# victoriyaforsythe/PyRayHF

Measured on AMD Instinct MI355X. Metric: virtual-height integrals/s (profile x frequency pairs), higher is better.
Workload: dtype f64

## Files before the change

### include/prhf.h

```cpp
#ifndef PRHF_H
#define PRHF_H

#include <stdint.h>

#ifdef __cplusplus
extern "C" {
#endif

#define PRHF_ABI_VERSION 4

#define PRHF_OK        0
#define PRHF_EINVAL   -1
#define PRHF_ENEGDEN  -2
#define PRHF_EPEAK0   -3
#define PRHF_EHIP     -4
#define PRHF_ENOMEM   -5

#define PRHF_MODE_O 0
#define PRHF_MODE_X 1

#define PRHF_FLAG_DEVICE_PTRS 0x1u
#define PRHF_FLAG_ASYNC       0x2u
#define PRHF_FLAG_GRID_STABLE 0x4u
#define PRHF_FLAG_SHARED_FIELD 0x8u
// ... 162 lines not shown
                                      double phi_max, int32_t renormalize_every, double fill_n, double fill_grad,
                                      double fill_mup, double* out, double* path_t, double* path_r, double* path_phi,
                                      double* path_v_r, double* path_v_phi, int64_t path_stride, uint32_t flags);

int prhf_gradient_home_f64(prhf_ctx* ctx, int32_t geometry, const double* records, int64_t n_fields, int64_t n0,
                           int64_t n1, const double* axis0, const double* axis1, const int64_t* group_field,
                           const double* group_x0_km, const double* group_z0_km, int64_t n_groups,
                           const int64_t* link_group, const double* link_target_km, int64_t n_links,
                           const double* scan_elevation_deg, int64_t n_scan, double earth_radius_km, double s_max_km,
                           double rtol, double atol, double max_step_km, double z_ground_km, double top, double left,
                           double right, int32_t renormalize_every, double fill_n, double fill_grad, double fill_mup,
                           double range_tol_km, int32_t max_iter, int32_t max_roots, double* out, int64_t* n_brackets,
                           uint32_t flags);

int prhf_gradient_home_counters(prhf_ctx* ctx, uint64_t* counters);

int prhf_trace_gradient_hops_f64(prhf_ctx* ctx, int32_t geometry, const double* records, int64_t n_fields, int64_t n0,
                                 int64_t n1, const double* axis0, const double* axis1, const double* x0_km,
                                 const double* z0_km, const double* elevation_deg, const int64_t* ray_field, int64_t n_rays,
                                 double earth_radius_km, double s_max_km, double rtol, double atol, double max_step_km,
                                 double z_ground_km, double top, double left, double right, int32_t renormalize_every,
                                 double fill_n, double fill_grad, double fill_mup, int32_t n_hops, double* out,
                                 double* path_t, double* path_a, double* path_b, double* path_va, double* path_vb,
                                 int64_t path_stride, uint32_t flags);

int prhf_gradient_hop_home_f64(prhf_ctx* ctx, int32_t geometry, const double* records, int64_t n_fields, int64_t n0,
                               int64_t n1, const double* axis0, const double* axis1, const int64_t* group_field,
                               const double* group_x0_km, const double* group_z0_km, int64_t n_groups,
                               const int64_t* link_group, const double* link_target_km, int64_t n_links,
                               const double* scan_elevation_deg, int64_t n_scan, double earth_radius_km, double s_max_km,
                               double rtol, double atol, double max_step_km, double z_ground_km, double top, double left,
                               double right, int32_t renormalize_every, double fill_n, double fill_grad, double fill_mup,
                               double range_tol_km, int32_t max_iter, int32_t max_roots, int32_t n_hops, double* out,
                               int64_t* n_brackets, uint32_t flags);

int prhf_field_build_f64(prhf_ctx* ctx, const double* den, const double* bmag, const double* bpsi, int64_t n0, int64_t n1,
                         const double* axis0, const double* axis1, const double* freq_hz, int64_t n_freq, int32_t mode,
                         int32_t edge_order, double* records, double* mu_out, double* mup_out, uint32_t flags);

int prhf_gradient_skip_f64(prhf_ctx* ctx, int32_t geometry, const double* records, int64_t n_fields, int64_t n0,
                           int64_t n1, const double* axis0, const double* axis1, const int64_t* group_field,
                           const double* group_x0_km, const double* group_z0_km, int64_t n_groups,
                           const double* scan_elevation_deg, int64_t n_scan, double earth_radius_km, double s_max_km,
                           double rtol, double atol, double max_step_km, double z_ground_km, double top, double left,
                           double right, int32_t renormalize_every, double fill_n, double fill_grad, double fill_mup,
                           double elev_tol_deg, int32_t max_iter, double* out, uint32_t flags);

int prhf_gradient_muf_f64(prhf_ctx* ctx, int32_t geometry, const double* den, const double* bmag, const double* bpsi,
                          int64_t n0, int64_t n1, const double* axis0, const double* axis1, int32_t mode, int32_t edge_order,
                          const double* link_x0_km, const double* link_z0_km, const double* link_target_km, int64_t n_links,
                          double f_lo_hz, double f_hi_hz, int32_t n_bisect, const double* scan_elevation_deg, int64_t n_scan,
                          double earth_radius_km, double s_max_km, double rtol, double atol, double max_step_km,
                          double z_ground_km, double top, double left, double right, int32_t renormalize_every,
                          double fill_n, double fill_grad, double fill_mup, double elev_tol_deg, int32_t max_iter,
                          double* out, uint32_t flags);

int prhf_gradient_skip_counters(prhf_ctx* ctx, uint64_t* counters);

int prhf_gradient_hop_skip_f64(prhf_ctx* ctx, int32_t geometry, const double* records, int64_t n_fields, int64_t n0,
                               int64_t n1, const double* axis0, const double* axis1, const int64_t* group_field,
                               const double* group_x0_km, const double* group_z0_km, int64_t n_groups,
                               const double* scan_elevation_deg, int64_t n_scan, double earth_radius_km, double s_max_km,
                               double rtol, double atol, double max_step_km, double z_ground_km, double top, double left,
                               double right, int32_t renormalize_every, double fill_n, double fill_grad, double fill_mup,
                               double elev_tol_deg, int32_t max_iter, int32_t n_hops, double* out, uint32_t flags);

int prhf_gradient_hop_muf_f64(prhf_ctx* ctx, int32_t geometry, const double* den, const double* bmag, const double* bpsi,
                              int64_t n0, int64_t n1, const double* axis0, const double* axis1, int32_t mode,
                              int32_t edge_order, const double* link_x0_km, const double* link_z0_km,
                              const double* link_target_km, int64_t n_links, double f_lo_hz, double f_hi_hz, int32_t n_bisect,
                              const double* scan_elevation_deg, int64_t n_scan, double earth_radius_km, double s_max_km,
                              double rtol, double atol, double max_step_km, double z_ground_km, double top, double left,
                              double right, int32_t renormalize_every, double fill_n, double fill_grad, double fill_mup,
                              double elev_tol_deg, int32_t max_iter, int32_t n_hops, double* out, uint32_t flags);

int prhf_gradient_hop_skip_counters(prhf_ctx* ctx, uint64_t* counters);

int prhf_pair_plan_counters(prhf_ctx* ctx, uint64_t* counters);

int prhf_panel_counters(prhf_ctx* ctx, uint64_t* counters);

int prhf_panel_upper_counters(prhf_ctx* ctx, uint64_t* counters);

int prhf_occupancy(prhf_ctx* ctx, int64_t n_alt, int32_t math, int32_t* workgroups_per_cu);

int prhf_sync(prhf_ctx* ctx);

int prhf_last_kernel_ms(prhf_ctx* ctx, double* ms);

int prhf_recent_kernel_ms(prhf_ctx* ctx, double* ms, int32_t capacity, int32_t* n);

#ifdef __cplusplus
}
#endif
#endif
```

### pyrayhf_amd/_native.py

```python

from __future__ import annotations

import ctypes
import os
import threading

_HERE = os.path.dirname(os.path.abspath(__file__))
LIB_PATH = os.environ.get("PRHF_LIB") or os.path.join(_HERE, "libprhf.so")

OK, EINVAL, ENEGDEN, EPEAK0, EHIP, ENOMEM = 0, -1, -2, -3, -4, -5
MODE_O, MODE_X = 0, 1
FLAG_DEVICE_PTRS, FLAG_ASYNC, FLAG_GRID_STABLE, FLAG_SHARED_FIELD = 0x1, 0x2, 0x4, 0x8
MATH_FAITHFUL, MATH_FAST, MATH_AUTO = 0, 1, 2
ABI_VERSION = 4

c_double_p = ctypes.POINTER(ctypes.c_double)


class Segment(ctypes.Structure):
    _fields_ = [("prof_begin", ctypes.c_int64), ("prof_end", ctypes.c_int64),
                ("mode", ctypes.c_int32), ("n_points", ctypes.c_int32),
                ("mult_offset", ctypes.c_int64), ("out_offset", ctypes.c_int64)]


# ... 60 lines not shown
    "prhf_snell_fan_f64": (ctypes.c_int, [
        ctypes.c_void_p, ctypes.c_int32, ctypes.c_void_p, ctypes.c_void_p, ctypes.c_int64, ctypes.c_void_p,
        ctypes.c_void_p, ctypes.c_int64, ctypes.c_void_p, ctypes.c_void_p, ctypes.c_void_p, ctypes.c_void_p,
        ctypes.c_int64, ctypes.c_int64, ctypes.c_int64, ctypes.c_int32, ctypes.c_double, ctypes.c_double,
        ctypes.c_double, ctypes.c_int32, ctypes.c_void_p, ctypes.c_void_p, ctypes.c_void_p, ctypes.c_int64,
        ctypes.c_uint32]),
    "prhf_snell_home_f64": (ctypes.c_int, [
        ctypes.c_void_p, ctypes.c_int32, ctypes.c_void_p, ctypes.c_void_p, ctypes.c_int64, ctypes.c_void_p,
        ctypes.c_void_p, ctypes.c_int64, ctypes.c_void_p, ctypes.c_int64, ctypes.c_void_p, ctypes.c_void_p,
        ctypes.c_void_p, ctypes.c_void_p, ctypes.c_int64, ctypes.c_int64, ctypes.c_int64, ctypes.c_int32,
        ctypes.c_double, ctypes.c_double, ctypes.c_double, ctypes.c_int32, ctypes.c_double, ctypes.c_int32,
        ctypes.c_int32, ctypes.c_void_p, ctypes.c_void_p, ctypes.c_uint32]),
    "prhf_snell_skip_f64": (ctypes.c_int, [
        ctypes.c_void_p, ctypes.c_int32, ctypes.c_void_p, ctypes.c_void_p, ctypes.c_int64, ctypes.c_void_p,
        ctypes.c_int64, ctypes.c_void_p, ctypes.c_void_p, ctypes.c_void_p, ctypes.c_void_p, ctypes.c_int64,
        ctypes.c_int64, ctypes.c_int64, ctypes.c_int32, ctypes.c_double, ctypes.c_double, ctypes.c_double,
        ctypes.c_int32, ctypes.c_double, ctypes.c_int32, ctypes.c_void_p, ctypes.c_uint32]),
    "prhf_snell_muf_f64": (ctypes.c_int, [
        ctypes.c_void_p, ctypes.c_int32, ctypes.c_void_p, ctypes.c_void_p, ctypes.c_int64, ctypes.c_double,
        ctypes.c_double, ctypes.c_int32, ctypes.c_void_p, ctypes.c_int64, ctypes.c_void_p, ctypes.c_void_p,
        ctypes.c_void_p, ctypes.c_void_p, ctypes.c_int64, ctypes.c_int64, ctypes.c_int64, ctypes.c_int32,
        ctypes.c_double, ctypes.c_double, ctypes.c_double, ctypes.c_int32, ctypes.c_double, ctypes.c_int32,
        ctypes.c_void_p, ctypes.c_uint32]),
    "prhf_field_pack_f64": (ctypes.c_int, [ctypes.c_void_p, ctypes.c_void_p, ctypes.c_void_p, ctypes.c_int64,
                                           ctypes.c_int64, ctypes.c_int64, ctypes.c_void_p, ctypes.c_void_p,
                                           ctypes.c_int32, ctypes.c_void_p, ctypes.c_uint32]),
    "prhf_field_sample_f64": (ctypes.c_int, [ctypes.c_void_p, ctypes.c_void_p, ctypes.c_int64, ctypes.c_int64,
                                             ctypes.c_int64] + [ctypes.c_void_p] * 5 + [ctypes.c_int64] +
                              [ctypes.c_double] * 3 + [ctypes.c_void_p] * 4 + [ctypes.c_uint32]),
    "prhf_trace_gradient_f64": (ctypes.c_int, [ctypes.c_void_p, ctypes.c_void_p, ctypes.c_int64, ctypes.c_int64,
                                               ctypes.c_int64] + [ctypes.c_void_p] * 6 + [ctypes.c_int64] +
                                [ctypes.c_double] * 8 + [ctypes.c_int32] + [ctypes.c_double] * 3 +
                                [ctypes.c_void_p] * 6 + [ctypes.c_int64, ctypes.c_uint32]),
    "prhf_trace_gradient_spherical_f64": (ctypes.c_int, [ctypes.c_void_p, ctypes.c_void_p, ctypes.c_int64, ctypes.c_int64,
                                                         ctypes.c_int64] + [ctypes.c_void_p] * 6 + [ctypes.c_int64] +
                                          [ctypes.c_double] * 9 + [ctypes.c_int32] + [ctypes.c_double] * 3 +
                                          [ctypes.c_void_p] * 6 + [ctypes.c_int64, ctypes.c_uint32]),
    "prhf_gradient_home_f64": (ctypes.c_int, [ctypes.c_void_p, ctypes.c_int32, ctypes.c_void_p, ctypes.c_int64,
                                              ctypes.c_int64, ctypes.c_int64] + [ctypes.c_void_p] * 5 + [ctypes.c_int64] +
                               [ctypes.c_void_p] * 2 + [ctypes.c_int64, ctypes.c_void_p, ctypes.c_int64] +
                               [ctypes.c_double] * 9 + [ctypes.c_int32] + [ctypes.c_double] * 4 +
                               [ctypes.c_int32, ctypes.c_int32, ctypes.c_void_p, ctypes.c_void_p, ctypes.c_uint32]),
    "prhf_gradient_home_counters": (ctypes.c_int, [ctypes.c_void_p, ctypes.POINTER(ctypes.c_uint64)]),
    "prhf_trace_gradient_hops_f64": (ctypes.c_int, [ctypes.c_void_p, ctypes.c_int32, ctypes.c_void_p, ctypes.c_int64,
                                                    ctypes.c_int64, ctypes.c_int64] + [ctypes.c_void_p] * 6 +
                                     [ctypes.c_int64] + [ctypes.c_double] * 9 + [ctypes.c_int32] + [ctypes.c_double] * 3 +
                                     [ctypes.c_int32] + [ctypes.c_void_p] * 6 + [ctypes.c_int64, ctypes.c_uint32]),
    "prhf_gradient_hop_home_f64": (ctypes.c_int, [ctypes.c_void_p, ctypes.c_int32, ctypes.c_void_p, ctypes.c_int64,
                                                  ctypes.c_int64, ctypes.c_int64] + [ctypes.c_void_p] * 5 +
                                   [ctypes.c_int64] + [ctypes.c_void_p] * 2 +
                                   [ctypes.c_int64, ctypes.c_void_p, ctypes.c_int64] + [ctypes.c_double] * 9 +
                                   [ctypes.c_int32] + [ctypes.c_double] * 4 +
                                   [ctypes.c_int32, ctypes.c_int32, ctypes.c_int32, ctypes.c_void_p, ctypes.c_void_p,
                                    ctypes.c_uint32]),
    "prhf_field_build_f64": (ctypes.c_int, [ctypes.c_void_p] * 4 + [ctypes.c_int64, ctypes.c_int64] +
                             [ctypes.c_void_p] * 3 + [ctypes.c_int64, ctypes.c_int32, ctypes.c_int32] +
                             [ctypes.c_void_p] * 3 + [ctypes.c_uint32]),
    "prhf_gradient_skip_f64": (ctypes.c_int, [ctypes.c_void_p, ctypes.c_int32, ctypes.c_void_p, ctypes.c_int64,
                                              ctypes.c_int64, ctypes.c_int64] + [ctypes.c_void_p] * 5 + [ctypes.c_int64] +
                               [ctypes.c_void_p, ctypes.c_int64] + [ctypes.c_double] * 9 + [ctypes.c_int32] +
                               [ctypes.c_double] * 4 + [ctypes.c_int32, ctypes.c_void_p, ctypes.c_uint32]),
    "prhf_gradient_muf_f64": (ctypes.c_int, [ctypes.c_void_p, ctypes.c_int32] + [ctypes.c_void_p] * 3 +
                              [ctypes.c_int64, ctypes.c_int64, ctypes.c_void_p, ctypes.c_void_p, ctypes.c_int32,
                               ctypes.c_int32] + [ctypes.c_void_p] * 3 +
                              [ctypes.c_int64, ctypes.c_double, ctypes.c_double, ctypes.c_int32, ctypes.c_void_p,
                               ctypes.c_int64] + [ctypes.c_double] * 9 + [ctypes.c_int32] + [ctypes.c_double] * 4 +
                              [ctypes.c_int32, ctypes.c_void_p, ctypes.c_uint32]),
    "prhf_gradient_hop_skip_f64": (ctypes.c_int, [ctypes.c_void_p, ctypes.c_int32, ctypes.c_void_p, ctypes.c_int64,
                                                  ctypes.c_int64, ctypes.c_int64] + [ctypes.c_void_p] * 5 +
                                   [ctypes.c_int64] + [ctypes.c_void_p, ctypes.c_int64] + [ctypes.c_double] * 9 +
                                   [ctypes.c_int32] + [ctypes.c_double] * 4 +
                                   [ctypes.c_int32, ctypes.c_int32, ctypes.c_void_p, ctypes.c_uint32]),
    "prhf_gradient_hop_muf_f64": (ctypes.c_int, [ctypes.c_void_p, ctypes.c_int32] + [ctypes.c_void_p] * 3 +
                                  [ctypes.c_int64, ctypes.c_int64, ctypes.c_void_p, ctypes.c_void_p, ctypes.c_int32,
                                   ctypes.c_int32] + [ctypes.c_void_p] * 3 +
                                  [ctypes.c_int64, ctypes.c_double, ctypes.c_double, ctypes.c_int32, ctypes.c_void_p,
                                   ctypes.c_int64] + [ctypes.c_double] * 9 + [ctypes.c_int32] + [ctypes.c_double] * 4 +
                                  [ctypes.c_int32, ctypes.c_int32, ctypes.c_void_p, ctypes.c_uint32]),
    "prhf_gradient_skip_counters": (ctypes.c_int, [ctypes.c_void_p, ctypes.POINTER(ctypes.c_uint64)]),
    "prhf_gradient_hop_skip_counters": (ctypes.c_int, [ctypes.c_void_p, ctypes.POINTER(ctypes.c_uint64)]),
    "prhf_pair_plan_counters": (ctypes.c_int, [ctypes.c_void_p, ctypes.POINTER(ctypes.c_uint64)]),
    "prhf_panel_counters": (ctypes.c_int, [ctypes.c_void_p, ctypes.POINTER(ctypes.c_uint64)]),
    "prhf_panel_upper_counters": (ctypes.c_int, [ctypes.c_void_p, ctypes.POINTER(ctypes.c_uint64)]),
    "prhf_occupancy": (ctypes.c_int, [ctypes.c_void_p, ctypes.c_int64, ctypes.c_int32,
                                      ctypes.POINTER(ctypes.c_int32)]),
    "prhf_sync": (ctypes.c_int, [ctypes.c_void_p]),
    "prhf_last_kernel_ms": (ctypes.c_int, [ctypes.c_void_p, ctypes.POINTER(ctypes.c_double)]),
    "prhf_recent_kernel_ms": (ctypes.c_int, [ctypes.c_void_p, ctypes.POINTER(ctypes.c_double), ctypes.c_int32,
                                             ctypes.POINTER(ctypes.c_int32)]),
}

_lib = None
_lib_lock = threading.Lock()


def load():
    global _lib
    if _lib is not None:
        return _lib
    with _lib_lock:
        if _lib is not None:
            return _lib
        if not os.path.exists(LIB_PATH):
            raise NativeLibraryError(
                f"{LIB_PATH} not found: build it with `python -c 'import __graft_entry__ as g; g.build()'` "
                "or `make -C pyrayhf_amd/csrc` (hipcc, gfx950). There is no CPU fallback.")
        if os.environ.get("PRHF_NO_TORCH_PRELOAD", "") == "":
            try:
                import torch
            except ImportError:
                pass
        try:
            lib = ctypes.CDLL(LIB_PATH)
        except OSError as exc:
            raise NativeLibraryError(f"cannot load {LIB_PATH}: {exc}") from exc
        for name, (res, args) in _PROTOTYPES.items():
            try:
                fn = getattr(lib, name)
            except AttributeError as exc:
                raise NativeLibraryError(f"{LIB_PATH} does not export {name}; rebuild it") from exc
            fn.restype = res
            fn.argtypes = args
        if lib.prhf_abi_version() != ABI_VERSION:
            raise NativeLibraryError(f"ABI version {lib.prhf_abi_version()} != {ABI_VERSION}; rebuild libprhf.so")
        _lib = lib
        return _lib


def exported_symbols():
    return sorted(_PROTOTYPES)


def last_error():
    msg = load().prhf_last_error()
    return msg.decode("utf-8", "replace") if msg else ""


def error_for(code, msg):
    if code == ENEGDEN:
        return ValueError("Density must be non-negative")
    if code == EPEAK0:
        return IndexError(msg or "density peak at index 0")
    if code == EINVAL:
        return ValueError(msg or "invalid argument")
    if code == ENOMEM:
        return MemoryError(msg)
    return NativeLibraryError(msg or f"libprhf error {code}")


def raise_for(code):
    if code == OK:
        return
    raise error_for(code, last_error())


def device_count():
    n = ctypes.c_int(0)
    raise_for(load().prhf_device_count(ctypes.byref(n)))
    return n.value


class Context:

    def __init__(self, device=0):
        self._lib = load()
        self._h = ctypes.c_void_p()
# ... 173 lines not shown
                                                      *(float(v) for v in controls[:8]), int(controls[8]),
                                                      *(float(v) for v in fills), int(n_hops), out, *paths,
                                                      int(path_stride), flags)

    def gradient_hop_home(self, geometry, records, n_fields, n0, n1, axis0, axis1, group_field, group_x0, group_z0, n_groups,
                          link_group, link_target, n_links, scan_elev, n_scan, earth_radius, controls, fills, range_tol,
                          max_iter, max_roots, n_hops, out, n_brackets, flags):
        return self._lib.prhf_gradient_hop_home_f64(self._h, int(geometry), records, n_fields, n0, n1, axis0, axis1,
                                                    group_field, group_x0, group_z0, n_groups, link_group, link_target,
                                                    n_links, scan_elev, n_scan, float(earth_radius),
                                                    *(float(v) for v in controls[:8]), int(controls[8]),
                                                    *(float(v) for v in fills), float(range_tol), int(max_iter),
                                                    int(max_roots), int(n_hops), out, n_brackets, flags)

    def gradient_home_counters(self):
        buf = (ctypes.c_uint64 * 4)()
        raise_for(self._lib.prhf_gradient_home_counters(self._h, buf))
        return tuple(int(v) for v in buf)

    def field_build(self, den, bmag, bpsi, n0, n1, axis0, axis1, freq_hz, n_freq, mode, edge_order, records, mu, mup,
                    flags):
        return self._lib.prhf_field_build_f64(self._h, den, bmag, bpsi, n0, n1, axis0, axis1, freq_hz, n_freq, int(mode),
                                              int(edge_order), records, mu or None, mup or None, flags)

    def gradient_skip(self, geometry, records, n_fields, n0, n1, axis0, axis1, group_field, group_x0, group_z0, n_groups,
                      scan_elev, n_scan, earth_radius, controls, fills, elev_tol, max_iter, out, flags):
        return self._lib.prhf_gradient_skip_f64(self._h, int(geometry), records, n_fields, n0, n1, axis0, axis1,
                                                group_field, group_x0, group_z0, n_groups, scan_elev, n_scan,
                                                float(earth_radius), *(float(v) for v in controls[:8]), int(controls[8]),
                                                *(float(v) for v in fills), float(elev_tol), int(max_iter), out, flags)

    def gradient_muf(self, geometry, den, bmag, bpsi, n0, n1, axis0, axis1, mode, edge_order, link_x0, link_z0, link_target,
                     n_links, f_lo, f_hi, n_bisect, scan_elev, n_scan, earth_radius, controls, fills, elev_tol, max_iter,
                     out, flags):
        return self._lib.prhf_gradient_muf_f64(self._h, int(geometry), den, bmag, bpsi, n0, n1, axis0, axis1, int(mode),
                                               int(edge_order), link_x0, link_z0, link_target, n_links, float(f_lo),
                                               float(f_hi), int(n_bisect), scan_elev, n_scan, float(earth_radius),
                                               *(float(v) for v in controls[:8]), int(controls[8]),
                                               *(float(v) for v in fills), float(elev_tol), int(max_iter), out, flags)

    def gradient_hop_skip(self, geometry, records, n_fields, n0, n1, axis0, axis1, group_field, group_x0, group_z0, n_groups,
                          scan_elev, n_scan, earth_radius, controls, fills, elev_tol, max_iter, n_hops, out, flags):
        return self._lib.prhf_gradient_hop_skip_f64(self._h, int(geometry), records, n_fields, n0, n1, axis0, axis1,
                                                    group_field, group_x0, group_z0, n_groups, scan_elev, n_scan,
                                                    float(earth_radius), *(float(v) for v in controls[:8]),
                                                    int(controls[8]), *(float(v) for v in fills), float(elev_tol),
                                                    int(max_iter), int(n_hops), out, flags)

    def gradient_hop_muf(self, geometry, den, bmag, bpsi, n0, n1, axis0, axis1, mode, edge_order, link_x0, link_z0,
                         link_target, n_links, f_lo, f_hi, n_bisect, scan_elev, n_scan, earth_radius, controls, fills,
                         elev_tol, max_iter, n_hops, out, flags):
        return self._lib.prhf_gradient_hop_muf_f64(self._h, int(geometry), den, bmag, bpsi, n0, n1, axis0, axis1, int(mode),
                                                   int(edge_order), link_x0, link_z0, link_target, n_links, float(f_lo),
                                                   float(f_hi), int(n_bisect), scan_elev, n_scan, float(earth_radius),
                                                   *(float(v) for v in controls[:8]), int(controls[8]),
                                                   *(float(v) for v in fills), float(elev_tol), int(max_iter),
                                                   int(n_hops), out, flags)

    def gradient_hop_skip_counters(self):
        buf = (ctypes.c_uint64 * 5)()
        raise_for(self._lib.prhf_gradient_hop_skip_counters(self._h, buf))
        return tuple(int(v) for v in buf)

    def gradient_skip_counters(self):
        buf = (ctypes.c_uint64 * 4)()
        raise_for(self._lib.prhf_gradient_skip_counters(self._h, buf))
        return tuple(int(v) for v in buf)

    def pair_plan_counters(self):
        buf = (ctypes.c_uint64 * 2)()
        raise_for(self._lib.prhf_pair_plan_counters(self._h, buf))
        return tuple(int(v) for v in buf)

    def panel_counters(self):
        buf = (ctypes.c_uint64 * 2)()
        raise_for(self._lib.prhf_panel_counters(self._h, buf))
        return tuple(int(v) for v in buf)

    def panel_upper_counters(self):
        buf = (ctypes.c_uint64 * 2)()
        raise_for(self._lib.prhf_panel_upper_counters(self._h, buf))
        return tuple(int(v) for v in buf)

    def occupancy(self, n_alt, math):
        n = ctypes.c_int32(0)
        raise_for(self._lib.prhf_occupancy(self._h, int(n_alt), int(math), ctypes.byref(n)))
        return n.value

    def sync(self):
        return self._lib.prhf_sync(self._h)

    def last_kernel_ms(self):
        ms = ctypes.c_double(0.0)
        raise_for(self._lib.prhf_last_kernel_ms(self._h, ctypes.byref(ms)))
        return ms.value

    def recent_kernel_ms(self, count=64):
        buf = (ctypes.c_double * max(int(count), 1))()
        n = ctypes.c_int32(0)
        raise_for(self._lib.prhf_recent_kernel_ms(self._h, buf, int(count), ctypes.byref(n)))
        return [buf[i] for i in range(n.value)]


_tls = threading.local()


def default_device():
    for key in ("PRHF_DEVICE", "LOCAL_RANK"):
        if os.environ.get(key, "") != "":
            return int(os.environ[key])
    return 0


def host_context(device=None):
    ctx = context(device)
    ctx.set_stream(0, borrow=False)
    return ctx


def context(device=None):
    dev = default_device() if device is None else int(device)
    cache = getattr(_tls, "ctx", None)
    if cache is None:
        cache = _tls.ctx = {}
    ctx = cache.get(dev)
    if ctx is None:
        ctx = cache[dev] = Context(dev)
    return ctx
```

### pyrayhf_amd/csrc/prhf_api.cpp

```cpp

#include <hip/hip_runtime_api.h>

#include <algorithm>
#include <cctype>
#include <cmath>
#include <cstdarg>
#include <cstdio>
#include <cstdlib>
#include <cstring>
#include <new>
#include <string>
#include <vector>
#include <xmmintrin.h>

#include "prhf.h"
#include "prhf_kernels.h"
#include "prhf_plan.h"

namespace {

thread_local std::string g_err;

int fail(int code, const char* fmt, ...) {
    char buf[512];
// ... 44 lines not shown
    int prev_ = -1;
    bool switched_ = false;
    hipError_t err_ = hipSuccess;
};
#define ENTER_DEVICE(dev)            \
    DeviceScope device_scope_(dev);  \
    HIP_TRY(device_scope_.error())

hipError_t create_events_untimed(hipEvent_t* ev, int n) {
    for (int i = 0; i < n; ++i) {
        const hipError_t e = hipEventCreateWithFlags(&ev[i], hipEventDisableTiming);
        if (e != hipSuccess) return e;
    }
    return hipSuccess;
}

hipError_t create_events(hipEvent_t* ev, int n) {
    for (int i = 0; i < n; ++i) {
        const hipError_t e = hipEventCreate(&ev[i]);
        if (e != hipSuccess) return e;
    }
    return hipSuccess;
}

}

struct prhf_ctx {
    int device = 0;
    hipStream_t own_stream = nullptr;
    hipStream_t aux_stream = nullptr;
    hipEvent_t fork_ev = nullptr, join_ev = nullptr;
    hipStream_t up_stream = nullptr, down_stream = nullptr;
    hipEvent_t slab_up[3] = {}, slab_done[3] = {}, slab_free = nullptr;
    hipStream_t stream = nullptr;
    static constexpr int kTimingRing = 64;
    hipEvent_t ring0[kTimingRing] = {}, ring1[kTimingRing] = {};
    unsigned long long n_timed = 0;
    int slot = 0;
    int pending = 0;
    bool timed = false;
    hipEvent_t begin_ev() { pending = (int)(n_timed % kTimingRing); return ring0[pending]; }
    hipEvent_t pending_end_ev() const { return ring1[pending]; }
    hipEvent_t end_ev() const { return ring1[slot]; }
    void mark_timed() { slot = pending; ++n_timed; timed = true; }
    int math = PRHF_MATH_AUTO;
    Knobs knobs;
    int cu_count = 256;
    int large_bar = 0;
    DevBuf arena;
    DevBuf partial;
    DevBuf altmin;
    DevBuf pairs;
    DevBuf ftab;
    DevBuf levels;
    DevBuf ptab;
    DevBuf leftover;
    DevBuf leftover_x;
    DevBuf leftover_tall;
    DevBuf leftover_tall_x;
    DevBuf order;
    DevBuf tall;
    DevBuf vjp;
    const double* pairs_src = nullptr;
    int64_t pairs_len = 0;
    prhf::StridedPieces pairs_pieces = {};
    struct HostGrid {
        const double* host = nullptr;
        int64_t len = 0;
        DevBuf mult, pairs;
        bool pairs_ready = false;
        prhf::StridedPieces pieces = {};
    };
    static constexpr int kHostGrids = 16;
    HostGrid host_grid[kHostGrids];
    int n_host_grids = 0;
    bool order_clean = false;
    unsigned* d_status = nullptr;
    unsigned* h_status = nullptr;
    unsigned* h_status_dev = nullptr;
    double* h_pack = nullptr;
    double* h_pack_dev = nullptr;
    unsigned long long* d_words = nullptr;
    unsigned long long* h_words = nullptr;
    unsigned long long* d_plan_counters = nullptr;
    bool status_pending = false;
    uint64_t grad_home_counters[PRHF_GRAD_HOME_COUNTERS] = {};
    DevBuf fields;
    uint64_t grad_skip_counters[PRHF_GRAD_SKIP_COUNTERS + 1] = {};
};

namespace {

int ensure(prhf_ctx* c, DevBuf& b, size_t bytes) {
    if (bytes <= b.cap) return PRHF_OK;
    if (b.p) {
        HIP_TRY(hipStreamSynchronize(c->stream));
        HIP_TRY(hipFree(b.p));
        b.p = nullptr;
        b.cap = 0;
    }
    size_t want = bytes + bytes / 4 + 4096;
    hipError_t e = hipMalloc(&b.p, want);
    if (e != hipSuccess) {
        b.p = nullptr;
        return fail(PRHF_ENOMEM, "hipMalloc(%zu) failed: %s", want, hipGetErrorString(e));
    }
    b.cap = want;
    return PRHF_OK;
}

struct Residual {
    const double* vh_obs;
    double* residual;
    double* cost;
    int64_t n_iono = 0;
    const int32_t* ionogram_of_row = nullptr;
    int64_t* best = nullptr;
    double* best_cost = nullptr;
    size_t cost_elems(int64_t n_prof) const { return (size_t)n_prof * (size_t)(n_iono && !ionogram_of_row ? n_iono : 1); }
};

int status_to_code(unsigned bits) {
    if (bits & PRHF_STATUS_PEAK0)
        return fail(PRHF_EPEAK0, "density peak at index 0: no bottomside levels below the peak");
    if (bits & PRHF_STATUS_NANINPUT)
        return fail(PRHF_EINVAL, "NaN in a profile (alt, bmag or bpsi below the density peak)");
    if (bits & PRHF_STATUS_NEGDEN) return fail(PRHF_ENEGDEN, "Density must be non-negative");
    if (bits & PRHF_STATUS_BADGROUP) return fail(PRHF_EINVAL, "ray_group outside [0, n_groups)");
    if (bits & PRHF_STATUS_BADINDEX) return fail(PRHF_EINVAL, "profile_index outside [0, n_prof)");
    if (bits & PRHF_STATUS_BADFIELD) return fail(PRHF_EINVAL, "field index outside [0, n_fields)");
    if (bits & PRHF_STATUS_PATHLEN) return fail(PRHF_EINVAL, "a ray has more path nodes than path_stride");
    return PRHF_OK;
}

struct Call {
    prhf_ctx* c;
    const double *freq, *den, *bmag, *bpsi, *alt, *mult;
    int64_t n_freq, n_prof, n_alt, prof_stride, alt_stride, mult_len;
    const prhf_segment* segs;
    int32_t n_segs;
    double* out;
    uint32_t flags;
    const Residual* post;
    bool dev, shared_field;
    prhf_ctx::HostGrid* grid;
    double* d_out;
    size_t in_elems, out_elems;
    bool out_direct;
    double* vh_dev;
    const double* d_obs;
    double *d_res, *d_cost;
    const int32_t* d_ion;
    int64_t* d_best;
    double* d_best_cost;
    unsigned* order_made;
};

prhf_ctx::HostGrid* find_host_grid(prhf_ctx* c, const double* mult, int64_t mult_len) {
    for (int g = 0; g < c->n_host_grids; ++g)
        if (c->host_grid[g].host == mult && c->host_grid[g].len == mult_len) return &c->host_grid[g];
    return nullptr;
}

int check_arguments(const Call& k) {
    if (!k.c) return fail(PRHF_EINVAL, "null context");
    if (!k.freq || !k.den || !k.bmag || !k.bpsi || !k.alt || !k.mult || !k.segs || (!k.out && !k.post))
        return fail(PRHF_EINVAL, "null array pointer");
    if (k.post && (!k.post->vh_obs || (!k.post->residual && !k.post->cost)))
        return fail(PRHF_EINVAL, "null array pointer");
    if (k.n_freq < 1 || k.n_prof < 0 || k.n_alt < 1) return fail(PRHF_EINVAL, "bad shape");
    if (k.n_alt > kMaxAltTall) return fail(PRHF_EINVAL, "n_alt %lld exceeds the limit of %lld levels",
                                           (long long)k.n_alt, kMaxAltTall);
    if (k.n_freq > (1 << 20)) return fail(PRHF_EINVAL, "n_freq too large");
    if (k.prof_stride < k.n_alt || (k.alt_stride != 0 && k.alt_stride < k.n_alt))
        return fail(PRHF_EINVAL, "row stride shorter than a row");
    if (k.n_segs < 1 || k.n_segs > PRHF_MAX_SEGMENTS)
        return fail(PRHF_EINVAL, "1..%d segments per launch", PRHF_MAX_SEGMENTS);
    if (k.flags & ~(PRHF_FLAG_DEVICE_PTRS | PRHF_FLAG_ASYNC | PRHF_FLAG_GRID_STABLE | PRHF_FLAG_SHARED_FIELD))
        return fail(PRHF_EINVAL, "unknown flag bits");
    if ((k.flags & PRHF_FLAG_ASYNC) && !k.dev) return fail(PRHF_EINVAL, "PRHF_FLAG_ASYNC needs device pointers");
    const bool grid_known = !k.dev && (k.flags & PRHF_FLAG_GRID_STABLE) && find_host_grid(k.c, k.mult, k.mult_len);
    if (!k.dev && !grid_known) {
        const long long bad = first_decreasing_grid_entry(k.mult, k.mult_len, k.segs, k.n_segs);
        if (bad >= 0) return fail(PRHF_EINVAL, "multiplier[%lld] decreases: the stretched grid must be non-decreasing", bad);
    }
    return PRHF_OK;
}

int decide_tall(const Call& k, bool& tall, long long& lds_levels) {
    prhf_ctx* c = k.c;
    tall = k.n_alt > kMaxAlt;
    lds_levels = k.n_alt;
    if (!(tall && k.n_prof > 0 && c->knobs.trim_lds != 0)) return PRHF_OK;
    long long max_peak = 0;
    if (k.dev) {
        HIP_TRY(hipMemsetAsync(c->d_status + kWordPeak, 0, sizeof(unsigned), c->stream));
        HIP_TRY(prhf::launch_peak_levels(k.den, k.n_prof, k.n_alt, k.prof_stride, c->d_status + kWordPeak, c->stream));
        unsigned peak = 0;
        HIP_TRY(hipMemcpyAsync(&peak, c->d_status + kWordPeak, sizeof(unsigned), hipMemcpyDeviceToHost, c->stream));
        HIP_TRY(hipStreamSynchronize(c->stream));
        max_peak = peak;
    } else {
        for (int64_t p = 0; p < k.n_prof; ++p) {
            const double* d = k.den + (size_t)p * k.prof_stride;
            double bv = -HUGE_VAL;
            long long bi = 0;
            for (int64_t i = 0; i < k.n_alt; ++i) {
                const double key = (d[i] != d[i]) ? HUGE_VAL : d[i];
                if (key > bv) { bv = key; bi = i; }
            }
            max_peak = std::max(max_peak, bi);
        }
    }
    if (max_peak + 1 <= kMaxAlt) {
// ... 153 lines not shown
    int rc;
    if ((rc = ensure(c, table, (size_t)pl.table_entries * 16)) != PRHF_OK) return rc;
    HIP_TRY(prhf::launch_grid_pairs(d_mult, mult_len, static_cast<double*>(table.p), c->stream));
    HIP_TRY(prhf::launch_grid_strided(d_mult, static_cast<double*>(table.p), pl.pieces, c->stream));
    return PRHF_OK;
}

int update_tables(Call& k, const LaunchPlan& pl, prhf::KArgs& a) {
    prhf_ctx* c = k.c;
    if (!pl.want_pairs) return PRHF_OK;
    int rc;
    auto same_pieces = [&](const prhf::StridedPieces& o) { return std::memcmp(&o, &pl.pieces, sizeof pl.pieces) == 0; };
    if (k.grid) {
        if (!k.grid->pairs_ready || !same_pieces(k.grid->pieces)) {
            if ((rc = build_pair_table(c, k.grid->pairs, a.mult, k.mult_len, pl)) != PRHF_OK) return rc;
            k.grid->pairs_ready = true;
            k.grid->pieces = pl.pieces;
        }
        a.pairs = static_cast<const double*>(k.grid->pairs.p);
    } else {
        const bool stable = k.dev && (k.flags & PRHF_FLAG_GRID_STABLE) != 0;
        if (!(stable && c->pairs.p && c->pairs_src == a.mult && c->pairs_len == k.mult_len && same_pieces(c->pairs_pieces))) {
            c->pairs_src = nullptr;
            if ((rc = build_pair_table(c, c->pairs, a.mult, k.mult_len, pl)) != PRHF_OK) return rc;
            if (stable) {
                c->pairs_src = a.mult;
                c->pairs_len = k.mult_len;
                c->pairs_pieces = pl.pieces;
            }
        }
        a.pairs = static_cast<const double*>(c->pairs.p);
    }
    if (!pl.freq_table) return PRHF_OK;
    if ((rc = ensure(c, c->ftab, ((size_t)k.n_freq + 1) * 64)) != PRHF_OK) return rc;
    prhf::ZeroWords zero;
    std::memset(&zero, 0, sizeof zero);
    auto zero_head = [&](DevBuf& b, size_t bytes) -> int {
        int rcz = ensure(c, b, bytes);
        if (rcz != PRHF_OK) return rcz;
        zero.p[zero.n] = static_cast<unsigned*>(b.p);
        zero.words[zero.n++] = 1;
        return PRHF_OK;
    };
    zero.p[zero.n] = c->d_status;
    zero.words[zero.n++] = kStatusWords;
    if (pl.o.blocks > 0) {
        if ((rc = zero_head(c->leftover, pl.o.list_bytes)) != PRHF_OK) return rc;
        if ((rc = zero_head(c->leftover_tall, pl.o.list_bytes)) != PRHF_OK) return rc;
    }
    if (pl.x.blocks > 0) {
        if ((rc = zero_head(c->leftover_x, pl.x.list_bytes)) != PRHF_OK) return rc;
        if ((rc = zero_head(c->leftover_tall_x, pl.x.list_bytes)) != PRHF_OK) return rc;
    }
    if (pl.short_order) {
        const size_t words = PRHF_ORDER_CLASSES * (size_t)(pl.o.blocks + 1);
        const void* before = c->order.p;
        if ((rc = ensure(c, c->order, words * sizeof(unsigned))) != PRHF_OK) return rc;
        unsigned* order = static_cast<unsigned*>(c->order.p);
        if (!c->order_clean || c->order.p != before)
            HIP_TRY(hipMemsetAsync(order, 0, PRHF_ORDER_CLASSES * sizeof(unsigned), c->stream));
        prhf::KArgs ap = a;
        ap.n_segs = pl.o.n_segs;
        ap.n_blocks = pl.o.blocks;
        std::copy(pl.o.seg, pl.o.seg + pl.o.n_segs, ap.seg);
        c->order_clean = false;
        HIP_TRY(prhf::launch_short_order(ap, order, a.freq, static_cast<double*>(c->ftab.p), zero, c->stream));
        k.order_made = order;
    } else {
        HIP_TRY(prhf::launch_freq_table(a.freq, k.n_freq, static_cast<double*>(c->ftab.p), zero, c->stream));
    }
    a.ftab = static_cast<const double*>(c->ftab.p);
    return PRHF_OK;
}

int zero_control_words(prhf_ctx* c, const LaunchPlan& pl) {
    if (!pl.zero_queues) return PRHF_OK;
    HIP_TRY(hipMemsetAsync(c->d_status, 0, kLaunchQueueWords * sizeof(unsigned), c->stream));
    if (pl.x.n_segs > 0) HIP_TRY(hipMemsetAsync(c->d_status + kWordShortXFull, 0, sizeof(unsigned), c->stream));
    return PRHF_OK;
}

int launch_general(prhf_ctx* c, const LaunchPlan& pl, prhf::KArgs& a) {
    if (pl.queue) a.queue = c->d_status + kWordGeneral;
    if (pl.tall) HIP_TRY(prhf::launch_vfo_tall(a, pl.grid, c->stream));
    else HIP_TRY(prhf::launch_vfo(a, pl.grid, pl.launch_tier, pl.lds_bytes, c->stream));
    return PRHF_OK;
}

struct ShortRoute {
    StatusWord first, full, follow;
    DevBuf *left, *left_tall;
    int follow_tier;
    unsigned* order;
    bool traced;
};

template <class Launch>
int launch_short_kind(prhf_ctx* c, const LaunchPlan& pl, const ShortKind& sk, const ShortRoute& r, const prhf::KArgs& a,
                      hipStream_t stream, Launch launch) {
    if (sk.blocks == 0) return PRHF_OK;
    prhf::KArgs as = a;
    as.n_segs = sk.n_segs;
    std::copy(sk.seg, sk.seg + sk.n_segs, as.seg);
    as.n_blocks = sk.blocks;
    as.short_prio = (int)c->knobs.short_prio;
    as.partial = nullptr;
    as.altmin = nullptr;
    as.trace = nullptr;
    int rc;
#ifdef PRHF_TRACE
    static DevBuf trace_short;
    const size_t short_trace_words = (size_t)sk.blocks * kWavesPerBlock * 8;
    unsigned long long* trace = nullptr;
    if (std::getenv("PRHF_TRACE_FILE") && r.traced) {
        if ((rc = ensure(c, trace_short, short_trace_words * 8)) != PRHF_OK) return rc;
        HIP_TRY(hipMemsetAsync(trace_short.p, 0, short_trace_words * 8, stream));
        as.trace = trace = static_cast<unsigned long long*>(trace_short.p);
    }
#endif
    if ((rc = ensure(c, *r.left, sk.list_bytes)) != PRHF_OK) return rc;
    as.leftover = static_cast<unsigned*>(r.left->p);
    if (!pl.freq_table) HIP_TRY(hipMemsetAsync(as.leftover, 0, sizeof(unsigned), stream));
    if (sk.second) {
        if ((rc = ensure(c, *r.left_tall, sk.list_bytes)) != PRHF_OK) return rc;
        as.leftover_tall = static_cast<unsigned*>(r.left_tall->p);
        if (!pl.freq_table) HIP_TRY(hipMemsetAsync(as.leftover_tall, 0, sizeof(unsigned), stream));
    }
    as.lds_levels = sk.first.lds_levels;
    as.short_queue = sk.first.short_queue;
    as.queue = sk.first.queue ? c->d_status + r.first : nullptr;
    as.order = r.order;
    if ((rc = launch(as, sk.first)) != PRHF_OK) return rc;
    if (sk.second) {
        as.trace = nullptr;
        as.lds_levels = sk.full.lds_levels;
        as.short_queue = sk.full.short_queue;
        as.block_list = as.leftover_tall;
        as.order = nullptr;
        as.leftover_tall = nullptr;
        as.queue = c->d_status + r.full;
        if ((rc = launch(as, sk.full)) != PRHF_OK) return rc;
    }
#ifdef PRHF_TRACE
    if (trace) {
        std::vector<unsigned long long> host(short_trace_words);
        HIP_TRY(hipMemcpyAsync(host.data(), trace, short_trace_words * 8, hipMemcpyDeviceToHost, stream));
        HIP_TRY(hipStreamSynchronize(stream));
        if (FILE* fp = std::fopen(std::getenv("PRHF_TRACE_FILE"), "wb")) {
            std::fwrite(host.data(), 8, short_trace_words, fp);
            std::fclose(fp);
        }
    }
#endif
    as.trace = nullptr;
    as.lds_levels = a.lds_levels;
    as.short_queue = sk.first.short_queue;
    as.leftover_tall = nullptr;
    as.order = nullptr;
    as.block_list = as.leftover;
    as.leftover = nullptr;
    as.queue = c->d_status + r.follow;
    as.zero_after = r.order;
    HIP_TRY(prhf::launch_vfo(as, sk.follow_grid, r.follow_tier, pl.lds_bytes, stream));
    if (as.zero_after) c->order_clean = true;
    return PRHF_OK;
}

// ... 58 lines not shown
        HIP_TRY(prhf::launch_vfo_shortx(as, l.grid, l.lds_bytes, l.threads, short_stream));
        return PRHF_OK;
    });
    if (rc != PRHF_OK) return rc;
    rc = launch_short_kind(c, pl, pl.o, route_o, a, short_stream, [&](const prhf::KArgs& as, const ShortLaunch& l) -> int {
        HIP_TRY(prhf::launch_vfo_short(as, l.grid, l.lds_bytes, l.threads, pl.o.lanes, short_stream));
        return PRHF_OK;
    });
    if (rc != PRHF_OK) return rc;
    if (pl.forked) {
        HIP_TRY(hipEventRecord(c->join_ev, c->aux_stream));
        HIP_TRY(hipStreamWaitEvent(c->stream, c->join_ev, 0));
        return PRHF_OK;
    }
    return launch_general(c, pl, a);
}

int download_and_sync(Call& k) {
    prhf_ctx* c = k.c;
    const size_t out_elems = k.out_elems;
    const bool out_via_pack = !k.out_direct && !k.dev && k.out && out_elems && c->h_pack && out_elems * 8 <= kPackBytes / 4 &&
                              k.in_elems * 8 <= kPackBytes / 2;
    double* h_out = c->h_pack ? c->h_pack + kPackBytes / 16 : nullptr;
    if (k.out_direct) {
    } else if (out_via_pack)
        HIP_TRY(hipMemcpyAsync(h_out, k.d_out, out_elems * 8, hipMemcpyDeviceToHost, c->stream));
    else if (!k.dev && out_elems && k.out)
        HIP_TRY(hipMemcpyAsync(k.out, k.d_out, out_elems * 8, hipMemcpyDeviceToHost, c->stream));
    if (!k.dev && k.post) {
        if (k.post->residual)
            HIP_TRY(hipMemcpyAsync(k.post->residual, k.d_res, out_elems * 8, hipMemcpyDeviceToHost, c->stream));
        if (k.post->cost && !k.post->n_iono)
            HIP_TRY(hipMemcpyAsync(k.post->cost, k.d_cost, (size_t)k.n_prof * 8, hipMemcpyDeviceToHost, c->stream));
        if (k.post->n_iono) {
            if (k.post->cost_elems(k.n_prof))
                HIP_TRY(hipMemcpyAsync(k.post->cost, k.d_cost, k.post->cost_elems(k.n_prof) * 8, hipMemcpyDeviceToHost,
                                       c->stream));
            HIP_TRY(hipMemcpyAsync(k.post->best, k.d_best, (size_t)k.post->n_iono * 8, hipMemcpyDeviceToHost, c->stream));
            HIP_TRY(hipMemcpyAsync(k.post->best_cost, k.d_best_cost, (size_t)k.post->n_iono * 8, hipMemcpyDeviceToHost, c->stream));
        }
    }
    if (k.flags & PRHF_FLAG_ASYNC) return PRHF_OK;
    const int rc = prhf_sync(c);
    if (out_via_pack || k.out_direct) std::memcpy(k.out, h_out, out_elems * 8);
    return rc;
}

int run(prhf_ctx* c, const double* freq, int64_t n_freq, const double* den, const double* bmag,
        const double* bpsi, const double* alt, int64_t n_prof, int64_t n_alt, int64_t prof_stride,
        int64_t alt_stride, const double* mult, int64_t mult_len, const prhf_segment* segs, int32_t n_segs,
        double* out, uint32_t flags, const Residual* post = nullptr) {
    Call k = {c, freq, den, bmag, bpsi, alt, mult, n_freq, n_prof, n_alt, prof_stride, alt_stride, mult_len, segs, n_segs,
              out, flags, post, (flags & PRHF_FLAG_DEVICE_PTRS) != 0, (flags & PRHF_FLAG_SHARED_FIELD) != 0};
    int rc;
    if ((rc = check_arguments(k)) != PRHF_OK) return rc;
    ENTER_DEVICE(c->device);
    bool tall;
    long long lds_levels;
    if ((rc = decide_tall(k, tall, lds_levels)) != PRHF_OK) return rc;

    const LaunchShape shape = {n_prof, n_freq, n_alt, lds_levels, tall, mult_len, c->cu_count, c->math};
    LaunchPlan pl;
    char why[160];
    if (plan_launch(shape, segs, n_segs, c->knobs, pl, why, sizeof why) != PRHF_OK) return fail(PRHF_EINVAL, "%s", why);

    prhf::KArgs a;
    std::memset(&a, 0, sizeof a);
    a.n_freq = n_freq;
    a.n_alt = n_alt;
    a.lds_levels = lds_levels;
    a.n_segs = pl.n_segs;
    std::copy(pl.seg, pl.seg + pl.n_segs, a.seg);
    a.n_blocks = pl.blocks;
    a.no_candidates = pl.no_candidates;
    a.plan_counters = c->d_plan_counters;
    a.plan_cap = (int)c->knobs.pair_plan_cap;
    if ((rc = stage_inputs(k, pl, a)) != PRHF_OK) return rc;

    const bool timed_launch = k.dev || c->knobs.timing != 0;
    if (timed_launch) HIP_TRY(hipEventRecord(c->begin_ev(), c->stream));
    if ((rc = update_tables(k, pl, a)) != PRHF_OK) return rc;
#ifdef PRHF_TRACE
    static DevBuf trace_buf;
    const size_t trace_words = (size_t)pl.blocks * kWavesPerBlock * 6;
    if (std::getenv("PRHF_TRACE_FILE") && pl.blocks > 0) {
        if ((rc = ensure(c, trace_buf, trace_words * 8)) != PRHF_OK) return rc;
        HIP_TRY(hipMemsetAsync(trace_buf.p, 0, trace_words * 8, c->stream));
        a.trace = static_cast<unsigned long long*>(trace_buf.p);
    }
#endif
    if (pl.tall_stride) {
        a.tall_stride = pl.tall_stride;
        if ((rc = ensure(c, c->tall, (size_t)pl.tall_slabs * a.tall_stride)) != PRHF_OK) return rc;
        a.tall = static_cast<unsigned char*>(c->tall.p);
    }
    if ((rc = zero_control_words(c, pl)) != PRHF_OK) return rc;
    if ((rc = launch_all(k, pl, a)) != PRHF_OK) return rc;
#ifdef PRHF_TRACE
    if (a.trace) {
        std::vector<unsigned long long> host(trace_words);
        HIP_TRY(hipMemcpyAsync(host.data(), a.trace, trace_words * 8, hipMemcpyDeviceToHost, c->stream));
        HIP_TRY(hipStreamSynchronize(c->stream));
        if (FILE* fp = std::fopen(std::getenv("PRHF_TRACE_FILE"), "wb")) {
            std::fwrite(host.data(), 8, trace_words, fp);
            std::fclose(fp);
        }
    }
#endif
    if (post && post->n_iono) {
        if ((rc = launch_many(c, k.vh_dev, n_prof, k.d_obs, post->n_iono, n_freq, k.d_ion, k.d_res, k.d_cost, k.d_best,
                              k.d_best_cost)) != PRHF_OK) return rc;
    } else if (post) HIP_TRY(prhf::launch_residual(k.vh_dev, k.d_obs, n_prof, (int)n_freq, k.d_res, k.d_cost, c->stream));
    if (timed_launch) {
        HIP_TRY(hipEventRecord(c->pending_end_ev(), c->stream));
        c->mark_timed();
    }
    c->status_pending = true;
    return download_and_sync(k);
}

int run_host_slabs(prhf_ctx* c, const double* freq, int64_t n_freq, const double* den, const double* bmag,
                   const double* bpsi, const double* alt, int64_t n_prof, int64_t n_alt, int64_t prof_stride,
                   int64_t alt_stride, const double* mult, int32_t n_points, int32_t mode, double* out, uint32_t flags) {
    const bool shared_field = (flags & PRHF_FLAG_SHARED_FIELD) != 0;
    ENTER_DEVICE(c->device);
    const size_t n_alt_rows = alt_stride ? (size_t)n_prof : 1, n_field_rows = shared_field ? 1 : (size_t)n_prof;
    const size_t row_bytes = (size_t)n_alt * 8;
    const size_t elems = (size_t)n_freq + ((size_t)n_prof + 2 * n_field_rows + n_alt_rows) * (size_t)n_alt + (size_t)n_points +
                         (size_t)n_prof * (size_t)n_freq;
    int rc;
    if ((rc = ensure(c, c->arena, elems * 8)) != PRHF_OK) return rc;
    double* d_freq = static_cast<double*>(c->arena.p);
    double* d_den = d_freq + n_freq;
    double* d_bmag = d_den + (size_t)n_prof * n_alt;
    double* d_bpsi = d_bmag + n_field_rows * n_alt;
    double* d_alt = d_bpsi + n_field_rows * n_alt;
    double* d_mult = d_alt + n_alt_rows * n_alt;
    double* d_out = d_mult + n_points;
    HIP_TRY(hipEventRecord(c->slab_free, c->stream));
    HIP_TRY(hipStreamWaitEvent(c->up_stream, c->slab_free, 0));
    HIP_TRY(hipMemcpyAsync(d_freq, freq, (size_t)n_freq * 8, hipMemcpyHostToDevice, c->up_stream));
    HIP_TRY(hipMemcpyAsync(d_mult, mult, (size_t)n_points * 8, hipMemcpyHostToDevice, c->up_stream));
    if (!alt_stride) HIP_TRY(hipMemcpyAsync(d_alt, alt, row_bytes, hipMemcpyHostToDevice, c->up_stream));
    if (shared_field) {
        HIP_TRY(hipMemcpyAsync(d_bmag, bmag, row_bytes, hipMemcpyHostToDevice, c->up_stream));
        HIP_TRY(hipMemcpyAsync(d_bpsi, bpsi, row_bytes, hipMemcpyHostToDevice, c->up_stream));
    }
    const int n_slabs = 3;
    const int64_t cut[4] = {0, std::max<int64_t>(1, n_prof / 10), std::max<int64_t>(2, (n_prof * 4) / 10), n_prof};
    const uint32_t dev_flags = PRHF_FLAG_DEVICE_PTRS | PRHF_FLAG_ASYNC | (shared_field ? PRHF_FLAG_SHARED_FIELD : 0);
    int first_error = PRHF_OK;
    for (int k = 0; k < n_slabs && first_error == PRHF_OK; ++k) {
        const int64_t p0 = cut[k], rows = cut[k + 1] - cut[k];
        if (rows <= 0) continue;
        auto up2d = [&](double* dst, const double* src, int64_t stride) {
            return hipMemcpy2DAsync(dst + (size_t)p0 * n_alt, row_bytes, src + (size_t)p0 * stride, (size_t)stride * 8, row_bytes,
                                    (size_t)rows, hipMemcpyHostToDevice, c->up_stream);
        };
        HIP_TRY(up2d(d_den, den, prof_stride));
        if (!shared_field) {
            HIP_TRY(up2d(d_bmag, bmag, prof_stride));
            HIP_TRY(up2d(d_bpsi, bpsi, prof_stride));
        }
        if (alt_stride) HIP_TRY(up2d(d_alt, alt, alt_stride));
        HIP_TRY(hipEventRecord(c->slab_up[k], c->up_stream));
        HIP_TRY(hipStreamWaitEvent(c->stream, c->slab_up[k], 0));
        prhf_segment seg;
        seg.prof_begin = 0;
        seg.prof_end = rows;
        seg.mode = mode;
        seg.n_points = n_points;
        seg.mult_offset = 0;
        seg.out_offset = 0;
        rc = run(c, d_freq, n_freq, d_den + (size_t)p0 * n_alt, shared_field ? d_bmag : d_bmag + (size_t)p0 * n_alt,
                 shared_field ? d_bpsi : d_bpsi + (size_t)p0 * n_alt, alt_stride ? d_alt + (size_t)p0 * n_alt : d_alt, rows, n_alt,
                 n_alt, alt_stride ? n_alt : 0, d_mult, n_points, &seg, 1, d_out + (size_t)p0 * n_freq, dev_flags);
        if (rc != PRHF_OK) { first_error = rc; break; }
        HIP_TRY(hipEventRecord(c->slab_done[k], c->stream));
        if (k > 0) {
            HIP_TRY(hipStreamWaitEvent(c->down_stream, c->slab_done[k - 1], 0));
            HIP_TRY(hipMemcpyAsync(out + (size_t)cut[k - 1] * n_freq, d_out + (size_t)cut[k - 1] * n_freq,
                                   (size_t)(cut[k] - cut[k - 1]) * n_freq * 8, hipMemcpyDeviceToHost, c->down_stream));
        }
    }
    if (first_error == PRHF_OK) {
        HIP_TRY(hipStreamWaitEvent(c->down_stream, c->slab_done[n_slabs - 1], 0));
        HIP_TRY(hipMemcpyAsync(out + (size_t)cut[n_slabs - 1] * n_freq, d_out + (size_t)cut[n_slabs - 1] * n_freq,
                               (size_t)(cut[n_slabs] - cut[n_slabs - 1]) * n_freq * 8, hipMemcpyDeviceToHost, c->down_stream));
    }
    HIP_TRY(hipStreamSynchronize(c->up_stream));
    const int rc_sync = prhf_sync(c);
    HIP_TRY(hipStreamSynchronize(c->down_stream));
    return first_error != PRHF_OK ? first_error : rc_sync;
}

}

extern "C" {

int prhf_abi_version(void) { return PRHF_ABI_VERSION; }

const char* prhf_last_error(void) { return g_err.c_str(); }

int prhf_device_count(int* n) {
    if (!n) return fail(PRHF_EINVAL, "null pointer");
    *n = 0;
    HIP_TRY(hipGetDeviceCount(n));
    return PRHF_OK;
}

int prhf_ctx_create(int device, prhf_ctx** out) {
    if (!out) return fail(PRHF_EINVAL, "null pointer");
    *out = nullptr;
    int n = 0;
    HIP_TRY(hipGetDeviceCount(&n));
    if (device < 0 || device >= n) return fail(PRHF_EINVAL, "device %d not in [0, %d)", device, n);
    ENTER_DEVICE(device);
    prhf_ctx* c = new (std::nothrow) prhf_ctx;
    if (!c) return fail(PRHF_ENOMEM, "out of host memory");
    c->device = device;
    hipError_t e;
    if ((e = hipStreamCreateWithFlags(&c->own_stream, hipStreamNonBlocking)) != hipSuccess ||
        (e = hipStreamCreateWithFlags(&c->aux_stream, hipStreamNonBlocking)) != hipSuccess ||
        (e = hipEventCreateWithFlags(&c->fork_ev, hipEventDisableTiming)) != hipSuccess ||
        (e = hipEventCreateWithFlags(&c->join_ev, hipEventDisableTiming)) != hipSuccess ||
        (e = hipStreamCreateWithFlags(&c->up_stream, hipStreamNonBlocking)) != hipSuccess ||
        (e = hipStreamCreateWithFlags(&c->down_stream, hipStreamNonBlocking)) != hipSuccess ||
        (e = hipEventCreateWithFlags(&c->slab_free, hipEventDisableTiming)) != hipSuccess ||
        (e = create_events_untimed(c->slab_up, 3)) != hipSuccess ||
        (e = create_events_untimed(c->slab_done, 3)) != hipSuccess ||
        (e = create_events(c->ring0, prhf_ctx::kTimingRing)) != hipSuccess ||
        (e = create_events(c->ring1, prhf_ctx::kTimingRing)) != hipSuccess ||
        (e = hipMalloc(reinterpret_cast<void**>(&c->d_status), kStatusWords * sizeof(unsigned))) != hipSuccess ||
        (e = hipHostMalloc(reinterpret_cast<void**>(&c->h_status), PRHF_STATUS_WORDS * sizeof(unsigned),
                           hipHostMallocMapped | hipHostMallocCoherent)) != hipSuccess ||
        (e = hipHostGetDevicePointer(reinterpret_cast<void**>(&c->h_status_dev), c->h_status, 0)) != hipSuccess ||
        (e = hipMemset(c->d_status, 0, kStatusWords * sizeof(unsigned))) != hipSuccess ||
        (e = hipHostMalloc(reinterpret_cast<void**>(&c->h_pack), kPackBytes, hipHostMallocMapped | hipHostMallocCoherent)) !=
            hipSuccess ||
        (e = hipHostGetDevicePointer(reinterpret_cast<void**>(&c->h_pack_dev), c->h_pack, 0)) != hipSuccess ||
        (e = hipMalloc(reinterpret_cast<void**>(&c->d_words), 2 * sizeof(unsigned long long))) != hipSuccess ||
        (e = hipHostMalloc(reinterpret_cast<void**>(&c->h_words), 2 * sizeof(unsigned long long),
                           hipHostMallocDefault)) != hipSuccess ||
        (e = hipMalloc(reinterpret_cast<void**>(&c->d_plan_counters), 6 * sizeof(unsigned long long))) != hipSuccess ||
        (e = hipMemset(c->d_plan_counters, 0, 6 * sizeof(unsigned long long))) != hipSuccess ||
        (e = prhf::configure_kernels(staged_lds_bytes(kMaxAlt))) != hipSuccess) {
        prhf_ctx_destroy(c);
        return fail(PRHF_EHIP, "context setup failed: %s", hipGetErrorString(e));
    }
    c->stream = c->own_stream;
    std::memset(c->h_status, 0, PRHF_STATUS_WORDS * sizeof(unsigned));
#ifdef PRHF_DIAG
    for (const KnobName& k : kKnobNames) {
        std::string env = "PRHF_";
        for (const char* p = k.name; *p; ++p) env += (char)std::toupper((unsigned char)*p);
        if (const char* v = std::getenv(env.c_str())) c->knobs.*(k.field) = std::min(k.hi, std::max(k.lo, std::atof(v)));
    }
#endif
    (void)hipDeviceGetAttribute(&c->cu_count, hipDeviceAttributeMultiprocessorCount, device);
    if (hipDeviceGetAttribute(&c->large_bar, hipDeviceAttributeIsLargeBar, device) != hipSuccess) c->large_bar = 0;
    if (c->cu_count < 1) c->cu_count = 256;
    *out = c;
    return PRHF_OK;
}

int prhf_ctx_destroy(prhf_ctx* c) {
    if (!c) return PRHF_OK;
    DeviceScope device_scope_(c->device);
    if (c->stream) (void)hipStreamSynchronize(c->stream);
    if (c->arena.p) (void)hipFree(c->arena.p);
    if (c->partial.p) (void)hipFree(c->partial.p);
    if (c->altmin.p) (void)hipFree(c->altmin.p);
    if (c->pairs.p) (void)hipFree(c->pairs.p);
    if (c->ftab.p) (void)hipFree(c->ftab.p);
    if (c->levels.p) (void)hipFree(c->levels.p);
    if (c->ptab.p) (void)hipFree(c->ptab.p);
    if (c->leftover.p) (void)hipFree(c->leftover.p);
    if (c->leftover_x.p) (void)hipFree(c->leftover_x.p);
    if (c->leftover_tall.p) (void)hipFree(c->leftover_tall.p);
    if (c->leftover_tall_x.p) (void)hipFree(c->leftover_tall_x.p);
    if (c->order.p) (void)hipFree(c->order.p);
    if (c->tall.p) (void)hipFree(c->tall.p);
    if (c->vjp.p) (void)hipFree(c->vjp.p);
    if (c->fields.p) (void)hipFree(c->fields.p);
    for (int g = 0; g < c->n_host_grids; ++g) {
        if (c->host_grid[g].mult.p) (void)hipFree(c->host_grid[g].mult.p);
        if (c->host_grid[g].pairs.p) (void)hipFree(c->host_grid[g].pairs.p);
    }
    if (c->d_status) (void)hipFree(c->d_status);
    if (c->h_status) (void)hipHostFree(c->h_status);
    if (c->h_pack) (void)hipHostFree(c->h_pack);
    if (c->d_words) (void)hipFree(c->d_words);
    if (c->h_words) (void)hipHostFree(c->h_words);
    if (c->d_plan_counters) (void)hipFree(c->d_plan_counters);
    for (int i = 0; i < prhf_ctx::kTimingRing; ++i) {
        if (c->ring0[i]) (void)hipEventDestroy(c->ring0[i]);
        if (c->ring1[i]) (void)hipEventDestroy(c->ring1[i]);
    }
    if (c->aux_stream) { (void)hipStreamSynchronize(c->aux_stream); (void)hipStreamDestroy(c->aux_stream); }
    if (c->up_stream) { (void)hipStreamSynchronize(c->up_stream); (void)hipStreamDestroy(c->up_stream); }
    if (c->down_stream) { (void)hipStreamSynchronize(c->down_stream); (void)hipStreamDestroy(c->down_stream); }
    for (int i = 0; i < 3; ++i) {
        if (c->slab_up[i]) (void)hipEventDestroy(c->slab_up[i]);
        if (c->slab_done[i]) (void)hipEventDestroy(c->slab_done[i]);
    }
    if (c->slab_free) (void)hipEventDestroy(c->slab_free);
    if (c->fork_ev) (void)hipEventDestroy(c->fork_ev);
    if (c->join_ev) (void)hipEventDestroy(c->join_ev);
    if (c->own_stream) (void)hipStreamDestroy(c->own_stream);
    delete c;
    return PRHF_OK;
}

int prhf_ctx_set_stream(prhf_ctx* c, void* hip_stream, int32_t borrow) {
    if (!c) return fail(PRHF_EINVAL, "null context");
    hipStream_t next = borrow ? static_cast<hipStream_t>(hip_stream) : c->own_stream;
    if (next == c->stream) return PRHF_OK;
    ENTER_DEVICE(c->device);
    if (c->timed) HIP_TRY(hipStreamWaitEvent(next, c->end_ev(), 0));
    c->stream = next;
    return PRHF_OK;
}

int prhf_ctx_set_option(prhf_ctx* c, const char* name, double value) {
    if (!c || !name) return fail(PRHF_EINVAL, "null pointer");
    for (const KnobName& k : kKnobNames)
        if (std::strcmp(k.name, name) == 0) {
            if (!(value >= k.lo && value <= k.hi))
                return fail(PRHF_EINVAL, "option %s: %g outside [%g, %g]", name, value, k.lo, k.hi);
// ... 1704 lines not shown
    HIP_TRY(hipEventRecord(c->pending_end_ev(), c->stream));
    c->mark_timed();
    c->status_pending = true;
    if (!dev) HIP_TRY(hipMemcpyAsync(out, d_result, out_elems * 8, hipMemcpyDeviceToHost, c->stream));
    return grad_skip_finish(c, h.queue);
}
}

int prhf_gradient_muf_f64(prhf_ctx* c, int32_t geometry, const double* den, const double* bmag, const double* bpsi, int64_t n0,
                          int64_t n1, const double* axis0, const double* axis1, int32_t mode, int32_t edge_order,
                          const double* link_x0_km, const double* link_z0_km, const double* link_target_km, int64_t n_links,
                          double f_lo_hz, double f_hi_hz, int32_t n_bisect, const double* scan_elevation_deg, int64_t n_scan,
                          double earth_radius_km, double s_max_km, double rtol, double atol, double max_step_km,
                          double z_ground_km, double top, double left, double right, int32_t renormalize_every, double fill_n,
                          double fill_grad, double fill_mup, double elev_tol_deg, int32_t max_iter, double* out, uint32_t flags) {
    if (!c) return fail(PRHF_EINVAL, "null context");
    return grad_muf_run(c, 0, geometry, den, bmag, bpsi, n0, n1, axis0, axis1, mode, edge_order, link_x0_km, link_z0_km, link_target_km,
                        n_links, f_lo_hz, f_hi_hz, n_bisect, scan_elevation_deg, n_scan, earth_radius_km, s_max_km, rtol, atol,
                        max_step_km, z_ground_km, top, left, right, renormalize_every, fill_n, fill_grad, fill_mup, elev_tol_deg,
                        max_iter, out, flags);
}

int prhf_gradient_hop_muf_f64(prhf_ctx* c, int32_t geometry, const double* den, const double* bmag, const double* bpsi,
                              int64_t n0, int64_t n1, const double* axis0, const double* axis1, int32_t mode,
                              int32_t edge_order, const double* link_x0_km, const double* link_z0_km,
                              const double* link_target_km, int64_t n_links, double f_lo_hz, double f_hi_hz, int32_t n_bisect,
                              const double* scan_elevation_deg, int64_t n_scan, double earth_radius_km, double s_max_km,
                              double rtol, double atol, double max_step_km, double z_ground_km, double top, double left,
                              double right, int32_t renormalize_every, double fill_n, double fill_grad, double fill_mup,
                              double elev_tol_deg, int32_t max_iter, int32_t n_hops, double* out, uint32_t flags) {
    if (!c) return fail(PRHF_EINVAL, "null context");
    if (n_hops < 1 || n_hops > PRHF_GRAD_MAX_HOPS) return fail(PRHF_EINVAL, "n_hops is 1 .. 16");
    return grad_muf_run(c, n_hops, geometry, den, bmag, bpsi, n0, n1, axis0, axis1, mode, edge_order, link_x0_km, link_z0_km, link_target_km,
                        n_links, f_lo_hz, f_hi_hz, n_bisect, scan_elevation_deg, n_scan, earth_radius_km, s_max_km, rtol, atol,
                        max_step_km, z_ground_km, top, left, right, renormalize_every, fill_n, fill_grad, fill_mup, elev_tol_deg,
                        max_iter, out, flags);
}

int prhf_gradient_skip_counters(prhf_ctx* c, uint64_t* counters) {
    if (!c || !counters) return fail(PRHF_EINVAL, "null pointer");
    for (int k = 0; k < PRHF_GRAD_SKIP_COUNTERS; ++k) counters[k] = c->grad_skip_counters[k];
    return PRHF_OK;
}

int prhf_gradient_hop_skip_counters(prhf_ctx* c, uint64_t* counters) {
    if (!c || !counters) return fail(PRHF_EINVAL, "null pointer");
    for (int k = 0; k <= PRHF_GRAD_SKIP_COUNTERS; ++k) counters[k] = c->grad_skip_counters[k];
    return PRHF_OK;
}

int prhf_pair_plan_counters(prhf_ctx* c, uint64_t* counters) {
    if (!c || !counters) return fail(PRHF_EINVAL, "null pointer");
    DeviceScope device_scope_(c->device);
    unsigned long long w[2] = {0, 0};
    HIP_TRY(hipStreamSynchronize(c->stream));
    HIP_TRY(hipMemcpy(w, c->d_plan_counters, sizeof w, hipMemcpyDeviceToHost));
    counters[0] = w[0];
    counters[1] = w[1];
    return PRHF_OK;
}

int prhf_panel_counters(prhf_ctx* c, uint64_t* counters) {
    if (!c || !counters) return fail(PRHF_EINVAL, "null pointer");
    DeviceScope device_scope_(c->device);
    unsigned long long w[2] = {0, 0};
    HIP_TRY(hipStreamSynchronize(c->stream));
    HIP_TRY(hipMemcpy(w, c->d_plan_counters + 2, sizeof w, hipMemcpyDeviceToHost));
    counters[0] = w[0];
    counters[1] = w[1];
    return PRHF_OK;
}

int prhf_panel_upper_counters(prhf_ctx* c, uint64_t* counters) {
    if (!c || !counters) return fail(PRHF_EINVAL, "null pointer");
    DeviceScope device_scope_(c->device);
    unsigned long long w[2] = {0, 0};
    HIP_TRY(hipStreamSynchronize(c->stream));
    HIP_TRY(hipMemcpy(w, c->d_plan_counters + 4, sizeof w, hipMemcpyDeviceToHost));
    counters[0] = w[0] - w[1];
    counters[1] = w[1];
    return PRHF_OK;
}

int prhf_occupancy(prhf_ctx* c, int64_t n_alt, int32_t math, int32_t* workgroups_per_cu) {
    if (!c || !workgroups_per_cu) return fail(PRHF_EINVAL, "null pointer");
    if (n_alt < 1 || n_alt > kMaxAlt) return fail(PRHF_EINVAL, "n_alt out of range");
    ENTER_DEVICE(c->device);
    int n = 0;
    HIP_TRY(prhf::query_occupancy(math, staged_lds_bytes(n_alt), &n));
    *workgroups_per_cu = n;
    return PRHF_OK;
}

int prhf_sync(prhf_ctx* c) {
    if (!c) return fail(PRHF_EINVAL, "null context");
    ENTER_DEVICE(c->device);
    HIP_TRY(hipStreamSynchronize(c->stream));
    if (c->status_pending) {
        c->status_pending = false;
        unsigned bits = 0;
        for (int b = 0; b < PRHF_STATUS_WORDS; ++b) {
            if (reinterpret_cast<volatile unsigned*>(c->h_status)[b]) bits |= 1u << b;
            c->h_status[b] = 0;
        }
        return status_to_code(bits);
    }
    return PRHF_OK;
}

int prhf_last_kernel_ms(prhf_ctx* c, double* ms) {
    if (!c || !ms) return fail(PRHF_EINVAL, "null pointer");
    if (!c->timed) return fail(PRHF_EINVAL, "no launch has been timed on this context");
    ENTER_DEVICE(c->device);
    HIP_TRY(hipEventSynchronize(c->end_ev()));
    float t = 0.f;
    HIP_TRY(hipEventElapsedTime(&t, c->ring0[c->slot], c->end_ev()));
    *ms = t;
    return PRHF_OK;
}

int prhf_recent_kernel_ms(prhf_ctx* c, double* ms, int32_t capacity, int32_t* n_out) {
    if (!c || !ms || !n_out || capacity < 0) return fail(PRHF_EINVAL, "null pointer or negative capacity");
    ENTER_DEVICE(c->device);
    long long n = (long long)std::min<unsigned long long>(c->n_timed, (unsigned long long)prhf_ctx::kTimingRing);
    if (n > capacity) n = capacity;
    *n_out = (int32_t)n;
    if (n == 0) return PRHF_OK;
    HIP_TRY(hipEventSynchronize(c->end_ev()));
    for (long long i = 0; i < n; ++i) {
        const int s = (int)((c->n_timed - (unsigned long long)n + (unsigned long long)i) % prhf_ctx::kTimingRing);
        float t = 0.f;
        HIP_TRY(hipEventElapsedTime(&t, c->ring0[s], c->ring1[s]));
        ms[i] = t;
    }
    return PRHF_OK;
}

}
```

### pyrayhf_amd/csrc/prhf_kernels.h

```cpp
#ifndef PRHF_KERNELS_H
#define PRHF_KERNELS_H

#include <hip/hip_runtime_api.h>
#include <stddef.h>
#include <stdint.h>

#define PRHF_KMODE_O 0
#define PRHF_KMODE_X 1

#define PRHF_STATUS_NEGDEN 0x1
#define PRHF_STATUS_PEAK0  0x2
#define PRHF_STATUS_BADINDEX 0x4
#define PRHF_STATUS_BADFIELD 0x20
#define PRHF_STATUS_PATHLEN 0x40
#define PRHF_STATUS_WORDS 8
#define PRHF_STATUS_NANINPUT 0x10
#define PRHF_STATUS_BADGROUP 0x8

#ifndef PRHF_BLOCK_THREADS
#define PRHF_BLOCK_THREADS 512
#endif
#ifndef PRHF_SHORT_THREADS
#define PRHF_SHORT_THREADS 512
#endif
#ifndef PRHF_SHORT_WAVES_PER_SIMD
#define PRHF_SHORT_WAVES_PER_SIMD 4
#endif
#define PRHF_HINT_BUCKETS 1024
#define PRHF_MAX_CAND 1024
#define PRHF_MAX_SEGMENTS 8
#define PRHF_RED_DOUBLES 160
#define PRHF_NODE_BYTES 96
#define PRHF_SNODE_BYTES 80
#define PRHF_SHORT_MIN_POINTS 2
#define PRHF_SHORT_MAX_POINTS 1024
#define PRHF_SHORTX_MAX_POINTS 1024
#define PRHF_SHORT_MASKS 32
#define PRHF_SHORT_MAX_QUEUE 4096
#define PRHF_ORDER_CLASSES 16
#ifndef PRHF_COMPACT_THREADS
#define PRHF_COMPACT_THREADS 256
#endif
#ifndef PRHF_COMPACT_WGS_PER_CU
#define PRHF_COMPACT_WGS_PER_CU 4
#endif
#ifndef PRHF_COMPACT_MIN_QUEUE
#define PRHF_COMPACT_MIN_QUEUE 256
#endif
#define PRHF_PAIR_PAD 256
#ifndef PRHF_TOP_MIN_POINTS
#define PRHF_TOP_MIN_POINTS 1024
#endif
#ifndef PRHF_TOP3_MIN_POINTS
#define PRHF_TOP3_MIN_POINTS 8192
#endif
#ifndef PRHF_STRIDED_MIN_SEGMENT
#define PRHF_STRIDED_MIN_SEGMENT 64
#endif
#ifndef PRHF_PANEL_BLOCK
#define PRHF_PANEL_BLOCK 128
#endif
#ifndef PRHF_PANEL_MIN_SEGMENT
#define PRHF_PANEL_MIN_SEGMENT 8
#endif
#ifndef PRHF_MIN_WAVES_PER_SIMD
#define PRHF_MIN_WAVES_PER_SIMD 4
#endif

namespace prhf {

constexpr int short_waves_per_simd(int threads) {
    return threads < PRHF_SHORT_THREADS && threads * PRHF_COMPACT_WGS_PER_CU / 256 > PRHF_SHORT_WAVES_PER_SIMD
               ? threads * PRHF_COMPACT_WGS_PER_CU / 256 : PRHF_SHORT_WAVES_PER_SIMD;
}

struct SegDev {
    long long prof_begin, prof_end;
    long long mult_off;
    long long out_off;
    long long block_begin;
    long long partial_off;
    long long altmin_off;
    int mode, n_points;
    int chunks;
    int chunk_len;
    int slots;
    int blocks_per_prof;
    int tier;
    long long tail_prof;
    int tail_bpp;
    int panel_upper;
    double well_conditioned;
    int lean;
    int prio;
    long long sp_off;
    int strided_lower;
    int panel_lower;
    int panel_nodes;
    int strided_grade;
    int pair_plan;
    int thread_scan;
};

struct KArgs {
    const double* freq;
    const double* den;
    const double* bmag;
    const double* bpsi;
    const double* alt;
    const double* mult;
    const double* pairs;
    const double* ftab;
    double* out;
    double* partial;
    double* altmin;
    unsigned* status;
    unsigned* queue;
    long long n_blocks;
    unsigned long long* trace;
    long long n_freq, n_alt, prof_stride, alt_stride;
    long long field_stride;
    int n_segs;
    int no_candidates;
    unsigned* leftover;
    unsigned* leftover_tall;
    const unsigned* block_list;
    int short_queue;
    int short_prio;
    const unsigned* order;
    unsigned* zero_after;
    unsigned char* tall;
    unsigned long long tall_stride;
    long long lds_levels;
    unsigned long long* plan_counters;
    int plan_cap;
    SegDev seg[PRHF_MAX_SEGMENTS];
};

inline size_t lds_bytes_for(long long n_alt) {
    return (size_t)(n_alt + 1) * PRHF_NODE_BYTES + (size_t)n_alt * 16 + PRHF_HINT_BUCKETS * 2 + PRHF_MAX_CAND * 2 +
           PRHF_RED_DOUBLES * 8;
}

inline size_t lds_bytes_tall() { return PRHF_HINT_BUCKETS * 2 + PRHF_MAX_CAND * 2 + PRHF_RED_DOUBLES * 8; }
inline size_t tall_slab_bytes(long long n_alt) {
    return (((size_t)(n_alt + 1) * PRHF_NODE_BYTES + (size_t)n_alt * 16) + 255) & ~(size_t)255;
}

inline __host__ __device__ size_t short_lds_lists(long long n_alt, long long n_freq, int threads) {
    const size_t b = (size_t)(n_alt > n_freq ? n_alt : n_freq) * 8 + (size_t)n_freq * 24 + (size_t)(threads / 64) * PRHF_SHORT_MASKS * 12 +
                     PRHF_RED_DOUBLES * 8 + (size_t)n_freq * 4 + (size_t)n_freq * 2;
    return (b + 15) & ~(size_t)15;
}
inline size_t short_lds_fixed(long long n_alt, long long n_freq, int threads) {
    return short_lds_lists(n_alt, n_freq, threads) + (size_t)(n_alt + 1) * PRHF_SNODE_BYTES;
}
inline __host__ __device__ size_t shortx_lds_lists(long long n_alt, long long n_freq) {
    const size_t b = (size_t)n_alt * 16 + (size_t)n_freq * 24 + PRHF_RED_DOUBLES * 8 + (size_t)n_freq * 2;
    return (b + 15) & ~(size_t)15;
}
inline size_t shortx_lds_bytes(long long n_alt, long long n_freq) {
    return shortx_lds_lists(n_alt, n_freq) + (size_t)(n_alt + 1) * PRHF_SNODE_BYTES;
}
inline int short_queue_entries(long long n_alt, long long n_freq, size_t budget, int threads) {
    const size_t fixed = short_lds_fixed(n_alt, n_freq, threads);
    if (fixed + 8 * 64 > budget) return 0;
    const size_t q = (budget - fixed) / 8;
    return (int)(q > PRHF_SHORT_MAX_QUEUE ? PRHF_SHORT_MAX_QUEUE : q);
}

hipError_t configure_kernels(size_t max_lds_bytes);
hipError_t query_occupancy(int tier, size_t lds_bytes, int* blocks_per_cu);
hipError_t launch_grid_pairs(const double* mult, long long n, double* pairs, hipStream_t stream);
struct StridedPieces {
    int n;
    int n_points[PRHF_MAX_SEGMENTS];
    long long mult_off[PRHF_MAX_SEGMENTS];
    long long sp_off[PRHF_MAX_SEGMENTS];
};
inline long long strided_piece_entries(long long n_points) { return 1 + ((n_points + 7) / 8 + 1) + PRHF_PAIR_PAD; }
hipError_t launch_grid_strided(const double* mult, double* pairs, const StridedPieces& pc, hipStream_t stream);
struct ZeroWords {
    unsigned* p[8];
    int words[8];
    int n;
};
hipError_t launch_freq_table(const double* freq_mhz, long long n_freq, double* tab, const ZeroWords& zero, hipStream_t stream);
hipError_t launch_vfo(const KArgs& a, long long grid_blocks, int tier, size_t lds_bytes, hipStream_t stream);
hipError_t launch_vfo_tall(const KArgs& a, long long grid_blocks, hipStream_t stream);
hipError_t launch_peak_levels(const double* den, long long n_prof, long long n_alt, long long prof_stride,
                              unsigned* max_peak, hipStream_t stream);
hipError_t launch_vfo_short(const KArgs& a, long long grid_blocks, size_t lds_bytes, int threads, int lanes, hipStream_t stream);
hipError_t launch_short_order(const KArgs& a, unsigned* order, const double* freq_mhz, double* tab, const ZeroWords& zero,
                              hipStream_t stream);
hipError_t launch_vfo_shortx(const KArgs& a, long long grid_blocks, size_t lds_bytes, int threads, hipStream_t stream);
hipError_t launch_mu_mup(const double* X, const double* Y, const double* psi, long long n, int mode, int tier,
                         unsigned long long* absmax_scratch, unsigned long long* absmax_host,
                         double* mu, double* mup, hipStream_t stream);
hipError_t launch_find_vh(const double* X, const double* Y, const double* psi, const double* dh, long long n_rows,
                          long long n_cols, double alt_min, int mode, int tier,
                          unsigned long long* absmax_scratch, unsigned long long* absmax_host, double* vh,
                          hipStream_t stream);

struct RegridArgs {
    const double* freq_hz;
    const double* den;
    const double* bmag;
    const double* bpsi;
    const double* alt;
    const double* mult;
    double* out_freq;
    double* out_den;
    double* out_bmag;
    double* out_bpsi;
    double* out_dist;
    double* out_alt;
    double* out_crit;
    long long* out_ind;
    unsigned* status;
    long long n_freq, n_alt;
    long long lds_levels;
    int n_points, mode;
};
hipError_t launch_regrid(const RegridArgs& a, size_t lds_bytes, hipStream_t stream);
#define PRHF_VJP_THREADS 256
struct VjpArgs {
    const double* freq;
    const double* den;
    const double* bmag;
    const double* bpsi;
    const double* alt;
    const double* mult;
    const double* grad_vh;
    double* out;
    unsigned* status;
    long long n_prof, n_freq, n_alt;
    long long prof_stride, field_stride, alt_stride;
    long long lds_levels;
    int n_points, mode;
    int waves;
};
inline size_t vjp_lds_bytes(long long levels, int waves, bool jacobian) {
    return (size_t)(levels + 1) * PRHF_NODE_BYTES + (size_t)levels * 16 + PRHF_HINT_BUCKETS * 2 + PRHF_RED_DOUBLES * 8 +
           (size_t)waves * (jacobian ? 1 : 2) * (size_t)levels * 8;
}
hipError_t launch_vfo_vjp(const VjpArgs& a, bool jacobian, size_t lds_bytes, hipStream_t stream);
#define PRHF_SNELL_OUTPUTS 8
struct SnellArgs {
    const double* den;
    const double* bmag;
    const double* bpsi;
    const double* alt;
    const double* freq_hz;
    const double* elev_deg;
    const long long* prof_idx;
    const long long* ray_group;
    const double* group_freq;
    const long long* group_prof;
    long long n_groups;
    double* levels;
    double* group_entries;
    int* group_kidx;
    int* group_info;
    unsigned* ray_queue;
    int resident_cus;
    double* prof_info;
    double* ptab;
    long long n_prof;
    double* out;
    double* path_x;
    double* path_z;
// ... 228 lines not shown
```

### pyrayhf_amd/csrc/prhf_kernels.hip

```cpp

#include <hip/hip_runtime.h>
#include <stdint.h>

#include "prhf_crmath.h"
#include "prhf_kernels.h"

namespace prhf {

namespace {

constexpr double kPlasma = 8.97866275;
constexpr double kGyro = 2.799249247e10;
constexpr double kBackoff = 1e-6;
constexpr double kDegToRad = 0.017453292519943295;
constexpr double kUnmagTol = 1e-12;
constexpr double kLightKmS = 299792.458;
constexpr double kPolyAngle = 3e-4;
constexpr double kQuadAngle = 4e-5;
constexpr double kTrigAngle = 0.05;
constexpr double kLinTol = 1e-10;

struct __attribute__((aligned(16))) Node {
    double alt, off, den, sden, b, sb, u0, u1, u2, u3, psi, spsi;
};
// ... 247 lines not shown
    double col_star = 0.0;
    if (MODE == PRHF_KMODE_O) {
        const double ulp_half = f2 * 0x1p-53;
        const int stride = (K + 63) >> 6;
        const int probe = min((lane + 1) * stride - 1, K - 1);
        const unsigned long long coarse = __ballot((pf2[probe] - f2) > ulp_half);
        double amax = -__builtin_inf(), a_star = 0.0;
        if (coarse) {
            const int lo = (__ffsll((long long)coarse) - 1) * stride;
            const int k = min(lo + lane, K - 1);
            const unsigned long long fine = __ballot(lane < stride && (pf2[k] - f2) > ulp_half);
            kstar = lo + __ffsll((long long)fine) - 1;
            a_star = pf2[kstar];
            if (kstar > 0) amax = pf2[kstar - 1];
        } else {
            amax = pf2[K - 1];
        }
        lmax = amax / f2;
        col_star = a_star / f2;
    } else {
        for (int base = 0; base < K; base += 64) {
            const int k = base + lane;
            double col = -__builtin_inf();
            if (k < K) col = pf2[k] / f2 + gb[k] / f_hz;
            const unsigned long long hit = __ballot(col > 1.0);
            if (hit) {
                const int first = __ffsll((long long)hit) - 1;
                kstar = base + first;
                col_star = __shfl(col, first);
                if (lane < first) lmax = fmax(lmax, col);
                break;
            }
            lmax = fmax(lmax, col);
        }
    }
    const double below = (MODE == PRHF_KMODE_O) ? lmax : wave_max(lmax);
    double h;
    if (kstar == K) {
        if (!(below >= 1.0)) return false;
        h = nodes[K - 1].alt;
    } else if (kstar == 0) {
        h = nodes[0].alt;
    } else {
        const int j = kstar - 1;
        const double aj = nodes[j].alt;
        if (below == 1.0) {
            h = aj;
        } else {
            const double slope = (nodes[j + 1].alt - aj) / (col_star - below);
            h = slope * (1.0 - below) + aj;
        }
    }
    *h_out = h - kBackoff;
    return true;
}

struct BlockInfo {
    int K;
    int bad;
    int unmag;
    int uniform;
    int poly_angle;
    int n_cand;
    int nan_b;
    int nan_p;
    const double* heights;
    double a0;
    double inv_w;
    double inv_step;
};

enum { kKeepAltMin = 0,
       kKeepPf2Max = 1,
       kKeepGbMax = 2 };
template <int THREADS>
__device__ __forceinline__ const double* kept_scalars(const double* red) { return red + 10 * (THREADS / 64); }

constexpr int kHintBuckets = PRHF_HINT_BUCKETS;
constexpr int kNanRow = 0x100;
static_assert(kNanRow >= (1 << PRHF_STATUS_WORDS), "kNanRow must not be a status bit");

#ifdef PRHF_TRACE
__device__ __forceinline__ unsigned long long* trace_marks() {
    __shared__ unsigned long long marks[4];
    return marks;
}
#define PRHF_MARK(i) do { if (threadIdx.x == 0) trace_marks()[i] = wall_clock64(); } while (0)
#else
#define PRHF_MARK(i) do { } while (0)
#endif

template <int TIER, int THREADS>
__device__ __forceinline__ BlockInfo stage_profile(const double* __restrict__ den,
                                                   const double* __restrict__ bmag,
                                                   const double* __restrict__ bpsi,
                                                   const double* __restrict__ alt,
                                                   const double* __restrict__ freq, int n_freq,
                                                   int n_alt, Node* nodes, double* pf2, double* gb,
                                                   unsigned short* hint, double* red, int capacity,
                                                   bool bottomside_alt = false) {
#pragma clang fp contract(off)
    constexpr int W = THREADS / 64;
    static_assert(10 * W + 3 <= PRHF_RED_DOUBLES, "reduction scratch too small");
    const int tid = threadIdx.x, lane = tid & 63, wave = tid >> 6;
    double bv = -__builtin_inf();
    int bi = 0x7fffffff;
    double amin = __builtin_inf();
    int nan_in = 0;
    for (int i = tid; i < n_alt; i += THREADS) {
        const double v = den[i], al = alt[i];
        const double key = (v != v) ? __builtin_inf() : v;
        if (key > bv) { bv = key; bi = i; }
        amin = fmin(amin, al);
        nan_in |= (al != al && !bottomside_alt) ? 1 : 0;
    }
    double fm = __builtin_inf();
    for (int i = tid; i < n_freq; i += THREADS) fm = fmin(fm, fabs(freq[i]));
    {
        double v0, v1;
        int i0, i1;
        halves(bv, &v0, &v1);
        halves(bi, &i0, &i1);
        const bool second = v1 > v0 || (v1 == v0 && i1 < i0);
        bv = second ? v1 : v0;
        bi = second ? i1 : i0;
#define PRHF_ARGMAX_STEP(OFF) do {                                                  \
            const double ov = lane_xor<OFF>(bv);                                    \
            const int oi = lane_xor<OFF>(bi);                                       \
            if (ov > bv || (ov == bv && oi < bi)) { bv = ov; bi = oi; }             \
        } while (0)
        PRHF_ARGMAX_STEP(16); PRHF_ARGMAX_STEP(8); PRHF_ARGMAX_STEP(4); PRHF_ARGMAX_STEP(2); PRHF_ARGMAX_STEP(1);
#undef PRHF_ARGMAX_STEP
    }
    amin = wave_min(amin);
    fm = wave_min(fm);
    nan_in = __any(nan_in) ? 1 : 0;
    if (lane == 0) {
        red[wave] = bv;
        red[W + wave] = (double)bi;
        red[2 * W + wave] = amin;
        red[3 * W + wave] = fm;
        red[9 * W + wave] = (double)nan_in;
    }
    __syncthreads();
    bv = red[0];
    bi = (int)red[W];
    amin = red[2 * W];
    fm = red[3 * W];
    nan_in = (int)red[9 * W];
#pragma unroll
    for (int w = 1; w < W; ++w) {
        const double ov = red[w];
        const int oi = (int)red[W + w];
        if (ov > bv || (ov == bv && oi < bi)) { bv = ov; bi = oi; }
        amin = fmin(amin, red[2 * W + w]);
        fm = fmin(fm, red[3 * W + w]);
        nan_in |= (int)red[9 * W + w];
    }
    PRHF_MARK(0);
    BlockInfo info;
    info.K = uniform((bi == 0x7fffffff) ? 0 : bi);
    red[10 * W + kKeepAltMin] = amin;
    fm = uniform(fm);
    info.bad = 0;
    info.unmag = 0;
    info.uniform = 0;
    info.poly_angle = 0;
    info.n_cand = -1;
    info.a0 = 0.0;
    info.inv_w = 0.0;
    info.inv_step = 0.0;
    const int K = info.K;
    info.nan_b = 0;
    info.nan_p = 0;
    if (uniform(nan_in)) {
        info.bad = kNanRow;
        info.K = 0;
        return info;
    }
    if (K == 0) {
        info.bad = PRHF_STATUS_PEAK0;
        return info;
    }
    if (K >= capacity) {
        info.bad = PRHF_STATUS_BADINDEX;
        info.K = 0;
        return info;
    }
    const double step0 = (K > 1) ? alt[1] - alt[0] : 1.0;
    double bmax = 0.0, pmax = 0.0;
    int neg = 0, ragged = 0, trig = 0, cubic = 0, quadratic = 0, steep = 0;
    for (int k = tid; k <= K; k += THREADS) {
        Node nd;
        if (k == K) {
            nd.alt = __builtin_inf();
            nd.den = nd.sden = nd.b = nd.sb = nd.u0 = nd.u1 = nd.u2 = nd.u3 = nd.off = nd.psi = nd.spsi = 0.0;
            nodes[k] = nd;
            continue;
        }
        const double a = alt[k], d = den[k], b = bmag[k], p = bpsi[k];
        nd.alt = a; nd.den = d; nd.b = b; nd.off = 0.0;
        double spsi = 0.0, turn = 0.0;
        if (k + 1 < K) {
            const double da = alt[k + 1] - a;
            const double dp = bpsi[k + 1] - p;
            nd.sden = (den[k + 1] - d) / da;
            nd.sb = (bmag[k + 1] - b) / da;
            spsi = dp / da;
            turn = fabs(dp) * kDegToRad;
            ragged |= (fabs(da - step0) > 1e-11 * fabs(step0)) ? 1 : 0;
        } else {
            nd.sden = 0.0; nd.sb = 0.0;
        }
        nd.psi = p;
        nd.spsi = spsi;
        nd.off = alt[0] - a;
        if (turn < kPolyAngle) {
            const double r = spsi * kDegToRad;
            double sp, cp;
            prhf_cr::sincos_table(p * kDegToRad, &sp, &cp);
            const double s2p = 2.0 * (sp * cp), c2p = (cp - sp) * (cp + sp);
            nd.u0 = sp * sp;
            nd.u1 = s2p * r;
            nd.u2 = c2p * (r * r);
            nd.u3 = (-2.0 / 3.0) * s2p * (r * r * r);
            if (turn < kQuadAngle) {
                const double L = (k + 1 < K) ? alt[k + 1] - a : 0.0;
                nd.u0 = nd.u0 + nd.u3 * (L * L * L) * (1.0 / 32.0);
                nd.u1 = nd.u1 - nd.u3 * (L * L) * (9.0 / 16.0);
                nd.u2 = nd.u2 + nd.u3 * L * 1.5;
                nd.u3 = 0.0;
                if (fabs(nd.u2) * (L * L) * 0.125 <= kLinTol) {
                    nd.u0 = nd.u0 - nd.u2 * (L * L) * 0.125;
                    nd.u1 = nd.u1 + nd.u2 * L;
                    nd.u2 = 0.0;
                } else {
                    quadratic = 1;
                }
            } else {
                cubic = 1;
            }
            nd.u0 = 2.0 - 2.0 * nd.u0; nd.u1 = -2.0 * nd.u1; nd.u2 = -2.0 * nd.u2; nd.u3 = -2.0 * nd.u3;
        } else {
            nd.u0 = nd.u1 = nd.u2 = 0.0;
            nd.u3 = qnan();
            trig = 1;
            steep |= (turn > kTrigAngle) ? 1 : 0;
        }
        steep |= (b != b || p != p || nd.sb != nd.sb || spsi != spsi) ? 1 : 0;
        nodes[k] = nd;
        const double fn = sqrt(d) * kPlasma;
        pf2[k] = fn * fn;
        gb[k] = kGyro * b;
        pmax = fmax(pmax, fn * fn);
        bmax = fmax(bmax, fabs(b));
        neg |= (d < 0.0) ? 1 : 0;
        neg |= (b != b) ? 2 : 0;
        neg |= (p != p) ? 4 : 0;
        neg |= ((k == 0 && b == b) || (k + 1 < K && b == b && bmag[k + 1] == bmag[k + 1])) ? 8 : 0;
        neg |= (bottomside_alt && a != a) ? 16 : 0;
    }
    bmax = wave_max(bmax);
    pmax = wave_max(pmax);
    neg = (__any(neg & 1) ? 1 : 0) | (__any(neg & 2) ? 2 : 0) | (__any(neg & 4) ? 4 : 0) | (__any(neg & 8) ? 8 : 0) |
          (bottomside_alt && __any(neg & 16) ? 16 : 0);
    ragged = __any(ragged) ? 1 : 0;
    trig = __any(steep) ? 5 : (__any(trig) ? 1 : (__any(cubic) ? 2 : (__any(quadratic) ? 3 : 0)));
    if (lane == 0) {
        red[4 * W + wave] = bmax;
        red[5 * W + wave] = (double)neg;
        red[6 * W + wave] = (double)trig;
        red[7 * W + wave] = (double)ragged;
        red[8 * W + wave] = pmax;
    }
    __syncthreads();
    pmax = red[8 * W];
    bmax = red[4 * W];
    neg = (int)red[5 * W];
    trig = (int)red[6 * W];
    ragged = (int)red[7 * W];
#pragma unroll
    for (int w = 1; w < W; ++w) {
        bmax = fmax(bmax, red[4 * W + w]);
        pmax = fmax(pmax, red[8 * W + w]);
        neg |= (int)red[5 * W + w];
        {
            const int o = (int)red[6 * W + w];
            trig = (trig == 5 || o == 5) ? 5
                 : ((trig == 1 || o == 1) ? 1 : ((trig == 2 || o == 2) ? 2 : ((trig == 3 || o == 3) ? 3 : 0)));
        }
        ragged |= (int)red[7 * W + w];
    }
    bmax = uniform(bmax);
    red[10 * W + kKeepPf2Max] = pmax;
    red[10 * W + kKeepGbMax] = kGyro * bmax;
    neg = uniform(neg);
    trig = uniform(trig);
    ragged = uniform(ragged);
    if (neg & 1) info.bad = PRHF_STATUS_NEGDEN;
    info.nan_b = (neg & 2) ? 1 : 0;
    info.nan_p = (neg & 4) ? 1 : 0;
    if (bottomside_alt && (neg & 16) && !info.bad) {
        info.bad = kNanRow;
        return info;
    }
    info.unmag = ((neg & 8) && (kGyro * bmax) / (fm * 1e6) < kUnmagTol) ? 1 : 0;
    info.poly_angle = trig == 5 ? 0 : (trig == 1 ? 4 : (trig == 2 ? 1 : (trig == 3 ? 2 : 3)));
    if (info.poly_angle == 4) {
        for (int k = tid; k < K; k += THREADS) {
            double sp, cp;
            prhf_cr::sincos_table(nodes[k].psi * kDegToRad, &sp, &cp);
            nodes[k].u0 = (cp - sp) * (cp + sp);
            nodes[k].u1 = 2.0 * (nodes[k].spsi * kDegToRad);
            nodes[k].u2 = 2.0 * (sp * cp);
            nodes[k].u3 = qnan();
        }
        __syncthreads();
    }
    const double a0 = uniform(nodes[0].alt);
    const double span = uniform(nodes[K - 1].alt) - a0;
    info.a0 = a0;
    info.uniform = (!ragged && K > 1 && step0 > 0.0) ? 1 : 0;
    info.inv_step = info.uniform ? 1.0 / step0 : 0.0;
    info.inv_w = (span > 0.0) ? (double)kHintBuckets / span : 0.0;
    if (!info.uniform) {
        const double w = span / (double)kHintBuckets;
        for (int b = tid; b < kHintBuckets; b += THREADS) {
            const double t = a0 + (double)b * w;
            int lo = 0, hi = K - 1;
            while (lo < hi) {
                const int mid = (lo + hi + 1) >> 1;
                if (nodes[mid].alt <= t) lo = mid; else hi = mid - 1;
            }
            hint[b] = (unsigned short)lo;
        }
        __syncthreads();
    }
    return info;
}

__device__ __forceinline__ int guess_segment(const unsigned short* __restrict__ hint, const BlockInfo& info,
                                             double z) {
    int j;
    if (info.uniform) {
        j = (int)((z - info.a0) * info.inv_step);
        j = j < 0 ? 0 : (j > info.K - 1 ? info.K - 1 : j);
    } else {
        int bucket = (int)((z - info.a0) * info.inv_w);
        bucket = bucket < 0 ? 0 : (bucket > kHintBuckets - 1 ? kHintBuckets - 1 : bucket);
        j = hint[bucket];
    }
    return j;
}

template <int MODE, int TIER, bool UNMAG>
__device__ __forceinline__ double point_mup(const Node& nd, double dz, double f_hz, double f2, double cX,
                                            double cY2, bool poly_angle, double well_conditioned) {
    double mu, mup;
    const double sden_ = dz == 0.0 ? 0.0 : nd.sden, sb_ = dz == 0.0 ? 0.0 : nd.sb, spsi_ = dz == 0.0 ? 0.0 : nd.spsi;
    if (TIER == 0) {
#pragma clang fp contract(off)
        const double den = sden_ * dz + nd.den;
        if (!UNMAG) {
            const double Xq = den * cX;
            if (__all(1.0 - Xq > well_conditioned)) {
#pragma clang fp contract(fast)
                const double b = sb_ * dz + nd.b;
                index_fast<MODE>(Xq, (b * b) * cY2, sin_sq_deg(spsi_ * dz + nd.psi), &mu, &mup);
                return mup;
            }
        }
        const double fn = sqrt(den) * kPlasma;
        const double X = (fn * fn) / f2;
        if (UNMAG) {
            index_unmagnetised(X, &mu, &mup);
        } else {
            const double b = sb_ * dz + nd.b;
            const double psi = spsi_ * dz + nd.psi;
            const double Y = (kGyro * b) / f_hz;
            index_faithful<MODE>(X, Y, psi, &mu, &mup);
        }
    } else {
#pragma clang fp contract(fast)
        const double den = sden_ * dz + nd.den;
        const double X = den * cX;
        if (UNMAG) {
            index_unmagnetised(X, &mu, &mup);
        } else {
            const double b = sb_ * dz + nd.b;
            const double Y2 = (b * b) * cY2;
            double S2;
            if (poly_angle || nd.u3 == nd.u3) {
                S2 = 1.0 - 0.5 * (nd.u0 + dz * (nd.u1 + dz * (nd.u2 + dz * nd.u3)));
            } else {
                S2 = sin_sq_deg(spsi_ * dz + nd.psi);
            }
            index_fast<MODE>(X, Y2, S2, &mu, &mup);
        }
    }
    return mup;
}

template <int MODE, bool THIRD>
__device__ __forceinline__ double group_index_lean(double den, double hY2, double C2, double cX, double* a_out) {
#pragma clang fp contract(fast)
    constexpr double sgn = (MODE == PRHF_KMODE_O) ? 1.0 : -1.0;
    const double a = __builtin_fma(-cX, den, 1.0);
    const double YL2 = hY2 * C2;
    const double h = __builtin_fma(-0.5, YL2, hY2);
    const double t = a * YL2;
    const double ta = t * a;
    const double alpha = __builtin_fma(h, h, ta);
    const double rbeta = rsqrt_tier<THIRD>(alpha);
    const double G = __builtin_fma(sgn * alpha, rbeta, -h);
    const double D = a + G;
    const double N = __builtin_fma(a, a, G);
    const double w = rsqrt_tier<THIRD>(N * D);
    const double DmX = __builtin_fma(-cX, den, D);
    const double v = __builtin_fma(-0.5, ta, t);
// ... 1120 lines not shown
                acc = 0.0;
                first = uniform(i0);
#ifdef PRHF_MARK_FALLBACK
                acc = 1e6;
#endif
            } else {
                acc = r.acc;
                first = uniform(r.first) & ((1 << kPanelStateShift) - 1);
            }
            panel_state = uniform(r.first) >> kPanelStateShift;
        }
    }
    const int n_iter = uniform((i1 - first + 63) >> 6);
    int i = i1 - (n_iter << 6) + lane;
    auto grid = [&](int idx) { return mult[idx < first ? first : (idx < last ? idx : last)]; };
    double m0 = 0.0, m1 = 0.0;
    if (n_iter > 0) {
        m0 = grid(i);
        m1 = grid(i + 1);
    }
    for (int it = 0; it < n_iter; ++it) {
        const int inext = i + 64;
        const double n0 = grid(inext);
        const double n1 = grid(inext + 1);
        const bool active = i >= first;
        double z, dh;
        if (TIER == 0) {
#pragma clang fp contract(off)
            z = m0 * span + a0;
            dh = (i < last) ? (m1 * span + a0) - z : kBackoff;
        } else {
            z = __builtin_fma(m0, span, a0);
            dh = (i < last) ? (m1 - m0) * span : kBackoff;
        }
        int j = guess_segment(hint, info, z);
        Node nd = nodes[j];
        const double an = nodes[j + 1].alt;
        if (__builtin_expect(__any((j > 0 && z < nd.alt) || z >= an), 0)) {
            while (j > 0 && z < nodes[j].alt) --j;
            while (j + 1 < K && z >= nodes[j + 1].alt) ++j;
            nd = nodes[j];
        }
        double dz;
        if (TIER == 0) {
            dz = z - nd.alt;
            if (dz < 0.0) dz = 0.0;
        } else {
            dz = fmax(__builtin_fma(m0, span, nd.off), 0.0);
        }
        const double mup = point_mup<MODE, TIER, UNMAG>(nd, dz, f_hz, f2, cX, cY2, poly_angle, well_conditioned);
        const double term = mup * dh;
        if (active && term == term) acc = acc + term;
        i = inext;
        m0 = n0;
        m1 = n1;
    }
    return wave_sum(acc);
}

template <int THREADS>
__device__ __forceinline__ void prefix_max_in_place(double* v, int K, double* red) {
    constexpr int W = THREADS / 64;
    const int tid = threadIdx.x, lane = tid & 63, wave = tid >> 6;
    const int per = (K + THREADS - 1) / THREADS;
    const int base = tid * per;
    double mine = -__builtin_inf();
    for (int i = 0; i < per; ++i)
        if (base + i < K) mine = fmax(mine, v[base + i]);
    const double inc = wave_scan_max(mine);
    double before = wave_shift_up_1(inc, -__builtin_inf());
    if (lane == 63) red[wave] = inc;
    __syncthreads();
#pragma unroll
    for (int w = 0; w < W; ++w)
        if (w < wave) before = fmax(before, red[w]);
    for (int i = 0; i < per; ++i)
        if (base + i < K) {
            before = fmax(before, v[base + i]);
            v[base + i] = before;
        }
    __syncthreads();
}

template <int THREADS>
__device__ __forceinline__ int list_candidates(const KArgs& a, const SegDev& sg, const double* keep,
                                               long long pair_base, unsigned short* cand, int* cand_count,
                                               const Node* nodes, const double* pf2, const double* gb, int K,
                                               double* heights) {
    constexpr int W = THREADS / 64;
    const int tid = threadIdx.x, lane = tid & 63, wave = tid >> 6;
    const int F = (int)a.n_freq;
    const double pmax = keep[kKeepPf2Max], gmax = keep[kKeepGbMax];
    int total = 0;
    for (int base = 0; base < F; base += THREADS) {
        const int f = base + tid;
        bool may = false;
        double h = 0.0;
        if (f < F) {
            const double* row = a.ftab + 8 * (long long)f;
            if (heights && sg.mode == PRHF_KMODE_X) {
#pragma clang fp contract(off)
                const double f_hz = row[0], f2 = row[1], rf2 = row[4], rf = row[5];
                int ks = K, kb = -1, nb = 0;
                double m1 = -__builtin_inf(), m2 = -__builtin_inf();
                bool exact = false;
                const int K_scan = (pmax * rf2 + gmax * rf < 1.0 - 1e-9) ? 0 : K;
                constexpr int U = 8;
                int k = 0;
                for (; k + U <= K_scan; k += U) {
                    double c[U];
#pragma unroll
                    for (int i = 0; i < U; ++i) c[i] = __builtin_fma(pf2[k + i], rf2, gb[k + i] * rf);
                    const double g = fmax(fmax(fmax(c[0], c[1]), fmax(c[2], c[3])), fmax(fmax(c[4], c[5]), fmax(c[6], c[7])));
                    if (g > 1.0 - 1e-13) break;
                    const double t = fmin(m1, g);
                    if (g > m1) { kb = k; nb = U; }
                    m1 = fmax(m1, g);
                    m2 = fmax(m2, t);
                }
                for (; k < K_scan; ++k) {
                    const double c = __builtin_fma(pf2[k], rf2, gb[k] * rf);
                    if (__builtin_fabs(c - 1.0) <= 1e-13) { exact = true; break; }
                    if (c > 1.0) { ks = k; break; }
                    if (c > m1) { m2 = m1; m1 = c; kb = k; nb = 1; }
                    else if (c > m2) m2 = c;
                }
                if (!exact && kb >= 0 && !(m1 - m2 > 1e-14 * __builtin_fabs(m1))) exact = true;
                double below = -__builtin_inf(), col_star = 0.0;
                if (K_scan == 0) {
                    ks = K;
                } else if (exact) {
                    ks = K;
                    for (int kk = 0; kk < K; ++kk) {
                        const double col = pf2[kk] / f2 + gb[kk] / f_hz;
                        if (col > 1.0) { ks = kk; col_star = col; break; }
                        below = fmax(below, col);
                    }
                } else {
                    for (int i = 0; i < nb; ++i) {
                        const double c = __builtin_fma(pf2[kb + i], rf2, gb[kb + i] * rf);
                        if (c >= m1 - 4e-15 * __builtin_fabs(m1)) below = fmax(below, pf2[kb + i] / f2 + gb[kb + i] / f_hz);
                    }
                    if (ks < K) col_star = pf2[ks] / f2 + gb[ks] / f_hz;
                }
                if (ks == K) {
                    may = below >= 1.0;
                    h = nodes[K - 1].alt;
                } else if (ks == 0) {
                    may = true;
                    h = nodes[0].alt;
                } else {
                    may = true;
                    const double aj = nodes[ks - 1].alt;
                    if (below == 1.0) {
                        h = aj;
                    } else {
                        const double slope = (nodes[ks].alt - aj) / (col_star - below);
                        h = slope * (1.0 - below) + aj;
                    }
                }
                h = h - kBackoff;
            } else if (heights) {
#pragma clang fp contract(off)
                const double f2 = row[1];
                const double ulp_half = f2 * 0x1p-53;
                int lo = 0, hi = K;
                while (lo < hi) {
                    const int mid = (lo + hi) >> 1;
                    if ((pf2[mid] - f2) > ulp_half) hi = mid; else lo = mid + 1;
                }
                const int kstar = lo;
                const double below = (kstar > 0 ? pf2[kstar - 1] : -__builtin_inf()) / f2;
                if (kstar == K) {
                    may = below >= 1.0;
                    h = nodes[K - 1].alt;
                } else if (kstar == 0) {
                    may = true;
                    h = nodes[0].alt;
                } else {
                    may = true;
                    const double aj = nodes[kstar - 1].alt;
                    if (below == 1.0) {
                        h = aj;
                    } else {
                        const double col_star = pf2[kstar] / f2;
                        const double slope = (nodes[kstar].alt - aj) / (col_star - below);
                        h = slope * (1.0 - below) + aj;
                    }
                }
                h = h - kBackoff;
            } else {
                double ub = pmax * row[4];
                if (sg.mode == PRHF_KMODE_X) ub = ub + gmax * row[5];
                may = !(ub < 1.0 - 1e-9);
            }
            if (!may) a.out[sg.out_off + pair_base + f] = qnan();
        }
        const unsigned long long mask = __ballot(may);
        if (lane == 0) cand_count[wave] = __popcll(mask);
        __syncthreads();
        int at = total, chunk = 0;
#pragma unroll
        for (int w = 0; w < W; ++w) {
            const int n = cand_count[w];
            if (w < wave) at += n;
            chunk += n;
        }
        if (may) {
            const int pos = at + __popcll(mask & ((1ull << lane) - 1ull));
            cand[pos] = (unsigned short)f;
            if (heights) heights[pos] = h;
        }
        __syncthreads();
        total += chunk;
    }
    return uniform(total);
}

struct PairFreq {
    double f_hz, f2, cX, cY2, inv_f2, inv_f;
};
__device__ __forceinline__ PairFreq pair_freq(const KArgs& a, int f) {
#pragma clang fp contract(off)
    PairFreq p;
    if (a.ftab) {
        const double* row = a.ftab + 8 * (long long)f;
        p.f_hz = uniform(row[0]); p.f2 = uniform(row[1]); p.cX = uniform(row[2]); p.cY2 = uniform(row[3]);
        p.inv_f2 = uniform(row[4]); p.inv_f = uniform(row[5]);
    } else {
        const double fm = a.freq[f];
        p.f_hz = uniform((fm > 0.0 && fm < __builtin_inf()) ? fm * 1e6 : qnan());
        p.f2 = uniform(p.f_hz * p.f_hz);
        p.cX = uniform((kPlasma * kPlasma) / p.f2);
        const double cY = kGyro / p.f_hz;
        p.cY2 = uniform(cY * cY);
        p.inv_f2 = uniform(1.0 / p.f2);
        p.inv_f = uniform(1.0 / p.f_hz);
    }
    return p;
}

template <int MODE>
__device__ __forceinline__ bool pair_reflects(const Node* nodes, const double* pf2, const double* gb,
                                              const BlockInfo& info, const double* keep, const PairFreq& pf,
                                              int lane, int list_pos, double* h_out) {
    if (info.heights) {
        *h_out = uniform(info.heights[list_pos]);
        return true;
    }
    if (info.K > 1 && info.n_cand < 0) {
        double ub = keep[kKeepPf2Max] * pf.inv_f2;
        if (MODE == PRHF_KMODE_X) ub = ub + keep[kKeepGbMax] * pf.inv_f;
        if (uniform((int)(ub < 1.0 - 1e-9))) return false;
    }
    double h = 0.0;
    const bool r = uniform((int)reflection_height<MODE>(nodes, pf2, gb, info.K, pf.f_hz, pf.f2, lane, &h)) != 0;
    *h_out = uniform(h);
    return r;
}

template <int MODE, int TIER>
__device__ __forceinline__ double one_level_term(const Node* nodes, const BlockInfo& info, const PairFreq& pf,
                                                 double well_conditioned) {
    const bool poly = info.poly_angle != 0 && info.poly_angle != 4;
    const double mup = info.unmag
        ? point_mup<MODE, TIER, true>(nodes[0], 0.0, pf.f_hz, pf.f2, pf.cX, pf.cY2, poly, well_conditioned)
        : point_mup<MODE, TIER, false>(nodes[0], 0.0, pf.f_hz, pf.f2, pf.cX, pf.cY2, poly, well_conditioned);
    const double term = mup * kBackoff;
    return (term == term) ? term : 0.0;
}

template <int MODE, int TIER>
__device__ __forceinline__ bool collapsed_grid_sum(const Node* nodes, const BlockInfo& info, const PairFreq& pf,
                                                   const double* __restrict__ mult, int n_points, double h_refl,
                                                   double well_conditioned, double* sum_out) {
#pragma clang fp contract(off)
    const double span = h_refl - info.a0;
    const double z_first = mult[0] * span + info.a0;
    const double z_last = mult[n_points - 1] * span + info.a0;
    const double S = (z_last - z_first) + kBackoff;
    if (!(__builtin_fabs(S) > 1e-21)) return false;
    const bool poly = info.poly_angle != 0 && info.poly_angle != 4;
    const double mup = info.unmag
        ? point_mup<MODE, TIER, true>(nodes[0], 0.0, pf.f_hz, pf.f2, pf.cX, pf.cY2, poly, well_conditioned)
        : point_mup<MODE, TIER, false>(nodes[0], 0.0, pf.f_hz, pf.f2, pf.cX, pf.cY2, poly, well_conditioned);
    const double term = mup * S;
    *sum_out = (term == term) ? term : 0.0;
    return true;
}

struct PlanRoom {
    unsigned base0, base1, base2;
    int cap0, cap01;
    int total;
};
__device__ __forceinline__ unsigned plan_slot(const PlanRoom& r, int i) {
    return i < r.cap0 ? r.base0 + (unsigned)i * (unsigned)kPlanBytes
                      : (i < r.cap01 ? r.base1 + (unsigned)(i - r.cap0) * (unsigned)kPlanBytes
                                     : r.base2 + (unsigned)(i - r.cap01) * (unsigned)kPlanBytes);
}

__device__ __attribute__((noinline)) bool plan_pair(const Node* nodes, int K, const double2* __restrict__ pairs, int n_points,
                                                    double span, double kj, double cX, double cY2, bool grade,
                                                    unsigned* rec) {
    const int i_last = n_points - 1;
    const double n1 = (double)i_last;
    const int j_top = (int)(pairs[i_last].x * kj);
    if (j_top < 0 || j_top > K - 1) return false;
    int search_hi = i_last + 1, run_end = i_last & ~63;
    auto find = [&](int j, int* lo_out) {
        if (j < 0) return 2;
        const double m_star = (double)j / kj;
        const int base = stretch_guess(m_star, n1);
        if (!(base >= 0 && base + 3 < search_hi)) return 0;
        const unsigned hit4 = (pairs[base].x >= m_star ? 1u : 0u) | (pairs[base + 1].x >= m_star ? 2u : 0u) |
                              (pairs[base + 2].x >= m_star ? 4u : 0u) | (pairs[base + 3].x >= m_star ? 8u : 0u);
        if (!(hit4 != 0u && (hit4 & 1u) == 0u)) return 0;
        const int lo = base + __ffs((int)hit4) - 1;
        if (((lo + 63) & ~63) + 128 > run_end) return 2;
        *lo_out = lo;
        search_hi = lo + 1;
        run_end = lo & ~63;
        return 1;
    };
    int lo0 = 0, lo1 = 0, lo2 = 0, n_seg = 0;
    const int f0 = find(j_top, &lo0);
    if (f0 == 0) return false;
    if (f0 == 1) {
        n_seg = 1;
        const int f1 = find(j_top - 1, &lo1);
        if (f1 == 0) return false;
        if (f1 == 1) {
            n_seg = 2;
            const int f2 = find(j_top - 2, &lo2);
            if (f2 == 0) return false;
            if (f2 == 1) n_seg = 3;
        }
    }
    const double hcY2 = 0.5 * cY2;
    const double cYs = hcY2 * rsqrt_cubic(hcY2);
    auto span_of = [&](int j, int lo, int q_s) {
        const Node& nd = nodes[j];
        const SegLinear lin = seg_linear(nd.off, nd.den, nd.sden, nd.b, nd.sb, span, cYs);
        const StridedZones sp = strided_zones(lo, q_s, (lo + 63) & ~63, lin, cX, n1, grade);
        const unsigned zz = (unsigned)(sp.z2_s >> 6) | ((unsigned)(sp.z1_s >> 6) << 10);
        return ((unsigned long long)zz << 32) | ((unsigned)(sp.a_s >> 6) | ((unsigned)(sp.e_s >> 6) << 10));
    };
    const unsigned long long s0 = n_seg > 0 ? span_of(j_top, lo0, i_last - 1) : 0ull;
    const unsigned long long s1 = n_seg > 1 ? span_of(j_top - 1, lo1, lo0 - 1) : 0ull;
    const unsigned long long s2 = n_seg > 2 ? span_of(j_top - 2, lo2, lo1 - 1) : 0ull;
    const unsigned ae0 = (unsigned)s0, ae1 = (unsigned)s1, ae2 = (unsigned)s2;
    const unsigned zz0 = (unsigned)(s0 >> 32), zz1 = (unsigned)(s1 >> 32), zz2 = (unsigned)(s2 >> 32);
    rec[0] = (unsigned)lo0 | ((unsigned)lo1 << 16);
    rec[1] = (unsigned)lo2 | ((unsigned)j_top << 16);
    rec[2] = ae0 | ((ae1 & 1023u) << 20) | ((unsigned)n_seg << 30);
    rec[3] = (ae1 >> 10) | (ae2 << 10) | kPlanValid;
    rec[4] = zz0 | ((zz1 & 1023u) << 20);
    rec[5] = (zz1 >> 10) | (zz2 << 10);
    return true;
}

template <int TIER, int THREADS, bool G>
__device__ __forceinline__ PlanRoom plan_pairs(const KArgs& a, const SegDev& sg, const Node* nodes, double* pf2, double* gb,
                                               unsigned short* hint, const unsigned short* cand, const BlockInfo& info,
                                               int block_in_prof, int blocks_per_prof, unsigned* plan_cnt) {
    constexpr int W = THREADS / 64;
    PlanRoom room;
    room.base0 = room.base1 = room.base2 = 0u;
    room.cap0 = room.cap01 = room.total = 0;
    if (TIER != 1 || G) return room;
    const bool shape_ok = sg.pair_plan && sg.mode == PRHF_KMODE_X && sg.lean && a.pairs && sg.sp_off > 0 && sg.chunks == 1 &&
                          sg.n_points >= PRHF_TOP3_MIN_POINTS && sg.n_points < 65536 && info.heights && info.n_cand > 0 &&
                          info.uniform && !info.unmag && info.poly_angle >= 1 && info.poly_angle <= 3;
    if (!shape_ok) return room;
    const double2* pairs = reinterpret_cast<const double2*>(a.pairs) + sg.mult_off;
    if (reinterpret_cast<const unsigned*>(pairs + (sg.sp_off - sg.mult_off))[0] != 0u) return room;
    typedef __attribute__((address_space(3))) const double* LdsDouble;
    typedef __attribute__((address_space(3))) const unsigned short* LdsU16;
    const int levels = (int)a.lds_levels;
    const int used = (info.n_cand + 1) & ~1;
    room.base0 = (unsigned)(uintptr_t)(LdsDouble)gb;
    room.base1 = (unsigned)(uintptr_t)(LdsU16)hint;
    room.base2 = (unsigned)(uintptr_t)(LdsDouble)(pf2 + used);
    room.cap0 = levels * 8 / kPlanBytes;
    room.cap01 = room.cap0 + kHintBuckets * 2 / kPlanBytes;
    room.total = room.cap01 + max(levels - used, 0) * 8 / kPlanBytes;
    if (a.plan_cap > 0) room.total = min(room.total, a.plan_cap);
    const int first_item = block_in_prof * W, round_items = blocks_per_prof * W;
    int n_planned = 0, n_self = 0;
    for (int u = threadIdx.x;; u += THREADS) {
        const int t = (u / W) * round_items + first_item + (u % W);
        if (t >= info.n_cand) break;
        const double span = info.heights[t] - info.a0;
        const double kj = span * info.inv_step;
        const bool main_loop = span > 0.0 && kj <= (double)(info.K - 1);
        bool done = false;
        if (u < room.total) {
            constexpr int kWords = kPlanBytes / 4;
            unsigned* rec = u < room.cap0 ? reinterpret_cast<unsigned*>(gb) + kWords * u
                                          : (u < room.cap01 ? reinterpret_cast<unsigned*>(hint) + kWords * (u - room.cap0)
                                                            : reinterpret_cast<unsigned*>(pf2 + used) + kWords * (u - room.cap01));
            if (main_loop) {
                const double* row = a.ftab + 8 * (long long)cand[t];
                done = plan_pair(nodes, info.K, pairs, sg.n_points, span, kj, row[2], row[3], sg.strided_grade != 0, rec);
            }
            if (!done) rec[3] = 0u;
        }
        if (main_loop) {
            if (done) ++n_planned; else ++n_self;
        }
    }
    if (n_planned) atomicAdd(&plan_cnt[0], (unsigned)n_planned);
    if (n_self) atomicAdd(&plan_cnt[1], (unsigned)n_self);
    __syncthreads();
    if (threadIdx.x == 0 && a.plan_counters) {
        if (plan_cnt[0]) atomicAdd(&a.plan_counters[0], (unsigned long long)plan_cnt[0]);
        if (plan_cnt[1]) atomicAdd(&a.plan_counters[1], (unsigned long long)plan_cnt[1]);
    }
    room.base0 = (unsigned)uniform((int)room.base0);
    room.base1 = (unsigned)uniform((int)room.base1);
    room.base2 = (unsigned)uniform((int)room.base2);
    room.cap0 = uniform(room.cap0);
    room.cap01 = uniform(room.cap01);
    room.total = uniform(room.total);
    return room;
}

template <int MODE, int TIER, int THREADS, bool G>
__device__ __forceinline__ void run_items(const KArgs& a, const SegDev& sg, const Node* nodes,
                                          const double* pf2, const double* gb, const unsigned short* hint,
                                          const unsigned short* cand, const BlockInfo& info, long long prof_local,
                                          int block_in_prof, int blocks_per_prof, int* item_next, double* red,
                                          const PlanRoom& room) {
    constexpr int W = THREADS / 64;
    const int lane = threadIdx.x & 63;
    const double* keep = kept_scalars<THREADS>(red);
    const double wc = uniform(sg.well_conditioned);
    const int F = uniform((int)a.n_freq);
    const int C = uniform(sg.chunks);
    const int T = info.n_cand >= 0 ? info.n_cand : F * C;
    const double* mult = a.mult + sg.mult_off;
    const double2* pairs = (a.pairs && sg.lean) ? reinterpret_cast<const double2*>(a.pairs) + sg.mult_off : nullptr;
    const int sp_off = (pairs && sg.sp_off > 0)
                           ? uniform((int)(sg.sp_off - sg.mult_off) | (sg.strided_lower ? kStridedLowerBit : 0) |
                                     (sg.strided_lower && sg.panel_lower ? kPanelLowerBit : 0) |
                                     (sg.strided_lower && sg.panel_lower && sg.panel_nodes == 4 ? kPanelNodes4Bit : 0) |
                                     (!G && sg.strided_lower && sg.panel_lower && sg.panel_upper ? kPanelUpperBit : 0) |
                                     (sg.strided_grade ? kStridedGradeBit : 0)) : 0;
    const long long pair_base = prof_local * F;
    const int first_item = block_in_prof * W, round_items = blocks_per_prof * W;
    static_assert(11 * W + 8 <= PRHF_RED_DOUBLES, "reduction scratch too small");
    const int S = uniform(sg.slots), wave = threadIdx.x >> 6;
    const bool local = S > 0;
    double* part = red + 10 * W + 8;
    if (local && lane == 0) part[wave] = 0.0;
    int pulled = 0;
    int panel_cnt = 0;
    auto next_item = [&]() {
        const int u = uniform(atomicAdd(item_next, 1)) >> 6;
        pulled = u;
        return uniform((u / W) * round_items + first_item + (u % W));
    };
    int t = local ? uniform(block_in_prof * W + wave) : next_item();
    const int t_end = local ? uniform(min(F * S, t + 1)) : T;
    for (; t < t_end; t = local ? t_end : next_item()) {
        int f = t, c = 0;
        if (local) {
            f = t / S;
            c = t % S;
            if (c >= C) break;
        } else if (info.n_cand >= 0) {
            f = uniform((int)cand[t]);
        } else if (C > 1) {
            f = t % F;
            c = t / F;
        }
        double result = qnan();
        bool reflects = false;
        int panel = 0;
        const unsigned plan_lds = pulled < room.total ? plan_slot(room, pulled) : 0u;
        if (!info.bad) {
            const PairFreq pf = pair_freq(a, f);
            double h = 0.0;
            reflects = pair_reflects<MODE>(nodes, pf2, gb, info, keep, pf, lane, t, &h);
            double collapsed = 0.0;
            if (reflects && info.K > 1 && h < info.a0 &&
                uniform((int)collapsed_grid_sum<MODE, TIER>(nodes, info, pf, mult, sg.n_points, h, sg.well_conditioned,
                                                            &collapsed))) {
                result = (c == C - 1) ? uniform(collapsed) : 0.0;
            } else if (reflects) {
                const int i0 = c * sg.chunk_len;
                const int i1 = min(sg.n_points, i0 + sg.chunk_len);
                if (info.unmag)
                    result = integrate_chunk<MODE, TIER, true, G>(nodes, hint, info, mult, pairs, sg.n_points, i0, i1,
                                                               pf.f_hz, pf.f2, pf.cX, pf.cY2, h, lane, wc, sp_off, plan_lds, panel);
                else
                    result = integrate_chunk<MODE, TIER, false, G>(nodes, hint, info, mult, pairs, sg.n_points, i0,
                                                                i1, pf.f_hz, pf.f2, pf.cX, pf.cY2, h, lane, wc, sp_off, plan_lds, panel);
            } else if (info.K == 1) {
                result = (c == C - 1) ? one_level_term<MODE, TIER>(nodes, info, pf, sg.well_conditioned) : 0.0;
                reflects = true;
            }
        }
        if constexpr (MODE == PRHF_KMODE_X && TIER == 1 && !G) {
            panel_cnt += panel == 2 ? 0x10000 : (panel != 0 ? 1 : 0);
            if (panel == 4 && lane == 0 && a.plan_counters) atomicAdd(&a.plan_counters[5], 1ull);
        }
        if (lane == 0) {
            if (local) {
                part[wave] = reflects ? result : qnan();
            } else if (C == 1) {
                const double vh = (reflects && result != 0.0) ? result + keep[kKeepAltMin] : qnan();
                a.out[sg.out_off + pair_base + f] = vh;
            } else {
                a.partial[sg.partial_off + (pair_base + f) * C + c] = reflects ? result : qnan();
            }
        }
    }
    if constexpr (MODE == PRHF_KMODE_X && TIER == 1 && !G) {
        if (lane == 0 && a.plan_counters) {
            if (panel_cnt & 0xffff) atomicAdd(&a.plan_counters[2], (unsigned long long)(panel_cnt & 0xffff));
            if (panel_cnt >> 16) atomicAdd(&a.plan_counters[3], (unsigned long long)(panel_cnt >> 16));
            if (sg.panel_upper && (panel_cnt & 0xffff)) atomicAdd(&a.plan_counters[4], (unsigned long long)(panel_cnt & 0xffff));
        }
    }
    if (local) {
        __syncthreads();
        const int item = block_in_prof * W + wave;
        const int f = item / S;
        if (f < F && item % S == 0 && lane == 0) {
            double sum = 0.0;
            for (int cc = 0; cc < C; ++cc) sum = sum + part[wave + cc];
            a.out[sg.out_off + pair_base + f] = (sum == sum && sum != 0.0) ? sum + keep[kKeepAltMin] : qnan();
        }
    }
}

}

template <int TIER, int THREADS, bool G>
__device__ __forceinline__ unsigned long long run_block(const KArgs& a, const SegDev& sg, Node* nodes, double* pf2, double* gb,
                                          unsigned short* hint, unsigned short* cand, int* cand_count, double* red,
                                          long long prof_local, int block_in_prof, int blocks_per_prof,
                                          int* item_next, unsigned* plan_cnt) {
    const long long p = sg.prof_begin + prof_local;
    BlockInfo info = stage_profile<TIER, THREADS>(
        a.den + p * a.prof_stride, a.bmag + p * a.field_stride, a.bpsi + p * a.field_stride,
        a.alt + p * a.alt_stride, a.freq, (int)a.n_freq, (int)a.n_alt, nodes, pf2, gb, hint, red, (int)a.lds_levels);
    PRHF_MARK(1);
    if (sg.mode == PRHF_KMODE_X && info.nan_b && !info.bad) info.bad = kNanRow;
    if (sg.mode == PRHF_KMODE_O && !info.bad) prefix_max_in_place<THREADS>(pf2, info.K, red);
    PRHF_MARK(2);
    info.n_cand = -1;
    info.heights = nullptr;
    if (a.ftab && !a.no_candidates && sg.chunks == 1 && a.n_freq <= PRHF_MAX_CAND && !info.bad && info.K > 1)
    {
        double* heights = nullptr;
        if (a.n_freq <= a.lds_levels) {
            if (sg.mode == PRHF_KMODE_O) heights = gb;
            else if (a.n_freq <= THREADS && sg.thread_scan) heights = pf2;
        }
        info.n_cand = list_candidates<THREADS>(a, sg, kept_scalars<THREADS>(red), prof_local * a.n_freq, cand,
                                               cand_count, nodes, pf2, gb, info.K, heights);
        info.heights = heights;
    }
#ifdef PRHF_TRACE
    const unsigned long long t_staged = wall_clock64();
#else
    const unsigned long long t_staged = 0;
#endif
    if (threadIdx.x == 0 && block_in_prof == 0) {
        if (info.bad) post_status(a.status, (unsigned)info.bad);
        if (sg.chunks > 1 && sg.slots == 0) a.altmin[sg.altmin_off + prof_local] = kept_scalars<THREADS>(red)[kKeepAltMin];
    }
    const PlanRoom room = plan_pairs<TIER, THREADS, G>(a, sg, nodes, pf2, gb, hint, cand, info, block_in_prof, blocks_per_prof,
                                                       plan_cnt);
    if (sg.mode == PRHF_KMODE_O)
        run_items<PRHF_KMODE_O, TIER, THREADS, G>(a, sg, nodes, pf2, gb, hint, cand, info, prof_local, block_in_prof,
                                               blocks_per_prof, item_next, red, room);
    else
        run_items<PRHF_KMODE_X, TIER, THREADS, G>(a, sg, nodes, pf2, gb, hint, cand, info, prof_local, block_in_prof,
                                               blocks_per_prof, item_next, red, room);
    return t_staged;
}

template <int TIER_SEL, int THREADS, bool TALL>
__device__ __forceinline__ void vfo_kernel_body(const KArgs& a) {
    extern __shared__ __attribute__((aligned(16))) unsigned char smem[];
    const int n_alt = (int)a.lds_levels;
    Node* nodes;
    double* pf2;
    unsigned short* hint;
    if (TALL) {
        unsigned char* slab = a.tall + (size_t)blockIdx.x * a.tall_stride;
        nodes = reinterpret_cast<Node*>(slab);
        pf2 = reinterpret_cast<double*>(slab + (size_t)(n_alt + 1) * sizeof(Node));
        hint = reinterpret_cast<unsigned short*>(smem);
    } else {
        nodes = reinterpret_cast<Node*>(smem);
        pf2 = reinterpret_cast<double*>(smem + (size_t)(n_alt + 1) * sizeof(Node));
        hint = reinterpret_cast<unsigned short*>(pf2 + 2 * (size_t)n_alt);
    }
    double* gb = pf2 + n_alt;
    unsigned short* cand = hint + kHintBuckets;
    double* red = reinterpret_cast<double*>(cand + PRHF_MAX_CAND);

    __shared__ long long next_bid;
    __shared__ int item_next;
    __shared__ int cand_count[PRHF_BLOCK_THREADS / 64 + 1];
    __shared__ unsigned plan_cnt[2];
    const unsigned* list = a.block_list;
    const long long n_blocks = list ? (long long)list[0] : a.n_blocks;
    if (a.zero_after && blockIdx.x == 0 && threadIdx.x < PRHF_ORDER_CLASSES) a.zero_after[threadIdx.x] = 0u;
    long long ticket = blockIdx.x;
    if (ticket >= n_blocks) return;
    long long bid = list ? (long long)list[1 + ticket] : ticket;
    for (;;) {
        if (threadIdx.x == 0) {
            item_next = 0;
            plan_cnt[0] = plan_cnt[1] = 0u;
        }
#ifdef PRHF_TRACE
        const unsigned long long t_start = wall_clock64();
#endif
        int s = 0;
        while (s + 1 < a.n_segs && bid >= a.seg[s + 1].block_begin) ++s;
        const SegDev& sg = a.seg[s];
        long long lb = bid - sg.block_begin;
        const long long head_blocks = sg.tail_prof * sg.blocks_per_prof;
        int bpp = sg.blocks_per_prof;
        long long prof0 = 0;
        if (lb >= head_blocks) {
            lb -= head_blocks;
            bpp = sg.tail_bpp;
            prof0 = sg.tail_prof;
        }
        const long long prof_local = prof0 + lb / bpp;
        const int block_in_prof = (int)(lb % bpp);
        int prio = sg.prio;
        if (a.n_segs == 1 && a.queue != nullptr) {
            const long long left = n_blocks - ticket, round = gridDim.x;
            prio = left > 3 * round ? 3 : (left > 2 * round ? 2 : (left > round ? 1 : 0));
        }
        if (a.n_segs > 1 || a.queue != nullptr) {
            if (prio >= 3) __builtin_amdgcn_s_setprio(3);
            else if (prio == 2) __builtin_amdgcn_s_setprio(2);
            else if (prio == 1) __builtin_amdgcn_s_setprio(1);
            else __builtin_amdgcn_s_setprio(0);
        }

        const unsigned long long t_staged = (TIER_SEL == 0 || (TIER_SEL == 2 && sg.tier == 0))
            ? run_block<0, THREADS, TALL>(a, sg, nodes, pf2, gb, hint, cand, cand_count, red, prof_local, block_in_prof, bpp,
                                    &item_next, plan_cnt)
            : run_block<1, THREADS, TALL>(a, sg, nodes, pf2, gb, hint, cand, cand_count, red, prof_local, block_in_prof, bpp,
                                    &item_next, plan_cnt);
        (void)t_staged;
#ifdef PRHF_TRACE
        if (a.trace && (threadIdx.x & 63) == 0) {
            unsigned long long* t = a.trace + (bid * (THREADS / 64) + (threadIdx.x >> 6)) * 6;
            t[0] = t_start;
            t[1] = wall_clock64();
            t[2] = t_staged;
            t[3] = trace_marks()[0];
            t[4] = trace_marks()[1];
            t[5] = trace_marks()[2];
        }
#endif
        if (a.queue == nullptr) break;
        __syncthreads();
        if (threadIdx.x == 0) next_bid = (long long)gridDim.x + atomicAdd(a.queue, 1u);
        __syncthreads();
        ticket = uniform((int)next_bid);
        if (ticket >= n_blocks) break;
        bid = list ? (long long)list[1 + ticket] : ticket;
    }
}

template <int TIER_SEL, int THREADS>
__global__ __launch_bounds__(THREADS, PRHF_MIN_WAVES_PER_SIMD) void vfo_kernel(const KArgs a) {
    vfo_kernel_body<TIER_SEL, THREADS, false>(a);
}
template <int THREADS>
__global__ __launch_bounds__(THREADS, PRHF_MIN_WAVES_PER_SIMD) void vfo_tall_kernel(const KArgs a) {
    vfo_kernel_body<2, THREADS, true>(a);
}

__global__ void grid_pairs_kernel(const double* __restrict__ mult, long long n, double2* __restrict__ pairs) {
    const long long i = (long long)blockIdx.x * blockDim.x + threadIdx.x;
    if (i >= n + PRHF_PAIR_PAD) return;
    if (i >= n) {
        pairs[i] = make_double2(0.0, 0.0);
        return;
    }
    const double m = mult[i];
    pairs[i] = make_double2(fmin(fmax(m, 0.0), 1.0), (i + 1 < n ? mult[i + 1] : m) - m);
}

hipError_t launch_grid_pairs(const double* mult, long long n, double* pairs, hipStream_t stream) {
    if (n <= 0) return hipSuccess;
    hipLaunchKernelGGL(grid_pairs_kernel, dim3((unsigned)((n + PRHF_PAIR_PAD + 255) / 256)), dim3(256), 0, stream, mult,
                       n, reinterpret_cast<double2*>(pairs));
    return hipGetLastError();
}

__global__ __launch_bounds__(1024) void grid_strided_kernel(const double* __restrict__ mult, double2* __restrict__ pairs,
                                                            const StridedPieces pc) {
    const int p = blockIdx.x, tid = threadIdx.x;
    const int N = pc.n_points[p];
    const double* m = mult + pc.mult_off[p];
    double2* out = pairs + pc.sp_off[p];
    const double c0 = 1.0 / 22025.465794806718;
    const double c1 = -expm1(-10.0 / (double)(N - 1));
    int bad = 0;
    for (int i = tid; i + 1 < N; i += 1024) {
        const double mi = m[i];
        const double dev = __builtin_fabs((m[i + 1] - mi) - c1 * ((1.0 - mi) + c0));
        if (!(dev <= 1e-14)) bad = 1;
    }
    const int any_bad = __syncthreads_or(bad);
    const int cnt = (N + 7) / 8 + 1;
    for (int j = tid; j < cnt + PRHF_PAIR_PAD; j += 1024) {
        double2 e = make_double2(0.0, 0.0);
        if (j < cnt && 8 * j < N) {
            const double mm = fmin(fmax(m[8 * j], 0.0), 1.0);
            e = make_double2(mm, 8.0 * (c1 * ((1.0 - mm) + c0)));
        }
        out[1 + j] = e;
    }
    if (tid == 0) {
        double2 h;
        const bool origin = __builtin_fabs(m[0]) <= 1e-14 && __builtin_fabs(m[N - 1] - 1.0) <= 1e-14;
        const unsigned long long word = (any_bad ? 1ull : 0ull) | (origin ? 0ull : 2ull);
        __builtin_memcpy(&h.x, &word, sizeof word);
        h.y = c1;
        out[0] = h;
    }
}

hipError_t launch_grid_strided(const double* mult, double* pairs, const StridedPieces& pc, hipStream_t stream) {
    if (pc.n <= 0) return hipSuccess;
    hipLaunchKernelGGL(grid_strided_kernel, dim3((unsigned)pc.n), dim3(1024), 0, stream, mult,
                       reinterpret_cast<double2*>(pairs), pc);
    return hipGetLastError();
}

__global__ __launch_bounds__(256) void freq_table_kernel(const double* __restrict__ freq_mhz, long long n_freq,
                                                         double* __restrict__ tab, const ZeroWords zero) {
#pragma clang fp contract(off)
    const long long f = (long long)blockIdx.x * blockDim.x + threadIdx.x;
    if (f < n_freq) {
        const double fm = freq_mhz[f];
        const double f_hz = (fm > 0.0 && fm < __builtin_inf()) ? fm * 1e6 : qnan();
        const double f2 = f_hz * f_hz;
        const double cY = kGyro / f_hz;
        double* row = tab + 8 * f;
        row[0] = f_hz; row[1] = f2; row[2] = (kPlasma * kPlasma) / f2; row[3] = cY * cY;
        row[4] = 1.0 / f2; row[5] = 1.0 / f_hz; row[6] = 0.0; row[7] = 0.0;
    }
    if (blockIdx.x != 0) return;
    for (int k = 0; k < zero.n; ++k)
        for (int i = threadIdx.x; i < zero.words[k]; i += blockDim.x) zero.p[k][i] = 0u;
    __shared__ double part[4];
    __shared__ double part_max[4];
    double fm = __builtin_inf(), fx = 0.0;
    for (long long i = threadIdx.x; i < n_freq; i += blockDim.x) {
        const double v = fabs(freq_mhz[i]);
        fm = fmin(fm, v);
// ... 357 lines not shown
    const long long row = (long long)blockIdx.x * (blockDim.x >> 6) + (threadIdx.x >> 6);
    if (row >= n_prof) return;
    const double* v = vh_model + row * n_freq;
    double sum = 0.0, cnt = 0.0;
    for (int f = lane; f < n_freq; f += 64) {
        const double a = fabs(v[f]);
        if (a == a) { sum += a; cnt += 1.0; }
    }
    sum = wave_sum(sum);
    cnt = wave_sum(cnt);
    const double mean = (cnt > 0.0) ? sum / cnt : qnan();
    const double fill = (mean == mean) ? fmax(mean, 100.0) : qnan();
    double c = 0.0;
    for (int f = lane; f < n_freq; f += 64) {
        double m = v[f];
        if (!(m == m)) m = fill;
        const double r = vh_obs[f] - m;
        if (residual) residual[row * n_freq + f] = r;
        c += r * r;
    }
    c = wave_sum(c);
    if (lane == 0 && cost) cost[row] = c;
}

hipError_t launch_residual(const double* vh_model, const double* vh_obs, long long n_prof, int n_freq,
                           double* residual, double* cost, hipStream_t stream) {
    if (n_prof <= 0) return hipSuccess;
    hipLaunchKernelGGL(residual_kernel, dim3((unsigned)((n_prof + 3) / 4)), dim3(256), 0, stream, vh_model, vh_obs,
                       n_prof, n_freq, residual, cost);
    return hipGetLastError();
}

#include "prhf_residual_many.inc"
#include "prhf_short.inc"

static const void* short_kernel_for(int threads, int lanes) {
    if (threads == PRHF_COMPACT_THREADS)
        return lanes == 8 ? reinterpret_cast<const void*>(&vfo_short_kernel<PRHF_COMPACT_THREADS, 8>)
                          : reinterpret_cast<const void*>(&vfo_short_kernel<PRHF_COMPACT_THREADS, 16>);
    if (threads == PRHF_SHORT_THREADS)
        return lanes == 8 ? reinterpret_cast<const void*>(&vfo_short_kernel<PRHF_SHORT_THREADS, 8>)
                          : reinterpret_cast<const void*>(&vfo_short_kernel<PRHF_SHORT_THREADS, 16>);
    return nullptr;
}

hipError_t launch_vfo_short(const KArgs& a, long long grid_blocks, size_t lds_bytes, int threads, int lanes, hipStream_t stream) {
    if (grid_blocks <= 0 || a.n_blocks <= 0) return hipSuccess;
    const void* kernel = short_kernel_for(threads, lanes);
    if (!kernel || (lanes != 8 && lanes != 16)) return hipErrorInvalidValue;
    void* params[] = {const_cast<KArgs*>(&a)};
    return hipLaunchKernel(kernel, dim3((unsigned)grid_blocks), dim3((unsigned)threads), params, lds_bytes, stream);
}

hipError_t launch_short_order(const KArgs& a, unsigned* order, const double* freq_mhz, double* tab, const ZeroWords& zero,
                              hipStream_t stream) {
    if (a.n_blocks <= 0) return hipErrorInvalidValue;
    hipLaunchKernelGGL(short_order_kernel, dim3((unsigned)((a.n_blocks + 63) / 64)), dim3(1024), 0, stream, a, order, freq_mhz,
                       tab, zero);
    return hipGetLastError();
}

hipError_t launch_vfo_shortx(const KArgs& a, long long grid_blocks, size_t lds_bytes, int threads, hipStream_t stream) {
    if (grid_blocks <= 0 || a.n_blocks <= 0) return hipSuccess;
    if (threads == PRHF_COMPACT_THREADS)
        hipLaunchKernelGGL((vfo_shortx_kernel<PRHF_COMPACT_THREADS>), dim3((unsigned)grid_blocks), dim3(PRHF_COMPACT_THREADS),
                           lds_bytes, stream, a);
    else if (threads == PRHF_SHORT_THREADS)
        hipLaunchKernelGGL((vfo_shortx_kernel<PRHF_SHORT_THREADS>), dim3((unsigned)grid_blocks), dim3(PRHF_SHORT_THREADS),
                           lds_bytes, stream, a);
    else
        return hipErrorInvalidValue;
    return hipGetLastError();
}

#include "prhf_snell.inc"
#include "prhf_homing.inc"
#include "prhf_skip.inc"
#include "prhf_gradient.inc"
#include "prhf_gradient_homing.inc"
#include "prhf_gradient_hops.inc"
#include "prhf_gradient_skip.inc"
#include "prhf_vjp.inc"

hipError_t query_occupancy(int tier, size_t lds_bytes, int* blocks_per_cu) {
    constexpr int THREADS = PRHF_BLOCK_THREADS;
    if (tier == 0)
        return hipOccupancyMaxActiveBlocksPerMultiprocessor(blocks_per_cu, vfo_kernel<0, THREADS>, THREADS, lds_bytes);
    if (tier == 1)
        return hipOccupancyMaxActiveBlocksPerMultiprocessor(blocks_per_cu, vfo_kernel<1, THREADS>, THREADS, lds_bytes);
    return hipOccupancyMaxActiveBlocksPerMultiprocessor(blocks_per_cu, vfo_kernel<2, THREADS>, THREADS, lds_bytes);
}

hipError_t configure_kernels(size_t max_lds_bytes) {
    constexpr int THREADS = PRHF_BLOCK_THREADS;
    const void* kernels[] = {reinterpret_cast<const void*>(&vfo_kernel<0, THREADS>),
                             reinterpret_cast<const void*>(&vfo_kernel<1, THREADS>),
                             reinterpret_cast<const void*>(&vfo_kernel<2, THREADS>),
                             short_kernel_for(PRHF_SHORT_THREADS, 16), short_kernel_for(PRHF_SHORT_THREADS, 8),
                             short_kernel_for(PRHF_COMPACT_THREADS, 16), short_kernel_for(PRHF_COMPACT_THREADS, 8),
                             reinterpret_cast<const void*>(&vfo_shortx_kernel<PRHF_SHORT_THREADS>),
                             reinterpret_cast<const void*>(&vfo_shortx_kernel<PRHF_COMPACT_THREADS>),
                             reinterpret_cast<const void*>(&regrid_kernel<512>)};
    for (const void* k : kernels) {
        hipError_t e = hipFuncSetAttribute(k, hipFuncAttributeMaxDynamicSharedMemorySize, (int)max_lds_bytes);
        if (e != hipSuccess) return e;
    }
    return hipSuccess;
}

}
```

### pyrayhf_amd/csrc/prhf_plan.h

```cpp

#ifndef PRHF_PLAN_H
#define PRHF_PLAN_H

#include <algorithm>
#include <cmath>
#include <cstdint>
#include <cstdio>
#include <cstring>

#include "prhf.h"
#include "prhf_kernels.h"

namespace {

struct Knobs {
    double target_waves = 4096;
    double lean_min_points = 65;
    double well_conditioned = 1e-5;
    double thread_scan_min = 0.0;
    double no_candidates = 0;
    double persistent = 1;
    double tail_rounds = 1.0;
    double tail_bpp = 4;
    double split_min_points = 1024;
    double split_few_profiles = 1;
    double short_kernel = 1;
    double shortx_kernel = 1;
    double short_concurrent = 1;
    double short_queue = 0;
    double direct_upload = 1;
    double timing = 0;
    double trim_lds = 1;
    double short_compact = 1;
    double short_prio = 4;
    double short_order = 1;
    double short_lanes = 0;
    double host_slabs = 3;
    double local_chunks = 1;
    double tall_lean = 1;
    double snell_table = 4;
    double strided_top = 1;
    double strided_lower = 1;
    double panel_lower = 1;
    double panel_nodes = 4;
    double panel_upper = 1;
    double strided_grade = 1;
    double pair_plan = 1;
    double pair_plan_cap = 0;
};
struct KnobName {
    const char* name;
    double Knobs::*field;
    double lo, hi;
};
const KnobName kKnobNames[] = {
    {"target_waves", &Knobs::target_waves, 64, 1e9},
    {"lean_min_points", &Knobs::lean_min_points, 2, 1e9},
    {"well_conditioned", &Knobs::well_conditioned, 0, 1},
    {"thread_scan_min", &Knobs::thread_scan_min, 0, 1e300},
    {"no_candidates", &Knobs::no_candidates, 0, 1},
    {"persistent", &Knobs::persistent, 0, 1},
    {"tail_rounds", &Knobs::tail_rounds, 0, 1e6},
    {"tail_bpp", &Knobs::tail_bpp, 1, 64},
    {"split_min_points", &Knobs::split_min_points, 1, 1e9},
    {"split_few_profiles", &Knobs::split_few_profiles, 0, 1},
    {"short_kernel", &Knobs::short_kernel, 0, 1},
    {"shortx_kernel", &Knobs::shortx_kernel, 0, 1},
    {"short_concurrent", &Knobs::short_concurrent, 0, 1},
    {"short_queue", &Knobs::short_queue, 0, PRHF_SHORT_MAX_QUEUE},
    {"local_chunks", &Knobs::local_chunks, 0, 1},
    {"direct_upload", &Knobs::direct_upload, 0, 1},
    {"timing", &Knobs::timing, 0, 1},
    {"trim_lds", &Knobs::trim_lds, 0, 1},
    {"short_compact", &Knobs::short_compact, 0, 1},
    {"short_prio", &Knobs::short_prio, 0, 7},
    {"host_slabs", &Knobs::host_slabs, 1, 3},
    {"short_order", &Knobs::short_order, 0, 1},
    {"short_lanes", &Knobs::short_lanes, 0, 16},
    {"snell_table", &Knobs::snell_table, 0, 1e9},
    {"tall_lean", &Knobs::tall_lean, 0, 1},
    {"strided_top", &Knobs::strided_top, 0, 1},
    {"strided_lower", &Knobs::strided_lower, 0, 1},
    {"panel_lower", &Knobs::panel_lower, 0, 1},
    {"panel_nodes", &Knobs::panel_nodes, 4, 8},
    {"panel_upper", &Knobs::panel_upper, 0, 1},
    {"strided_grade", &Knobs::strided_grade, 0, 1},
    {"pair_plan", &Knobs::pair_plan, 0, 1},
    {"pair_plan_cap", &Knobs::pair_plan_cap, 0, 1024},
};
constexpr int kWavesPerBlock = PRHF_BLOCK_THREADS / 64;

inline void plan_slice(prhf::SegDev& s, long long n_freq, long long wg_slots, const Knobs& kn) {
    const long long kTargetWaves = (long long)kn.target_waves;
    const bool kSplitFewProfiles = kn.split_few_profiles != 0;
    const long long kSplitMinPoints = (long long)kn.split_min_points;
    const double kTailRounds = kn.tail_rounds;
    const int kTailBpp = (int)kn.tail_bpp;
    const long long P = s.prof_end - s.prof_begin;
    const long long pairs = P * n_freq;
    const long long N = s.n_points;
    long long chunks = 1, chunk_len = ((N + 63) / 64) * 64;
    if (pairs > 0 && pairs < kTargetWaves && N > 256) {
        long long want = std::min((kTargetWaves + pairs - 1) / pairs, (N + 255) / 256);
        chunk_len = (((N + want - 1) / want + 63) / 64) * 64;
        chunks = (N + chunk_len - 1) / chunk_len;
    }
    s.slots = 0;
    if (chunks > 1 && kn.local_chunks != 0) {
        long long want = std::min<long long>(std::min((kTargetWaves + pairs - 1) / pairs, (N + 255) / 256), kWavesPerBlock);
        long long S = 1;
        while (S * 2 <= want) S *= 2;
        if (S > 1) {
            chunk_len = (((N + S - 1) / S + 63) / 64) * 64;
            chunks = (N + chunk_len - 1) / chunk_len;
            s.slots = (int)S;
        }
    }
    s.chunks = (int)chunks;
    s.chunk_len = (int)chunk_len;
    if (s.slots > 0) {
        s.blocks_per_prof = (int)((n_freq * s.slots + kWavesPerBlock - 1) / kWavesPerBlock);
        s.tail_prof = P;
        s.tail_bpp = s.blocks_per_prof;
        return;
    }
    const long long items = n_freq * chunks;
    long long waves = std::max<long long>(1, std::min(items, (kTargetWaves + std::max<long long>(P, 1) - 1) /
                                                                 std::max<long long>(P, 1)));
    s.blocks_per_prof = (int)((waves + kWavesPerBlock - 1) / kWavesPerBlock);
    if (kSplitFewProfiles && chunks == 1 && N >= kSplitMinPoints && P > 0 && P * s.blocks_per_prof < 4 * wg_slots) {
        long long bpp = std::min<long long>(32, (4 * wg_slots + P - 1) / P);
        while (bpp > 1 && items < bpp * kWavesPerBlock * 2) --bpp;
        if (bpp > s.blocks_per_prof) s.blocks_per_prof = (int)bpp;
    }
    s.tail_prof = P;
    s.tail_bpp = s.blocks_per_prof;
    const long long tail = (long long)(kTailRounds * (double)wg_slots);
    if (kTailBpp > 1 && s.blocks_per_prof == 1 && chunks == 1 && N >= 1024 && P >= 4 * tail && tail > 0 &&
        n_freq >= (long long)kTailBpp * kWavesPerBlock) {
        s.tail_prof = P - tail;
        s.tail_bpp = kTailBpp;
    }
}

inline bool slice_plans_pairs(const prhf::SegDev& s, bool tall, long long n_freq, long long lds_levels, const Knobs& kn) {
    return kn.pair_plan != 0 && !tall && s.sp_off > 0 && s.chunks == 1 && s.slots == 0 && s.lean != 0 && s.tier == 1 &&
           s.mode == PRHF_KMODE_X && s.thread_scan != 0 && kn.no_candidates == 0 && n_freq <= PRHF_BLOCK_THREADS &&
           n_freq <= lds_levels && s.n_points >= PRHF_TOP3_MIN_POINTS && s.n_points < 65536;
}

inline long long first_decreasing_grid_entry(const double* mult, int64_t mult_len, const prhf_segment* segs, int32_t n_segs) {
    for (int32_t g = 0; g < n_segs; ++g)
        if (segs[g].mult_offset >= 0 && segs[g].n_points >= 1 && segs[g].mult_offset + segs[g].n_points <= mult_len)
            for (int64_t i = segs[g].mult_offset + 1; i < segs[g].mult_offset + segs[g].n_points; ++i)
                if (mult[i] < mult[i - 1]) return (long long)i;
    return -1;
}

inline int validate_work_list(const prhf_segment* segs, int32_t n_segs, int64_t n_prof, int64_t n_freq, int64_t mult_len,
                              char* msg, size_t msg_len) {
    for (int i = 0; i < n_segs; ++i) {
        const prhf_segment& u = segs[i];
        if (u.prof_begin < 0 || u.prof_end < u.prof_begin || u.prof_end > n_prof) {
            std::snprintf(msg, msg_len, "segment %d: profile range outside [0, n_prof]", i);
            return PRHF_EINVAL;
        }
        if (u.mode != PRHF_MODE_O && u.mode != PRHF_MODE_X) {
            std::snprintf(msg, msg_len, "mode must be 'O' or 'X'");
            return PRHF_EINVAL;
        }
        if (u.n_points < 1) {
// ... 28 lines not shown
    kWordShortX = 4,
    kWordShortXFollow = 5,
    kLaunchQueueWords = 6,
    kWordRayQueue = 6,
    kWordPeak = 7,
    kWordShortXFull = 8,
    kStatusWords = 12,
};

#ifndef PRHF_COMPACT_RESERVE
#define PRHF_COMPACT_RESERVE 512
#endif
constexpr size_t kLdsPerCu = 160 * 1024;
constexpr size_t kShortReserve = 512;
constexpr size_t kLdsHalf = kLdsPerCu / 2 - kShortReserve, kLdsFull = kLdsPerCu - kShortReserve;
constexpr size_t kLdsQuarter = kLdsPerCu / PRHF_COMPACT_WGS_PER_CU - PRHF_COMPACT_RESERVE;

inline size_t staged_lds_bytes(long long levels) { return prhf::lds_bytes_for(levels); }

inline long long resident_slots(int cu_count, size_t lds_bytes, size_t reserve) {
    return (long long)cu_count * (lds_bytes + reserve <= kLdsPerCu / 2 ? 2 : 1);
}

template <class LdsOf>
inline long long compact_levels_for(long long lds_levels, LdsOf lds_of) {
    long long L = lds_levels;
    while (L > 1 && lds_of(L) > kLdsQuarter) --L;
    return (2 * L >= lds_levels && L >= 8 && lds_of(L) <= kLdsQuarter) ? L : 0;
}

struct LaunchShape {
    long long n_prof, n_freq, n_alt;
    long long lds_levels;
    bool tall;
    long long mult_len;
    int cu_count;
    int math;
};

struct ShortLaunch {
    long long lds_levels;
    int threads;
    int queue_entries;
    int short_queue;
    size_t lds_bytes;
    long long slots;
    long long grid;
    bool queue;
};

struct ShortKind {
    int n_segs;
    long long blocks;
    ShortLaunch first;
    bool second;
    ShortLaunch full;
    int lanes;
    long long follow_grid;
    size_t list_bytes;
    prhf::SegDev seg[PRHF_MAX_SEGMENTS];
};

struct LaunchPlan {
    int n_segs;
    bool tall;
    int launch_tier;
    long long blocks;
    long long wg_slots;
    long long grid;
    bool queue;
    size_t lds_bytes;
    int no_candidates;
    long long partial_elems, altmin_elems;
    long long out_rows;
    unsigned long long tall_stride;
    long long tall_slabs;
    bool want_pairs;
    long long table_entries;
    bool any_plan;
    bool freq_table;
    bool short_order;
    bool zero_queues;
    bool forked;
    prhf::StridedPieces pieces;
    prhf::SegDev seg[PRHF_MAX_SEGMENTS];
    ShortKind o, x;
};

inline ShortLaunch size_short_launch(bool xmode, bool compact, long long levels, int queue_entries, bool from_list,
                                     long long blocks, const LaunchShape& sh, const Knobs& kn) {
    ShortLaunch l;
    l.lds_levels = levels;
    l.threads = compact ? PRHF_COMPACT_THREADS : PRHF_SHORT_THREADS;
    l.queue_entries = xmode ? 0 : queue_entries;
    const int fixed = (int)kn.short_queue;
    l.short_queue = fixed > 0 && !xmode ? -std::min(fixed, queue_entries) : l.queue_entries;
    l.lds_bytes = xmode ? prhf::shortx_lds_bytes(levels, sh.n_freq)
                        : prhf::short_lds_fixed(levels, sh.n_freq, l.threads) + 8 * (size_t)queue_entries;
    l.slots = compact ? (long long)sh.cu_count * PRHF_COMPACT_WGS_PER_CU : resident_slots(sh.cu_count, l.lds_bytes, kShortReserve);
    l.queue = from_list || blocks > l.slots;
    l.grid = std::min(blocks, l.slots);
    return l;
}

inline void plan_short_kind(ShortKind& k, bool xmode, int full_queue, long long wg_slots, const LaunchShape& sh, const Knobs& kn) {
    k.blocks = 0;
    for (int i = 0; i < k.n_segs; ++i) {
        k.seg[i].block_begin = k.blocks;
        k.blocks += k.seg[i].prof_end - k.seg[i].prof_begin;
    }
    k.second = false;
    k.lanes = 0;
    k.follow_grid = std::min(k.blocks, wg_slots);
    k.list_bytes = (size_t)(k.blocks + 1) * sizeof(unsigned);
    k.first = k.full = ShortLaunch();
    if (k.blocks == 0) return;
    long long compact = 0;
    int compact_queue = 0;
    if (kn.short_compact != 0) {
        if (xmode) {
            compact = compact_levels_for(sh.lds_levels, [&](long long L) { return prhf::shortx_lds_bytes(L, sh.n_freq); });
        } else {
            compact = compact_levels_for(sh.lds_levels, [&](long long L) {
                return prhf::short_lds_fixed(L, sh.n_freq, PRHF_COMPACT_THREADS) + 8 * PRHF_COMPACT_MIN_QUEUE;
            });
            if (compact) compact_queue = prhf::short_queue_entries(compact, sh.n_freq, kLdsQuarter, PRHF_COMPACT_THREADS);
        }
    }
    k.first = size_short_launch(xmode, compact > 0, compact ? compact : sh.lds_levels, compact ? compact_queue : full_queue,
                                false, k.blocks, sh, kn);
    k.second = compact > 0 && compact < sh.lds_levels;
    if (k.second) k.full = size_short_launch(xmode, false, sh.lds_levels, full_queue, true, k.blocks, sh, kn);
    if (!xmode) {
        int longest = 0;
        for (int i = 0; i < k.n_segs; ++i) longest = std::max(longest, k.seg[i].n_points);
        k.lanes = kn.short_lanes == 0 ? (longest <= 256 ? 8 : 16) : (kn.short_lanes < 12 ? 8 : 16);
    }
}

inline int plan_launch(const LaunchShape& sh, const prhf_segment* segs, int32_t n_user_segs, const Knobs& kn, LaunchPlan& pl,
                       char* msg, size_t msg_len) {
    const long long n_freq = sh.n_freq, n_prof = sh.n_prof, lds_levels = sh.lds_levels;
    const bool tall = sh.tall;
    const int kLeanMinPoints = (int)kn.lean_min_points;
    const bool kNoCandidates = kn.no_candidates != 0, kPersistent = kn.persistent != 0;
    if (validate_work_list(segs, n_user_segs, n_prof, n_freq, sh.mult_len, msg, msg_len) != PRHF_OK) return PRHF_EINVAL;
    pl.tall = tall;
    pl.lds_bytes = tall ? prhf::lds_bytes_tall() : staged_lds_bytes(lds_levels);
    pl.wg_slots = resident_slots(sh.cu_count, pl.lds_bytes, 0);
    const size_t short_budget = prhf::short_queue_entries(lds_levels, n_freq, kLdsHalf, PRHF_SHORT_THREADS) ? kLdsHalf : kLdsFull;
    const int full_queue = prhf::short_queue_entries(lds_levels, n_freq, short_budget, PRHF_SHORT_THREADS);

    pl.n_segs = pl.o.n_segs = pl.x.n_segs = 0;
    pl.want_pairs = false;
    pl.out_rows = 0;
    for (int i = 0; i < n_user_segs; ++i) {
        const prhf_segment& u = segs[i];
        prhf::SegDev s;
        std::memset(&s, 0, sizeof s);
        s.prof_begin = u.prof_begin;
        s.prof_end = u.prof_end;
        s.mult_off = u.mult_offset;
        s.out_off = u.out_offset;
        s.mode = u.mode == PRHF_MODE_O ? PRHF_KMODE_O : PRHF_KMODE_X;
        s.n_points = u.n_points;
        s.tier = sh.math == PRHF_MATH_AUTO ? (u.mode == PRHF_MODE_O ? 0 : 1) : (sh.math == PRHF_MATH_FAST ? 1 : 0);
// ... 10 lines not shown
                                n_prof * n_freq >= 4096 && !kNoCandidates;
        const bool is_short = kn.short_kernel != 0 && fits_short && s.tier == 0 && s.well_conditioned < 1.0 &&
                              s.n_points <= PRHF_SHORT_MAX_POINTS && full_queue > 0;
        const bool is_shortx = kn.shortx_kernel != 0 && fits_short && s.tier == 1 && s.mode == PRHF_KMODE_X &&
                               s.n_points <= PRHF_SHORTX_MAX_POINTS && s.thread_scan &&
                               prhf::shortx_lds_bytes(lds_levels, n_freq) <= kLdsFull;
        if (is_short || is_shortx) {
            ShortKind& k = is_short ? pl.o : pl.x;
            prhf::SegDev& t = k.seg[k.n_segs++];
            t = s;
            t.lean = 1;
            t.blocks_per_prof = 1;
            t.tail_prof = t.prof_end - t.prof_begin;
            t.tail_bpp = 1;
            pl.want_pairs = true;
        } else {
            pl.want_pairs = pl.want_pairs || s.lean != 0;
            pl.seg[pl.n_segs++] = s;
        }
    }
    pl.launch_tier = 0;
    for (int i = 0; i < pl.n_segs; ++i) pl.launch_tier = (i == 0 || pl.launch_tier == pl.seg[i].tier) ? pl.seg[i].tier : 2;
    auto cost = [](const prhf::SegDev& s) {
        const double per_point = s.tier == 1 ? 1.0 : (s.well_conditioned < 1.0 ? 1.8 : 3.5);
        return (double)s.n_points / s.chunks / s.blocks_per_prof * per_point;
    };
    for (int i = 1; i < pl.n_segs; ++i)
        for (int k = i; k > 0 && cost(pl.seg[k]) > cost(pl.seg[k - 1]); --k) std::swap(pl.seg[k], pl.seg[k - 1]);
    pl.blocks = pl.partial_elems = pl.altmin_elems = 0;
    for (int i = 0; i < pl.n_segs; ++i) {
        prhf::SegDev& s = pl.seg[i];
        const long long P = s.prof_end - s.prof_begin;
        s.prio = std::max(0, 3 - i);
        s.block_begin = pl.blocks;
        pl.blocks += s.tail_prof * s.blocks_per_prof + (P - s.tail_prof) * s.tail_bpp;
        if (s.chunks > 1 && s.slots == 0) {
            s.partial_off = pl.partial_elems;
            s.altmin_off = pl.altmin_elems;
            pl.partial_elems += P * n_freq * s.chunks;
            pl.altmin_elems += P;
        }
    }
    pl.queue = (kPersistent || tall) && pl.blocks > pl.wg_slots;
    pl.grid = pl.queue ? pl.wg_slots : pl.blocks;
    pl.no_candidates = kNoCandidates || tall;
    pl.tall_stride = tall && pl.blocks > 0 ? prhf::tall_slab_bytes(sh.n_alt) : 0;
    pl.tall_slabs = tall ? std::min(pl.blocks, pl.wg_slots) : 0;
    plan_short_kind(pl.x, true, full_queue, pl.wg_slots, sh, kn);
    plan_short_kind(pl.o, false, full_queue, pl.wg_slots, sh, kn);
    if (pl.blocks > 0x7fffffffLL || pl.o.blocks > 0x7fffffffLL || pl.x.blocks > 0x7fffffffLL) {
        std::snprintf(msg, msg_len, "launch too large");
        return PRHF_EINVAL;
    }

    std::memset(&pl.pieces, 0, sizeof pl.pieces);
    pl.table_entries = sh.mult_len + PRHF_PAIR_PAD;
    pl.any_plan = false;
    if (pl.want_pairs && kn.strided_top != 0 && !tall) {
        prhf::StridedPieces& pieces = pl.pieces;
        for (int i = 0; i < pl.n_segs; ++i) {
            prhf::SegDev& s = pl.seg[i];
            if (!(s.lean && s.tier == 1 && s.mode == PRHF_KMODE_X && s.chunks == 1 && s.n_points >= PRHF_TOP3_MIN_POINTS)) continue;
            int p = 0;
            while (p < pieces.n && !(pieces.mult_off[p] == s.mult_off && pieces.n_points[p] == s.n_points)) ++p;
            if (p == pieces.n) {
                const long long len = prhf::strided_piece_entries(s.n_points);
                if ((pl.table_entries + len) * 16 >= 0x7fffffffLL) continue;
                pieces.mult_off[p] = s.mult_off;
                pieces.n_points[p] = s.n_points;
                pieces.sp_off[p] = pl.table_entries;
                pl.table_entries += len;
                ++pieces.n;
            }
            s.sp_off = pieces.sp_off[p];
            s.strided_lower = kn.strided_lower != 0;
            s.panel_lower = s.strided_lower && kn.panel_lower != 0;
            s.panel_nodes = s.panel_lower && kn.panel_nodes == 4 ? 4 : 8;
            s.panel_upper = s.panel_lower && kn.panel_upper != 0;
            s.strided_grade = kn.strided_grade != 0;
            s.pair_plan = slice_plans_pairs(s, tall, n_freq, lds_levels, kn) ? 1 : 0;
            pl.any_plan = pl.any_plan || s.pair_plan != 0;
        }
    }
    pl.freq_table = pl.want_pairs && (n_prof * n_freq >= 4096 || pl.any_plan);
    pl.short_order = pl.freq_table && pl.o.blocks > 0 && kn.short_order != 0 && pl.o.blocks >= 4 * pl.o.first.slots;
    const bool any_short = pl.o.n_segs > 0 || pl.x.n_segs > 0;
    pl.zero_queues = !pl.freq_table && (any_short || pl.queue);
    pl.forked = any_short && pl.blocks > 0 && kn.short_concurrent != 0;
    return PRHF_OK;
}

struct VjpPlan {
    long long blocks;
    int threads, waves;
    size_t lds_bytes;
};
inline long long vjp_max_levels(bool jacobian, int waves) {
    long long L = 1;
    while (prhf::vjp_lds_bytes(L + 1, waves, jacobian) <= kLdsFull) ++L;
    return L;
}
inline int plan_vjp(long long n_prof, long long n_freq, long long lds_levels, bool jacobian, VjpPlan& pl, char* why,
                    size_t why_len) {
    std::memset(&pl, 0, sizeof pl);
    if (n_prof < 0 || n_freq < 1 || lds_levels < 1) {
        std::snprintf(why, why_len, "bad shape");
        return PRHF_EINVAL;
    }
    int waves = PRHF_VJP_THREADS / 64;
    while (waves > 1 && (waves / 2 >= n_freq || prhf::vjp_lds_bytes(lds_levels, waves, jacobian) > kLdsFull)) waves /= 2;
    if (prhf::vjp_lds_bytes(lds_levels, waves, jacobian) > kLdsFull) {
        std::snprintf(why, why_len, "the %s stages at most %lld levels up to the density peak in LDS; this launch needs %lld "
                      "(tall bottomsides are not supported by the derivative kernels)", jacobian ? "Jacobian" : "VJP",
                      vjp_max_levels(jacobian, 1), lds_levels);
        return PRHF_EINVAL;
    }
    pl.blocks = n_prof;
    pl.threads = PRHF_VJP_THREADS;
    pl.waves = waves;
    pl.lds_bytes = prhf::vjp_lds_bytes(lds_levels, waves, jacobian);
    return PRHF_OK;
}

}

#endif
```

Measured before the change: 379.6 million.

## Add double-buffered streaming persistent kernel with per-wave profile staging

Adds a persistent streaming kernel with 1024-thread workgroups, one per CU. Each holds two LDS slots, so one profile can be staged by a single wave team while the other waves run frequency items on the previous profile. Slots are handed off through per-slot headers and a global ticket queue, and staging and candidate-listing helpers are generalised to run at wave granularity. The aim is to hide staging latency and tail imbalance behind compute. The cost is extra complexity, a stall/abort path, a doubled LDS footprint and different occupancy.

```diff
diff --git a/include/prhf.h b/include/prhf.h
--- a/include/prhf.h
+++ b/include/prhf.h
@@ -268,6 +268,8 @@
 
 int prhf_panel_upper_counters(prhf_ctx* ctx, uint64_t* counters);
 
+int prhf_stream_launches(prhf_ctx* ctx, uint64_t* count);
+
 int prhf_occupancy(prhf_ctx* ctx, int64_t n_alt, int32_t math, int32_t* workgroups_per_cu);
 
 int prhf_sync(prhf_ctx* ctx);
diff --git a/pyrayhf_amd/_native.py b/pyrayhf_amd/_native.py
--- a/pyrayhf_amd/_native.py
+++ b/pyrayhf_amd/_native.py
@@ -166,6 +166,7 @@
     "prhf_pair_plan_counters": (ctypes.c_int, [ctypes.c_void_p, ctypes.POINTER(ctypes.c_uint64)]),
     "prhf_panel_counters": (ctypes.c_int, [ctypes.c_void_p, ctypes.POINTER(ctypes.c_uint64)]),
     "prhf_panel_upper_counters": (ctypes.c_int, [ctypes.c_void_p, ctypes.POINTER(ctypes.c_uint64)]),
+    "prhf_stream_launches": (ctypes.c_int, [ctypes.c_void_p, ctypes.POINTER(ctypes.c_uint64)]),
     "prhf_occupancy": (ctypes.c_int, [ctypes.c_void_p, ctypes.c_int64, ctypes.c_int32,
                                       ctypes.POINTER(ctypes.c_int32)]),
     "prhf_sync": (ctypes.c_int, [ctypes.c_void_p]),
@@ -505,6 +506,11 @@
         raise_for(self._lib.prhf_panel_upper_counters(self._h, buf))
         return tuple(int(v) for v in buf)
 
+    def stream_launches(self):
+        n = ctypes.c_uint64(0)
+        raise_for(self._lib.prhf_stream_launches(self._h, ctypes.byref(n)))
+        return int(n.value)
+
     def occupancy(self, n_alt, math):
         n = ctypes.c_int32(0)
         raise_for(self._lib.prhf_occupancy(self._h, int(n_alt), int(math), ctypes.byref(n)))
diff --git a/pyrayhf_amd/csrc/prhf_api.cpp b/pyrayhf_amd/csrc/prhf_api.cpp
--- a/pyrayhf_amd/csrc/prhf_api.cpp
+++ b/pyrayhf_amd/csrc/prhf_api.cpp
@@ -150,6 +150,7 @@
     double* h_pack_dev = nullptr;
     unsigned long long* d_words = nullptr;
     unsigned long long* h_words = nullptr;
+    uint64_t stream_launches = 0;
     unsigned long long* d_plan_counters = nullptr;
     bool status_pending = false;
     uint64_t grad_home_counters[PRHF_GRAD_HOME_COUNTERS] = {};
@@ -188,6 +189,12 @@
     size_t cost_elems(int64_t n_prof) const { return (size_t)n_prof * (size_t)(n_iono && !ionogram_of_row ? n_iono : 1); }
 };
 
+#ifdef PRHF_TRACE
+constexpr size_t kStreamLdsMax = kLdsFull - 2048;
+#else
+constexpr size_t kStreamLdsMax = kLdsFull;
+#endif
+
 int status_to_code(unsigned bits) {
     if (bits & PRHF_STATUS_PEAK0)
         return fail(PRHF_EPEAK0, "density peak at index 0: no bottomside levels below the peak");
@@ -198,6 +205,9 @@
     if (bits & PRHF_STATUS_BADINDEX) return fail(PRHF_EINVAL, "profile_index outside [0, n_prof)");
     if (bits & PRHF_STATUS_BADFIELD) return fail(PRHF_EINVAL, "field index outside [0, n_fields)");
     if (bits & PRHF_STATUS_PATHLEN) return fail(PRHF_EINVAL, "a ray has more path nodes than path_stride");
+    if (bits & PRHF_STATUS_STALL)
+        return fail(PRHF_EHIP, "streaming launch gave up: a wave waited seconds for a slot of its own workgroup (the outputs of "
+                    "this call are incomplete; option stream_blocks = 0 takes the general kernel)");
     return PRHF_OK;
 }
 
@@ -517,7 +527,13 @@
 
 int launch_general(prhf_ctx* c, const LaunchPlan& pl, prhf::KArgs& a) {
     if (pl.queue) a.queue = c->d_status + kWordGeneral;
-    if (pl.tall) HIP_TRY(prhf::launch_vfo_tall(a, pl.grid, c->stream));
+    if (pl.stream) {
+        a.n_blocks = pl.stream_blocks;
+        a.seg[0].tail_bpp = pl.stream_tail_bpp;
+        a.seg[0].tail_prof = pl.stream_tail_prof;
+        HIP_TRY(prhf::launch_vfo_stream(a, pl.stream_grid, c->stream));
+        ++c->stream_launches;
+    } else if (pl.tall) HIP_TRY(prhf::launch_vfo_tall(a, pl.grid, c->stream));
     else HIP_TRY(prhf::launch_vfo(a, pl.grid, pl.launch_tier, pl.lds_bytes, c->stream));
     return PRHF_OK;
 }
@@ -742,7 +758,7 @@
     if ((rc = update_tables(k, pl, a)) != PRHF_OK) return rc;
 #ifdef PRHF_TRACE
     static DevBuf trace_buf;
-    const size_t trace_words = (size_t)pl.blocks * kWavesPerBlock * 6;
+    const size_t trace_words = (size_t)pl.blocks * (pl.stream ? PRHF_STREAM_THREADS / 64 : kWavesPerBlock) * 8;
     if (std::getenv("PRHF_TRACE_FILE") && pl.blocks > 0) {
         if ((rc = ensure(c, trace_buf, trace_words * 8)) != PRHF_OK) return rc;
         HIP_TRY(hipMemsetAsync(trace_buf.p, 0, trace_words * 8, c->stream));
@@ -904,7 +920,7 @@
                            hipHostMallocDefault)) != hipSuccess ||
         (e = hipMalloc(reinterpret_cast<void**>(&c->d_plan_counters), 6 * sizeof(unsigned long long))) != hipSuccess ||
         (e = hipMemset(c->d_plan_counters, 0, 6 * sizeof(unsigned long long))) != hipSuccess ||
-        (e = prhf::configure_kernels(staged_lds_bytes(kMaxAlt))) != hipSuccess) {
+        (e = prhf::configure_kernels(staged_lds_bytes(kMaxAlt), kStreamLdsMax)) != hipSuccess) {
         prhf_ctx_destroy(c);
         return fail(PRHF_EHIP, "context setup failed: %s", hipGetErrorString(e));
     }
@@ -2775,6 +2791,12 @@
     return PRHF_OK;
 }
 
+int prhf_stream_launches(prhf_ctx* c, uint64_t* count) {
+    if (!c || !count) return fail(PRHF_EINVAL, "null pointer");
+    *count = c->stream_launches;
+    return PRHF_OK;
+}
+
 int prhf_occupancy(prhf_ctx* c, int64_t n_alt, int32_t math, int32_t* workgroups_per_cu) {
     if (!c || !workgroups_per_cu) return fail(PRHF_EINVAL, "null pointer");
     if (n_alt < 1 || n_alt > kMaxAlt) return fail(PRHF_EINVAL, "n_alt out of range");
diff --git a/pyrayhf_amd/csrc/prhf_kernels.h b/pyrayhf_amd/csrc/prhf_kernels.h
--- a/pyrayhf_amd/csrc/prhf_kernels.h
+++ b/pyrayhf_amd/csrc/prhf_kernels.h
@@ -16,6 +16,7 @@
 #define PRHF_STATUS_WORDS 8
 #define PRHF_STATUS_NANINPUT 0x10
 #define PRHF_STATUS_BADGROUP 0x8
+#define PRHF_STATUS_STALL 0x80
 
 #ifndef PRHF_BLOCK_THREADS
 #define PRHF_BLOCK_THREADS 512
@@ -26,6 +27,7 @@
 #ifndef PRHF_SHORT_WAVES_PER_SIMD
 #define PRHF_SHORT_WAVES_PER_SIMD 4
 #endif
+#define PRHF_STREAM_THREADS 1024
 #define PRHF_HINT_BUCKETS 1024
 #define PRHF_MAX_CAND 1024
 #define PRHF_MAX_SEGMENTS 8
@@ -137,7 +139,7 @@
     SegDev seg[PRHF_MAX_SEGMENTS];
 };
 
-inline size_t lds_bytes_for(long long n_alt) {
+inline __host__ __device__ size_t lds_bytes_for(long long n_alt) {
     return (size_t)(n_alt + 1) * PRHF_NODE_BYTES + (size_t)n_alt * 16 + PRHF_HINT_BUCKETS * 2 + PRHF_MAX_CAND * 2 +
            PRHF_RED_DOUBLES * 8;
 }
@@ -169,7 +171,7 @@
     return (int)(q > PRHF_SHORT_MAX_QUEUE ? PRHF_SHORT_MAX_QUEUE : q);
 }
 
-hipError_t configure_kernels(size_t max_lds_bytes);
+hipError_t configure_kernels(size_t max_lds_bytes, size_t max_stream_lds_bytes);
 hipError_t query_occupancy(int tier, size_t lds_bytes, int* blocks_per_cu);
 hipError_t launch_grid_pairs(const double* mult, long long n, double* pairs, hipStream_t stream);
 struct StridedPieces {
@@ -187,6 +189,7 @@
 };
 hipError_t launch_freq_table(const double* freq_mhz, long long n_freq, double* tab, const ZeroWords& zero, hipStream_t stream);
 hipError_t launch_vfo(const KArgs& a, long long grid_blocks, int tier, size_t lds_bytes, hipStream_t stream);
+hipError_t launch_vfo_stream(const KArgs& a, long long grid_blocks, hipStream_t stream);
 hipError_t launch_vfo_tall(const KArgs& a, long long grid_blocks, hipStream_t stream);
 hipError_t launch_peak_levels(const double* den, long long n_prof, long long n_alt, long long prof_stride,
                               unsigned* max_peak, hipStream_t stream);
diff --git a/pyrayhf_amd/csrc/prhf_kernels.hip b/pyrayhf_amd/csrc/prhf_kernels.hip
--- a/pyrayhf_amd/csrc/prhf_kernels.hip
+++ b/pyrayhf_amd/csrc/prhf_kernels.hip
@@ -353,7 +353,7 @@
 
 #ifdef PRHF_TRACE
 __device__ __forceinline__ unsigned long long* trace_marks() {
-    __shared__ unsigned long long marks[4];
+    __shared__ unsigned long long marks[8 + 8 * 16];
     return marks;
 }
 #define PRHF_MARK(i) do { if (threadIdx.x == 0) trace_marks()[i] = wall_clock64(); } while (0)
@@ -361,7 +361,32 @@
 #define PRHF_MARK(i) do { } while (0)
 #endif
 
-template <int TIER, int THREADS>
+template <int TEAM, int THREADS>
+__device__ __forceinline__ int team_tid() {
+    static_assert(TEAM == THREADS || TEAM == 64, "a team is the workgroup or one wave");
+    return TEAM == THREADS ? (int)threadIdx.x : (int)(threadIdx.x & 63);
+}
+template <int TEAM, int THREADS>
+__device__ __forceinline__ void team_sync() {
+    if constexpr (TEAM == THREADS) {
+        __syncthreads();
+    } else {
+        __builtin_amdgcn_fence(__ATOMIC_ACQ_REL, "wavefront");
+        __builtin_amdgcn_wave_barrier();
+    }
+}
+template <int TEAM, int THREADS>
+__device__ __forceinline__ void team_mark(int i) {
+#ifdef PRHF_TRACE
+    if constexpr (TEAM == THREADS) {
+        if (threadIdx.x == 0) trace_marks()[i] = wall_clock64();
+    } else {
+        if ((threadIdx.x & 63) == 0) trace_marks()[8 + 8 * (threadIdx.x >> 6) + i] = wall_clock64();
+    }
+#endif
+}
+
+template <int TIER, int THREADS, int TEAM = THREADS>
 __device__ __forceinline__ BlockInfo stage_profile(const double* __restrict__ den,
                                                    const double* __restrict__ bmag,
                                                    const double* __restrict__ bpsi,
@@ -371,14 +396,15 @@
                                                    unsigned short* hint, double* red, int capacity,
                                                    bool bottomside_alt = false) {
 #pragma clang fp contract(off)
-    constexpr int W = THREADS / 64;
-    static_assert(10 * W + 3 <= PRHF_RED_DOUBLES, "reduction scratch too small");
-    const int tid = threadIdx.x, lane = tid & 63, wave = tid >> 6;
+    constexpr int W = TEAM / 64;
+    constexpr int KW = 10 * (THREADS / 64);
+    static_assert(10 * W <= KW && KW + 3 <= PRHF_RED_DOUBLES, "reduction scratch too small");
+    const int tid = team_tid<TEAM, THREADS>(), lane = tid & 63, wave = tid >> 6;
     double bv = -__builtin_inf();
     int bi = 0x7fffffff;
     double amin = __builtin_inf();
     int nan_in = 0;
-    for (int i = tid; i < n_alt; i += THREADS) {
+    for (int i = tid; i < n_alt; i += TEAM) {
         const double v = den[i], al = alt[i];
         const double key = (v != v) ? __builtin_inf() : v;
         if (key > bv) { bv = key; bi = i; }
@@ -386,7 +412,7 @@
         nan_in |= (al != al && !bottomside_alt) ? 1 : 0;
     }
     double fm = __builtin_inf();
-    for (int i = tid; i < n_freq; i += THREADS) fm = fmin(fm, fabs(freq[i]));
+    for (int i = tid; i < n_freq; i += TEAM) fm = fmin(fm, fabs(freq[i]));
     {
         double v0, v1;
         int i0, i1;
@@ -413,7 +439,7 @@
         red[3 * W + wave] = fm;
         red[9 * W + wave] = (double)nan_in;
     }
-    __syncthreads();
+    team_sync<TEAM, THREADS>();
     bv = red[0];
     bi = (int)red[W];
     amin = red[2 * W];
@@ -428,10 +454,10 @@
         fm = fmin(fm, red[3 * W + w]);
         nan_in |= (int)red[9 * W + w];
     }
-    PRHF_MARK(0);
+    team_mark<TEAM, THREADS>(0);
     BlockInfo info;
     info.K = uniform((bi == 0x7fffffff) ? 0 : bi);
-    red[10 * W + kKeepAltMin] = amin;
+    red[KW + kKeepAltMin] = amin;
     fm = uniform(fm);
     info.bad = 0;
     info.unmag = 0;
@@ -461,7 +487,7 @@
     const double step0 = (K > 1) ? alt[1] - alt[0] : 1.0;
     double bmax = 0.0, pmax = 0.0;
     int neg = 0, ragged = 0, trig = 0, cubic = 0, quadratic = 0, steep = 0;
-    for (int k = tid; k <= K; k += THREADS) {
+    for (int k = tid; k <= K; k += TEAM) {
         Node nd;
         if (k == K) {
             nd.alt = __builtin_inf();
@@ -544,7 +570,7 @@
         red[7 * W + wave] = (double)ragged;
         red[8 * W + wave] = pmax;
     }
-    __syncthreads();
+    team_sync<TEAM, THREADS>();
     pmax = red[8 * W];
     bmax = red[4 * W];
     neg = (int)red[5 * W];
@@ -563,8 +589,8 @@
         ragged |= (int)red[7 * W + w];
     }
     bmax = uniform(bmax);
-    red[10 * W + kKeepPf2Max] = pmax;
-    red[10 * W + kKeepGbMax] = kGyro * bmax;
+    red[KW + kKeepPf2Max] = pmax;
+    red[KW + kKeepGbMax] = kGyro * bmax;
     neg = uniform(neg);
     trig = uniform(trig);
     ragged = uniform(ragged);
@@ -578,7 +604,7 @@
     info.unmag = ((neg & 8) && (kGyro * bmax) / (fm * 1e6) < kUnmagTol) ? 1 : 0;
     info.poly_angle = trig == 5 ? 0 : (trig == 1 ? 4 : (trig == 2 ? 1 : (trig == 3 ? 2 : 3)));
     if (info.poly_angle == 4) {
-        for (int k = tid; k < K; k += THREADS) {
+        for (int k = tid; k < K; k += TEAM) {
             double sp, cp;
             prhf_cr::sincos_table(nodes[k].psi * kDegToRad, &sp, &cp);
             nodes[k].u0 = (cp - sp) * (cp + sp);
@@ -586,7 +612,7 @@
             nodes[k].u2 = 2.0 * (sp * cp);
             nodes[k].u3 = qnan();
         }
-        __syncthreads();
+        team_sync<TEAM, THREADS>();
     }
     const double a0 = uniform(nodes[0].alt);
     const double span = uniform(nodes[K - 1].alt) - a0;
@@ -596,7 +622,7 @@
     info.inv_w = (span > 0.0) ? (double)kHintBuckets / span : 0.0;
     if (!info.uniform) {
         const double w = span / (double)kHintBuckets;
-        for (int b = tid; b < kHintBuckets; b += THREADS) {
+        for (int b = tid; b < kHintBuckets; b += TEAM) {
             const double t = a0 + (double)b * w;
             int lo = 0, hi = K - 1;
             while (lo < hi) {
@@ -605,7 +631,7 @@
             }
             hint[b] = (unsigned short)lo;
         }
-        __syncthreads();
+        team_sync<TEAM, THREADS>();
     }
     return info;
 }
@@ -1892,17 +1918,25 @@
     __syncthreads();
 }
 
-template <int THREADS>
+template <int THREADS, int TEAM = THREADS>
 __device__ __forceinline__ int list_candidates(const KArgs& a, const SegDev& sg, const double* keep,
                                                long long pair_base, unsigned short* cand, int* cand_count,
                                                const Node* nodes, const double* pf2, const double* gb, int K,
                                                double* heights) {
-    constexpr int W = THREADS / 64;
-    const int tid = threadIdx.x, lane = tid & 63, wave = tid >> 6;
+    constexpr int W = TEAM / 64;
+    const int tid = team_tid<TEAM, THREADS>(), lane = tid & 63, wave = tid >> 6;
     const int F = (int)a.n_freq;
+    constexpr bool kDefer = TEAM != THREADS;
+    constexpr int kRounds = kDefer ? THREADS / TEAM : 1;
+    [[maybe_unused]] double h_kept[kRounds];
+    [[maybe_unused]] int pos_kept[kRounds];
+    if constexpr (kDefer) {
+#pragma unroll
+        for (int r = 0; r < kRounds; ++r) { h_kept[r] = 0.0; pos_kept[r] = -1; }
+    }
     const double pmax = keep[kKeepPf2Max], gmax = keep[kKeepGbMax];
     int total = 0;
-    for (int base = 0; base < F; base += THREADS) {
+    for (int base = 0; base < F; base += TEAM) {
         const int f = base + tid;
         bool may = false;
         double h = 0.0;
@@ -2008,7 +2042,7 @@
         }
         const unsigned long long mask = __ballot(may);
         if (lane == 0) cand_count[wave] = __popcll(mask);
-        __syncthreads();
+        team_sync<TEAM, THREADS>();
         int at = total, chunk = 0;
 #pragma unroll
         for (int w = 0; w < W; ++w) {
@@ -2019,10 +2053,25 @@
         if (may) {
             const int pos = at + __popcll(mask & ((1ull << lane) - 1ull));
             cand[pos] = (unsigned short)f;
-            if (heights) heights[pos] = h;
-        }
-        __syncthreads();
+            if constexpr (!kDefer) {
+                if (heights) heights[pos] = h;
+            } else {
+                const int round = base / TEAM;
+#pragma unroll
+                for (int r = 0; r < kRounds; ++r)
+                    if (r == round) { h_kept[r] = h; pos_kept[r] = pos; }
+            }
+        }
+        team_sync<TEAM, THREADS>();
         total += chunk;
+    }
+    if constexpr (kDefer) {
+        if (heights) {
+#pragma unroll
+            for (int r = 0; r < kRounds; ++r)
+                if (pos_kept[r] >= 0) heights[pos_kept[r]] = h_kept[r];
+        }
+        team_sync<TEAM, THREADS>();
     }
     return uniform(total);
 }
@@ -2110,6 +2159,7 @@
                                      : r.base2 + (unsigned)(i - r.cap01) * (unsigned)kPlanBytes);
 }
 
+template <int FORM>
 __device__ __attribute__((noinline)) bool plan_pair(const Node* nodes, int K, const double2* __restrict__ pairs, int n_points,
                                                     double span, double kj, double cX, double cY2, bool grade,
                                                     unsigned* rec) {
@@ -2170,7 +2220,7 @@
     return true;
 }
 
-template <int TIER, int THREADS, bool G>
+template <int TIER, int THREADS, bool G, int TEAM = THREADS>
 __device__ __forceinline__ PlanRoom plan_pairs(const KArgs& a, const SegDev& sg, const Node* nodes, double* pf2, double* gb,
                                                unsigned short* hint, const unsigned short* cand, const BlockInfo& info,
                                                int block_in_prof, int blocks_per_prof, unsigned* plan_cnt) {
@@ -2198,7 +2248,7 @@
     if (a.plan_cap > 0) room.total = min(room.total, a.plan_cap);
     const int first_item = block_in_prof * W, round_items = blocks_per_prof * W;
     int n_planned = 0, n_self = 0;
-    for (int u = threadIdx.x;; u += THREADS) {
+    for (int u = team_tid<TEAM, THREADS>();; u += TEAM) {
         const int t = (u / W) * round_items + first_item + (u % W);
         if (t >= info.n_cand) break;
         const double span = info.heights[t] - info.a0;
@@ -2212,7 +2262,7 @@
                                                             : reinterpret_cast<unsigned*>(pf2 + used) + kWords * (u - room.cap01));
             if (main_loop) {
                 const double* row = a.ftab + 8 * (long long)cand[t];
-                done = plan_pair(nodes, info.K, pairs, sg.n_points, span, kj, row[2], row[3], sg.strided_grade != 0, rec);
+                done = plan_pair<TEAM == THREADS ? 0 : 1>(nodes, info.K, pairs, sg.n_points, span, kj, row[2], row[3], sg.strided_grade != 0, rec);
             }
             if (!done) rec[3] = 0u;
         }
@@ -2222,8 +2272,8 @@
     }
     if (n_planned) atomicAdd(&plan_cnt[0], (unsigned)n_planned);
     if (n_self) atomicAdd(&plan_cnt[1], (unsigned)n_self);
-    __syncthreads();
-    if (threadIdx.x == 0 && a.plan_counters) {
+    team_sync<TEAM, THREADS>();
+    if (team_tid<TEAM, THREADS>() == 0 && a.plan_counters) {
         if (plan_cnt[0]) atomicAdd(&a.plan_counters[0], (unsigned long long)plan_cnt[0]);
         if (plan_cnt[1]) atomicAdd(&a.plan_counters[1], (unsigned long long)plan_cnt[1]);
     }
@@ -2385,6 +2435,7 @@
     }
     const PlanRoom room = plan_pairs<TIER, THREADS, G>(a, sg, nodes, pf2, gb, hint, cand, info, block_in_prof, blocks_per_prof,
                                                        plan_cnt);
+    PRHF_MARK(3);
     if (sg.mode == PRHF_KMODE_O)
         run_items<PRHF_KMODE_O, TIER, THREADS, G>(a, sg, nodes, pf2, gb, hint, cand, info, prof_local, block_in_prof,
                                                blocks_per_prof, item_next, red, room);
@@ -2467,13 +2518,15 @@
         (void)t_staged;
 #ifdef PRHF_TRACE
         if (a.trace && (threadIdx.x & 63) == 0) {
-            unsigned long long* t = a.trace + (bid * (THREADS / 64) + (threadIdx.x >> 6)) * 6;
+            unsigned long long* t = a.trace + (bid * (THREADS / 64) + (threadIdx.x >> 6)) * 8;
             t[0] = t_start;
             t[1] = wall_clock64();
             t[2] = t_staged;
             t[3] = trace_marks()[0];
             t[4] = trace_marks()[1];
             t[5] = trace_marks()[2];
+            t[6] = trace_marks()[3];
+            t[7] = blockIdx.x;
         }
 #endif
         if (a.queue == nullptr) break;
@@ -2493,6 +2546,214 @@
 template <int THREADS>
 __global__ __launch_bounds__(THREADS, PRHF_MIN_WAVES_PER_SIMD) void vfo_tall_kernel(const KArgs a) {
     vfo_kernel_body<2, THREADS, true>(a);
+}
+
+struct SlotHeader {
+    int state;
+    int item_next;
+    int left;
+    unsigned plan_cnt[2];
+    int cand_count[2];
+    BlockInfo info;
+    PlanRoom room;
+    long long prof_local, bid;
+    int block_in_prof, bpp, prio;
+};
+constexpr int kSlotFinished = 0x7fffffff;
+constexpr int kSlotAbort = -1;
+constexpr unsigned long long kStallTicks = 400000000ull;
+
+struct SlotArrays {
+    Node* nodes;
+    double* pf2;
+    double* gb;
+    unsigned short* hint;
+    unsigned short* cand;
+    double* red;
+};
+__device__ __forceinline__ SlotArrays slot_arrays(unsigned char* smem, int slot, int levels) {
+    unsigned char* base = smem + (size_t)slot * lds_bytes_for(levels);
+    SlotArrays s;
+    s.nodes = reinterpret_cast<Node*>(base);
+    s.pf2 = reinterpret_cast<double*>(base + (size_t)(levels + 1) * sizeof(Node));
+    s.gb = s.pf2 + levels;
+    s.hint = reinterpret_cast<unsigned short*>(s.pf2 + 2 * (size_t)levels);
+    s.cand = s.hint + kHintBuckets;
+    s.red = reinterpret_cast<double*>(s.cand + PRHF_MAX_CAND);
+    return s;
+}
+
+__device__ __forceinline__ int slot_wait(SlotHeader* h, int gen, int* abort_word, unsigned* status) {
+    const int lane = threadIdx.x & 63;
+    const unsigned long long t0 = wall_clock64();
+    for (;;) {
+        int st = 0, ab = 0;
+        if (lane == 0) {
+            st = __hip_atomic_load(&h->state, __ATOMIC_RELAXED, __HIP_MEMORY_SCOPE_WORKGROUP);
+            ab = __hip_atomic_load(abort_word, __ATOMIC_RELAXED, __HIP_MEMORY_SCOPE_WORKGROUP);
+        }
+        st = uniform(st);
+        ab = uniform(ab);
+        if (ab) return kSlotAbort;
+        if (st >= gen) {
+            __builtin_amdgcn_fence(__ATOMIC_ACQUIRE, "workgroup");
+            return st;
+        }
+        if (wall_clock64() - t0 > kStallTicks) {
+            if (lane == 0) {
+                __hip_atomic_store(abort_word, 1, __ATOMIC_RELAXED, __HIP_MEMORY_SCOPE_WORKGROUP);
+                post_status(status, PRHF_STATUS_STALL);
+            }
+            return kSlotAbort;
+        }
+        __builtin_amdgcn_s_sleep(8);
+    }
+}
+
+template <int LAYOUT>
+__device__ __forceinline__ void stage_slot(const KArgs& a, const SegDev& sg, SlotHeader* h, const SlotArrays& s, long long ticket,
+                                           int gen, long long resident) {
+    const int lane = threadIdx.x & 63;
+    if (ticket >= a.n_blocks) {
+        if (lane == 0) __hip_atomic_store(&h->state, kSlotFinished, __ATOMIC_RELEASE, __HIP_MEMORY_SCOPE_WORKGROUP);
+        return;
+    }
+    team_mark<64, LAYOUT>(4);
+    __builtin_amdgcn_s_setprio(3);
+    long long lb = ticket - sg.block_begin;
+    const long long head_blocks = sg.tail_prof * sg.blocks_per_prof;
+    int bpp = sg.blocks_per_prof;
+    long long prof0 = 0;
+    if (lb >= head_blocks) {
+        lb -= head_blocks;
+        bpp = sg.tail_bpp;
+        prof0 = sg.tail_prof;
+    }
+    const long long prof_local = prof0 + lb / bpp;
+    const int block_in_prof = (int)(lb % bpp);
+    const long long left = a.n_blocks - ticket;
+    const int prio = left > 3 * resident ? 3 : (left > 2 * resident ? 2 : (left > resident ? 1 : 0));
+    if (lane == 0) {
+        h->item_next = 0;
+        h->plan_cnt[0] = h->plan_cnt[1] = 0u;
+    }
+    const long long p = sg.prof_begin + prof_local;
+    BlockInfo info = stage_profile<1, LAYOUT, 64>(
+        a.den + p * a.prof_stride, a.bmag + p * a.field_stride, a.bpsi + p * a.field_stride,
+        a.alt + p * a.alt_stride, a.freq, (int)a.n_freq, (int)a.n_alt, s.nodes, s.pf2, s.gb, s.hint, s.red, (int)a.lds_levels);
+    team_mark<64, LAYOUT>(1);
+    if (info.nan_b && !info.bad) info.bad = kNanRow;
+    info.n_cand = -1;
+    info.heights = nullptr;
+    if (a.ftab && !a.no_candidates && sg.chunks == 1 && a.n_freq <= PRHF_MAX_CAND && !info.bad && info.K > 1) {
+        double* heights = (a.n_freq <= a.lds_levels && a.n_freq <= LAYOUT && sg.thread_scan) ? s.pf2 : nullptr;
+        info.n_cand = list_candidates<LAYOUT, 64>(a, sg, kept_scalars<LAYOUT>(s.red), prof_local * a.n_freq, s.cand,
+                                                  h->cand_count, s.nodes, s.pf2, s.gb, info.K, heights);
+        info.heights = heights;
+    }
+    team_mark<64, LAYOUT>(2);
+    if (lane == 0 && block_in_prof == 0 && info.bad) post_status(a.status, (unsigned)info.bad);
+    const PlanRoom room = plan_pairs<1, LAYOUT, false, 64>(a, sg, s.nodes, s.pf2, s.gb, s.hint, s.cand, info, block_in_prof, bpp,
+                                                           h->plan_cnt);
+    if (lane == 0) {
+        h->info = info;
+        h->room = room;
+        h->prof_local = prof_local;
+        h->bid = ticket;
+        h->block_in_prof = block_in_prof;
+        h->bpp = bpp;
+        h->prio = prio;
+        __hip_atomic_store(&h->state, gen, __ATOMIC_RELEASE, __HIP_MEMORY_SCOPE_WORKGROUP);
+    }
+    team_mark<64, LAYOUT>(3);
+#ifdef PRHF_TRACE
+    if (a.trace && lane == 0) {
+        unsigned long long* t = a.trace + (ticket * (blockDim.x / 64) + (threadIdx.x >> 6)) * 8;
+        const unsigned long long* m = trace_marks() + 8 + 8 * (threadIdx.x >> 6);
+        t[3] = m[0]; t[4] = m[1]; t[5] = m[2]; t[6] = m[3]; t[7] = m[4];
+    }
+#endif
+}
+
+template <int THREADS>
+__global__ __launch_bounds__(THREADS, PRHF_MIN_WAVES_PER_SIMD) void vfo_stream_kernel(const KArgs a) {
+    constexpr int LAYOUT = PRHF_BLOCK_THREADS, W = THREADS / 64;
+    extern __shared__ __attribute__((aligned(16))) unsigned char smem[];
+    __shared__ SlotHeader hdr[2];
+    __shared__ int abort_word;
+    const int lane = threadIdx.x & 63, wave = uniform((int)(threadIdx.x >> 6));
+    const int levels = (int)a.lds_levels;
+    const SegDev& sg = a.seg[0];
+    const long long resident = 2 * (long long)gridDim.x;
+    if (threadIdx.x < 2) {
+        hdr[threadIdx.x].state = 0;
+        hdr[threadIdx.x].left = 0;
+    }
+    if (threadIdx.x == 0) abort_word = 0;
+    __syncthreads();
+    if (wave < 2) stage_slot<LAYOUT>(a, sg, &hdr[wave], slot_arrays(smem, wave, levels), (long long)blockIdx.x + wave * (long long)gridDim.x,
+                                     1, resident);
+    for (int visit = 0;; ++visit) {
+        const int slot = visit & 1, gen = (visit >> 1) + 1;
+        SlotHeader* h = &hdr[slot];
+#ifdef PRHF_TRACE
+        const unsigned long long t_arrive = wall_clock64();
+#endif
+        const int st = slot_wait(h, gen, &abort_word, a.status);
+        if (st == kSlotFinished || st == kSlotAbort) break;
+#ifdef PRHF_TRACE
+        const unsigned long long t_ready = wall_clock64();
+#endif
+        const SlotArrays s = slot_arrays(smem, slot, levels);
+        BlockInfo info;
+        info.K = uniform(h->info.K);
+        info.bad = uniform(h->info.bad);
+        info.unmag = uniform(h->info.unmag);
+        info.uniform = uniform(h->info.uniform);
+        info.poly_angle = uniform(h->info.poly_angle);
+        info.n_cand = uniform(h->info.n_cand);
+        info.nan_b = uniform(h->info.nan_b);
+        info.nan_p = uniform(h->info.nan_p);
+        info.heights = uniform(h->info.heights != nullptr ? 1 : 0) ? s.pf2 : nullptr;
+        info.a0 = uniform(h->info.a0);
+        info.inv_w = uniform(h->info.inv_w);
+        info.inv_step = uniform(h->info.inv_step);
+        PlanRoom room;
+        room.base0 = (unsigned)uniform((int)h->room.base0);
+        room.base1 = (unsigned)uniform((int)h->room.base1);
+        room.base2 = (unsigned)uniform((int)h->room.base2);
+        room.cap0 = uniform(h->room.cap0);
+        room.cap01 = uniform(h->room.cap01);
+        room.total = uniform(h->room.total);
+        const int block_in_prof = uniform(h->block_in_prof), bpp = uniform(h->bpp), prio = uniform(h->prio);
+        const long long prof_local = ((long long)uniform((int)(h->prof_local >> 32)) << 32) |
+                                     (unsigned)uniform((int)(h->prof_local & 0xffffffffLL));
+        if (prio >= 2) __builtin_amdgcn_s_setprio(2);
+        else if (prio == 1) __builtin_amdgcn_s_setprio(1);
+        else __builtin_amdgcn_s_setprio(0);
+        run_items<PRHF_KMODE_X, 1, LAYOUT, false>(a, sg, s.nodes, s.pf2, s.gb, s.hint, s.cand, info, prof_local, block_in_prof, bpp,
+                                                  &h->item_next, s.red, room);
+#ifdef PRHF_TRACE
+        if (a.trace && lane == 0) {
+            const long long bid = h->bid;
+            unsigned long long* t = a.trace + (bid * W + wave) * 8;
+            t[0] = t_arrive;
+            t[1] = wall_clock64();
+            t[2] = t_ready;
+        }
+#endif
+        int n_left = 0;
+        if (lane == 0) n_left = __hip_atomic_fetch_add(&h->left, 1, __ATOMIC_ACQ_REL, __HIP_MEMORY_SCOPE_WORKGROUP);
+        if (uniform(n_left) == W - 1) {
+            long long ticket = 0;
+            if (lane == 0) {
+                h->left = 0;
+                ticket = resident + (long long)atomicAdd(a.queue, 1u);
+            }
+            ticket = (long long)(unsigned)uniform((int)ticket);
+            stage_slot<LAYOUT>(a, sg, h, s, ticket, gen + 1, resident);
+        }
+    }
 }
 
 __global__ void grid_pairs_kernel(const double* __restrict__ mult, long long n, double2* __restrict__ pairs) {
@@ -3016,6 +3277,14 @@
 #include "prhf_gradient_skip.inc"
 #include "prhf_vjp.inc"
 
+hipError_t launch_vfo_stream(const KArgs& a, long long grid_blocks, hipStream_t stream) {
+    if (grid_blocks <= 0 || a.n_blocks <= 0) return hipSuccess;
+    if (!a.queue || a.n_segs != 1 || a.block_list || a.seg[0].slots != 0 || a.seg[0].chunks != 1) return hipErrorInvalidValue;
+    hipLaunchKernelGGL((vfo_stream_kernel<PRHF_STREAM_THREADS>), dim3((unsigned)grid_blocks), dim3(PRHF_STREAM_THREADS),
+                       2 * lds_bytes_for(a.lds_levels), stream, a);
+    return hipGetLastError();
+}
+
 hipError_t query_occupancy(int tier, size_t lds_bytes, int* blocks_per_cu) {
     constexpr int THREADS = PRHF_BLOCK_THREADS;
     if (tier == 0)
@@ -3025,7 +3294,12 @@
     return hipOccupancyMaxActiveBlocksPerMultiprocessor(blocks_per_cu, vfo_kernel<2, THREADS>, THREADS, lds_bytes);
 }
 
-hipError_t configure_kernels(size_t max_lds_bytes) {
+hipError_t configure_kernels(size_t max_lds_bytes, size_t max_stream_lds_bytes) {
+    {
+        hipError_t e = hipFuncSetAttribute(reinterpret_cast<const void*>(&vfo_stream_kernel<PRHF_STREAM_THREADS>),
+                                           hipFuncAttributeMaxDynamicSharedMemorySize, (int)max_stream_lds_bytes);
+        if (e != hipSuccess) return e;
+    }
     constexpr int THREADS = PRHF_BLOCK_THREADS;
     const void* kernels[] = {reinterpret_cast<const void*>(&vfo_kernel<0, THREADS>),
                              reinterpret_cast<const void*>(&vfo_kernel<1, THREADS>),
diff --git a/pyrayhf_amd/csrc/prhf_plan.h b/pyrayhf_amd/csrc/prhf_plan.h
--- a/pyrayhf_amd/csrc/prhf_plan.h
+++ b/pyrayhf_amd/csrc/prhf_plan.h
@@ -47,6 +47,8 @@
     double strided_grade = 1;
     double pair_plan = 1;
     double pair_plan_cap = 0;
+    double stream_blocks = 1;
+    double stream_grid = 0;
 };
 struct KnobName {
     const char* name;
@@ -87,6 +89,8 @@
     {"strided_grade", &Knobs::strided_grade, 0, 1},
     {"pair_plan", &Knobs::pair_plan, 0, 1},
     {"pair_plan_cap", &Knobs::pair_plan_cap, 0, 1024},
+    {"stream_blocks", &Knobs::stream_blocks, 0, 2},
+    {"stream_grid", &Knobs::stream_grid, 0, 65536},
 };
 constexpr int kWavesPerBlock = PRHF_BLOCK_THREADS / 64;
 
@@ -281,6 +285,12 @@
     bool short_order;
     bool zero_queues;
     bool forked;
+    bool stream;
+    long long stream_grid;
+    size_t stream_lds_bytes;
+    long long stream_blocks;
+    int stream_tail_bpp;
+    long long stream_tail_prof;
     prhf::StridedPieces pieces;
     prhf::SegDev seg[PRHF_MAX_SEGMENTS];
     ShortKind o, x;
@@ -457,6 +467,35 @@
             pl.any_plan = pl.any_plan || s.pair_plan != 0;
         }
     }
+    pl.stream = false;
+    pl.stream_grid = 0;
+    pl.stream_lds_bytes = 0;
+    pl.stream_blocks = 0;
+    pl.stream_tail_bpp = 0;
+    pl.stream_tail_prof = 0;
+    if (kn.stream_blocks != 0 && kPersistent && !tall && pl.n_segs == 1 && pl.o.n_segs == 0 && pl.x.n_segs == 0 && pl.blocks > 0 &&
+        (pl.queue || kn.stream_blocks == 2) && 2 * pl.lds_bytes <= kLdsFull) {
+        Knobs with_plans = kn;
+        with_plans.pair_plan = 1;
+        if (slice_plans_pairs(pl.seg[0], tall, n_freq, lds_levels, with_plans)) {
+            pl.stream = true;
+            pl.queue = true;
+            const prhf::SegDev& s = pl.seg[0];
+            const long long P = s.prof_end - s.prof_begin;
+            pl.stream_blocks = pl.blocks;
+            pl.stream_tail_bpp = s.tail_bpp;
+            pl.stream_tail_prof = s.tail_prof;
+            if (s.tail_prof < P && s.tail_bpp > s.blocks_per_prof) {
+                const int bpp = std::max(s.blocks_per_prof, s.tail_bpp / (PRHF_STREAM_THREADS / PRHF_BLOCK_THREADS));
+                pl.stream_blocks -= (P - s.tail_prof) * (s.tail_bpp - bpp);
+                pl.stream_tail_bpp = bpp;
+                if (bpp == s.blocks_per_prof) pl.stream_tail_prof = P;
+            }
+            pl.stream_lds_bytes = 2 * pl.lds_bytes;
+            pl.stream_grid = std::min<long long>(sh.cu_count, (pl.stream_blocks + 1) / 2);
+            if (kn.stream_grid > 0) pl.stream_grid = std::min(pl.stream_grid, (long long)kn.stream_grid);
+        }
+    }
     pl.freq_table = pl.want_pairs && (n_prof * n_freq >= 4096 || pl.any_plan);
     pl.short_order = pl.freq_table && pl.o.blocks > 0 && kn.short_order != 0 && pl.o.blocks >= 4 * pl.o.first.slots;
     const bool any_short = pl.o.n_segs > 0 || pl.x.n_segs > 0;
```

Result: faster. 393.8 million (median of 6 runs) (+3.7%).
